# yu45020/Text_Segmentation_Image_Inpainting

Measured on NVIDIA H100. Metric: PartialConv UNet 512x512 images/sec (fwd+bwd), higher is better.
Workload: dtype bf16

## Files before the change

### text_segmentation_image_inpainting_b200/csrc/conv_tc.cu

```cuda
#include <cuda.h>
#include <stdlib.h>
#include <string.h>

#include <algorithm>

#include "pcb_common.cuh"
#include "pcb_ptx.cuh"

namespace {

constexpr int BLOCK_M = 128;
constexpr int BLOCK_K = 64;
constexpr int A_STAGE_BYTES = BLOCK_M * 128;
constexpr int NUM_PRODUCER_THREADS = 128;
constexpr int TC_MAX_PARTS = 2;
constexpr int MMA_WARPS = 8;
constexpr int MMA_THREADS = MMA_WARPS * 32;
constexpr int acc_pitch(int block_n) { return block_n + 4; }
constexpr int acc_stage_bytes(int block_n) { return BLOCK_M * acc_pitch(block_n) * 4; }

inline int rup(int v, int m) { return (v + m - 1) / m * m; }

struct TcPart {
    const bf16 *x;
    const uint64_t *tapmask;
    const uint8_t *mask;
    bf16 *dx;
    int c, c8, kext, koff, choff, cstride, xup, mup, dx_cstride;
};

struct TcParams {
    int n, h, w, cin, cout, kh, kw, stride, pad_h, pad_w, dil, ho, wo;
    int m_total;
    int nparts, no_guard, rowpack;
    int hg;
    int ring_a, ring_b;
    int ktap;
    int ncols;
    TcPart parts[TC_MAX_PARTS];
    const float *bias; const float *msum; bf16 *y; int y_cstride;
    const bf16 *dc; int dc_cstride, dc_c8, dc_kext;
    int *abort_flag;
    int l2pf;
    int box_w, box_h, box_n, stages, use_fix;
    int wk_base, wk_row, wk_col;
    int sub, py, px, fh, fw;
    int ksplit;
    float *partial;
    double *bn_sums;
    int bn_c;
    const float *ep_scale, *ep_shift;
    int ep_on, ep_act;
    float ep_slope;
};

constexpr int STAT_SLICE = 256;
constexpr int STAT_SMEM_BYTES = MMA_WARPS * STAT_SLICE * 4 + 16;
constexpr int EPI_WARPS = 4;
constexpr int EPI_STAT_SMEM_BYTES = EPI_WARPS * STAT_SLICE * 4;

__device__ __forceinline__ float warp_transpose_sum(float (&v)[32], int lane) {
#pragma unroll
    for (int off = 16, n = 32; off >= 1; off >>= 1, n >>= 1) {
        const bool upper = (lane & off) != 0;
#pragma unroll
        for (int i = 0; i < 16; ++i) {
            if (i < (n >> 1)) {
                const float send = upper ? v[i] : v[i + (n >> 1)];
                const float keep = upper ? v[i + (n >> 1)] : v[i];
                v[i] = keep + __shfl_xor_sync(0xffffffffu, send, off);
            }
        }
    }
    return v[0];
}

__device__ __forceinline__ uint32_t align1024(uint32_t a) { return (a + 1023u) & ~1023u; }

__device__ __forceinline__ void load_acc32(const float *src, uint32_t (&r)[32]) {
#pragma unroll
    for (int j = 0; j < 8; ++j) {
        const uint4 v = reinterpret_cast<const uint4 *>(src)[j];
        r[4 * j] = v.x; r[4 * j + 1] = v.y; r[4 * j + 2] = v.z; r[4 * j + 3] = v.w;
    }
}

struct EpiRow {
    long long mo;
    int m;
    bool rvalid, hole;
    float inv;
    float dscale[TC_MAX_PARTS];
};

template <int MODE>
__device__ __forceinline__ EpiRow tc_epi_row(const TcParams &P, int m) {
    EpiRow er;
    er.m = m;
    er.rvalid = m < P.m_total;
    er.inv = 0.f;
    er.hole = false;
    er.mo = m;
    int en = 0, eh = 0, ew = 0;
    if (MODE == 1 && er.rvalid) {
        en = m / (P.h * P.w); const int rem = m - en * P.h * P.w; eh = rem / P.w; ew = rem - eh * P.w;
        eh = eh * P.sub + P.py; ew = ew * P.sub + P.px;
        er.mo = (static_cast<long long>(en) * P.fh + eh) * P.fw + ew;
    }
    if (MODE == 0 && er.rvalid && P.sub != 1) {
        en = m / (P.ho * P.wo); const int rem = m - en * P.ho * P.wo; eh = rem / P.wo; ew = rem - eh * P.wo;
        er.mo = (static_cast<long long>(en) * P.fh + eh * P.sub + P.py) * P.fw + ew * P.sub + P.px;
    }
    if (MODE == 0 && er.rvalid) {
        const float s = P.msum ? P.msum[er.mo] : 1.f;
        er.hole = (s == 0.f) && !P.no_guard;
        er.inv = er.hole ? 0.f : 1.0f / s;
    }
#pragma unroll
    for (int p = 0; p < TC_MAX_PARTS; ++p) {
        er.dscale[p] = 1.f;
        if (MODE == 1 && p < P.nparts) {
            const TcPart &pt = P.parts[p];
            if (er.rvalid && pt.dx != nullptr && pt.mask != nullptr)
                er.dscale[p] = pt.mask[(static_cast<long long>(en) * (P.fh >> pt.mup) + (eh >> pt.mup)) * (P.fw >> pt.mup) + (ew >> pt.mup)] ? 1.f : 0.f;
        }
    }
    return er;
}

template <int BLOCK_N, int MODE>
__device__ __forceinline__ void tc_epilogue(const TcParams &P, const EpiRow &er, const float *acc_row, int lane, int n0, float *s_stat,
                                            int cb, int ce, int sq_off) {
                const int m = er.m;
                const bool rvalid = er.rvalid, hole = er.hole;
                const long long mo = er.mo;
                if (P.partial != nullptr) {
    #pragma unroll 1
                    for (int c0 = cb; c0 < ce; c0 += 32) {
                        uint32_t r[32];
                        load_acc32(acc_row + c0, r);
                        if (rvalid) {
                            float *dst = P.partial + static_cast<long long>(m) * P.ncols + n0 + c0;
    #pragma unroll
                            for (int j = 0; j < 32; ++j) atomicAdd(dst + j, __uint_as_float(r[j]));
                        }
                    }
                    return;
                }
    #pragma unroll 1
                for (int c0 = cb; c0 < ce; c0 += 32) {
                    uint32_t r[32];
                    load_acc32(acc_row + c0, r);
                    const int col = n0 + c0;
                    bf16 *orow = nullptr;
                    int nstore = 0;
                    float scale = er.inv;
                    if (MODE == 0) {
                        if (rvalid && col < P.y_cstride) { orow = P.y + mo * P.y_cstride + col; nstore = min(32, P.y_cstride - col); }
                    } else {
                        scale = 1.f;
#pragma unroll
                        for (int p = 0; p < TC_MAX_PARTS; ++p) {
                            if (p >= P.nparts) break;
                            const TcPart &pt = P.parts[p];
                            const int local = col - pt.koff;
                            if (local >= 0 && local < pt.kext && pt.dx != nullptr && local < pt.c8 && rvalid) {
                                orow = pt.dx + mo * pt.dx_cstride + local;
                                nstore = min(32, pt.c8 - local);
                                scale = er.dscale[p];
                            }
                        }
                    }
                    const bool stats = (MODE == 0) && (s_stat != nullptr);
                    if (__any_sync(0xffffffffu, nstore > 0) || stats) {
                        uint4 o[4];
                        __nv_bfloat162 *ob = reinterpret_cast<__nv_bfloat162 *>(o);
                        float bl = 0.f;
                        const bool has_bias = (MODE == 0) && (P.bias != nullptr);
                        if (has_bias && col + lane < P.cout) bl = P.bias[col + lane];
                        const bool edge = (MODE == 0) && (col + 32 > P.cout);
                        const bool ep = (MODE == 0) && (P.ep_on != 0);
                        float el = 1.f, eh = 0.f;
                        if (ep && P.ep_scale != nullptr && col + lane < P.cout) { el = P.ep_scale[col + lane]; eh = P.ep_shift[col + lane]; }
    #pragma unroll
                        for (int j = 0; j < 16; ++j) {
                            float a = __uint_as_float(r[2 * j]), b = __uint_as_float(r[2 * j + 1]);
                            if (MODE == 0) {
                                const float b0 = has_bias ? __shfl_sync(0xffffffffu, bl, 2 * j) : 0.f;
                                const float b1 = has_bias ? __shfl_sync(0xffffffffu, bl, 2 * j + 1) : 0.f;
                                a = hole ? 0.f : fmaf(a, scale, b0);
                                b = hole ? 0.f : fmaf(b, scale, b1);
                                if (ep) {
                                    a = apply_act(fmaf(a, __shfl_sync(0xffffffffu, el, 2 * j), __shfl_sync(0xffffffffu, eh, 2 * j)), P.ep_act, P.ep_slope);
                                    b = apply_act(fmaf(b, __shfl_sync(0xffffffffu, el, 2 * j + 1), __shfl_sync(0xffffffffu, eh, 2 * j + 1)), P.ep_act, P.ep_slope);
                                }
                                if (edge) {
                                    if (col + 2 * j >= P.cout) a = 0.f;
                                    if (col + 2 * j + 1 >= P.cout) b = 0.f;
                                }
                            } else {
                                a *= scale; b *= scale;
                            }
                            ob[j] = __floats2bfloat162_rn(a, b);
                        }
                        if (nstore > 0) {
                            uint4 *dst = reinterpret_cast<uint4 *>(orow);
    #pragma unroll
                            for (int j = 0; j < 4; ++j)
                                if (j * 8 < nstore) dst[j] = o[j];
                        }
                        if (stats) {
                            float v[32], q[32];
                            const float live = rvalid ? 1.f : 0.f;
    #pragma unroll
                            for (int j = 0; j < 16; ++j) {
                                const float2 f = __bfloat1622float2(ob[j]);
                                v[2 * j] = f.x * live; v[2 * j + 1] = f.y * live;
                                q[2 * j] = v[2 * j] * v[2 * j]; q[2 * j + 1] = v[2 * j + 1] * v[2 * j + 1];
                            }
                            const float cs = warp_transpose_sum(v, lane), cq = warp_transpose_sum(q, lane);
                            s_stat[c0 - cb + lane] += cs;
                            s_stat[sq_off + c0 - cb + lane] += cq;
                        }
                    }
                }
}

template <int BLOCK_N>
__device__ __forceinline__ void tc_stats_flush(const TcParams &P, float *s_stat, int lane, int n0, int cb, int ce, int sq_off) {
    __syncwarp();
    for (int c0 = cb; c0 < ce; c0 += 32) {
        const int co = n0 + c0 + lane;
        if (co < P.bn_c) {
            atomicAdd(P.bn_sums + co, static_cast<double>(s_stat[c0 - cb + lane]));
            atomicAdd(P.bn_sums + P.bn_c + co, static_cast<double>(s_stat[sq_off + c0 - cb + lane]));
        }
        s_stat[c0 - cb + lane] = 0.f; s_stat[sq_off + c0 - cb + lane] = 0.f;
    }
    __syncwarp();
}

template <int BLOCK_N>
struct EpiRole {
    static constexpr int HN = (BLOCK_N >= 64) ? BLOCK_N / 2 : BLOCK_N;
    int q, half, cb, ce;
    __device__ __forceinline__ explicit EpiRole(int e) {
        q = 2 * (e >> 2) + (e & 1);
        half = (e & 3) >> 1;
        cb = half * HN;
        ce = (cb + HN <= BLOCK_N) ? cb + HN : cb;
    }
    __device__ __forceinline__ int slice() const { return half * 4 + q; }
};

template <int BLOCK_N>
__device__ __forceinline__ void stage_acc(const float (&acc)[BLOCK_N / 2], float *stage, int e, int lane) {
    constexpr int PITCH = acc_pitch(BLOCK_N);
    const int r0 = 64 * (e >> 2) + 16 * (e & 3) + (lane >> 2), c0 = 2 * (lane & 3);
#pragma unroll
    for (int i = 0; i < BLOCK_N / 2; i += 2) {
        const int row = r0 + 8 * ((i >> 1) & 1), col = 8 * (i >> 2) + c0;
        *reinterpret_cast<float2 *>(stage + row * PITCH + col) = make_float2(acc[i], acc[i + 1]);
    }
}

template <int BLOCK_N, int MODE>
__device__ __forceinline__ void mma_epilogue(const TcParams &P, const float (&acc)[BLOCK_N / 2], float *stage, int e, int lane, int m0, int n0,
                                             float *s_stat) {
    constexpr int PITCH = acc_pitch(BLOCK_N);
    const int g = e >> 2;
    stage_acc<BLOCK_N>(acc, stage, e, lane);
    ptx::named_sync(1 + g, 128);
    const EpiRole<BLOCK_N> R(e);
    const EpiRow er = tc_epi_row<MODE>(P, m0 + R.q * 32 + lane);
    tc_epilogue<BLOCK_N, MODE>(P, er, stage + (R.q * 32 + lane) * PITCH, lane, n0, s_stat, R.cb, R.ce, 128);
    ptx::named_sync(1 + g, 128);
}

template <int BLOCK_N>
__device__ __forceinline__ void tc_stats_final(const TcParams &P, const float *stat_base, int w, int lane, int stat_n0) {
    for (int col = w * 32 + lane; col < BLOCK_N; col += EPI_WARPS * 32) {
        const int co = stat_n0 + col;
        if (co < P.bn_c) {
            float a = 0.f, q = 0.f;
#pragma unroll
            for (int w4 = 0; w4 < EPI_WARPS; ++w4) { a += stat_base[w4 * STAT_SLICE + col]; q += stat_base[w4 * STAT_SLICE + 128 + col]; }
            atomicAdd(P.bn_sums + co, static_cast<double>(a));
            atomicAdd(P.bn_sums + P.bn_c + co, static_cast<double>(q));
        }
    }
}

template <int R> __device__ __forceinline__ void zero_acc(float (&a)[R]) {
#pragma unroll
    for (int i = 0; i < R; ++i) a[i] = 0.f;
}

constexpr int HALO_MAX_HG = 12;
constexpr int PERSIST_THREADS = 4 * 32 + MMA_THREADS + 32;
constexpr int MAX_RING = 8;

template <int BLOCK_N, int MODE, bool HALO>
__global__ void __launch_bounds__(PERSIST_THREADS, 1)
pconv_tc_persistent_kernel(const __grid_constant__ TcParams P, const __grid_constant__ CUtensorMap tmap_w) {
    constexpr int B_STAGE_BYTES = BLOCK_N * 128;
    extern __shared__ uint8_t smem_raw[];
    const uint32_t smem_base = align1024(ptx::smem_u32(smem_raw));
    const int SA = P.ring_a, SB = P.ring_b;
    const int HG = P.hg;
    const uint32_t LBO = 16u * (16u * HG + 1u);
    const uint32_t A_STAGE = HALO ? ((8u * LBO + 127u) & ~127u) : static_cast<uint32_t>(A_STAGE_BYTES);
    const uint32_t sB = smem_base;
    const uint32_t sA = sB + SB * B_STAGE_BYTES;
    const uint32_t sBar = (sA + SA * A_STAGE + 15u) & ~15u;
    const uint32_t bar_full_a = sBar, bar_empty_a = sBar + 8 * MAX_RING;
    const uint32_t bar_full_b = sBar + 16 * MAX_RING, bar_empty_b = sBar + 24 * MAX_RING;
    const uint32_t s_stat_addr = sBar + 32 * MAX_RING;
    const uint32_t s_acc = (s_stat_addr + STAT_SMEM_BYTES + 15u) & ~15u;
    float *acc_stage = reinterpret_cast<float *>(smem_raw + (s_acc - ptx::smem_u32(smem_raw)));

    const int warp = threadIdx.x >> 5, lane = threadIdx.x & 31;
    const int taps = P.kh * P.kw;
    const int np = (MODE == 0) ? P.nparts : 1;
    const int n_tiles = P.ncols / BLOCK_N;
    const int num_tiles = ((P.m_total + BLOCK_M - 1) / BLOCK_M) * n_tiles;
    const int nB = HALO ? P.kw : 1;

    auto tile_active = [&](int n0) -> bool {
        if (MODE == 0) return true;
        for (int p = 0; p < P.nparts; ++p)
            if (P.parts[p].dx && n0 < P.parts[p].koff + P.parts[p].kext && n0 + BLOCK_N > P.parts[p].koff) return true;
        return false;
    };

    if (threadIdx.x == 0) {
        for (int s = 0; s < MAX_RING; ++s) {
            ptx::mbar_init(bar_full_a + 8 * s, NUM_PRODUCER_THREADS); ptx::mbar_init(bar_empty_a + 8 * s, 2);
            ptx::mbar_init(bar_full_b + 8 * s, 1); ptx::mbar_init(bar_empty_b + 8 * s, 2);
        }
        ptx::fence_mbar_init();
    }
    if (warp == 12 && lane == 0) ptx::prefetch_tmap(&tmap_w);
    __syncthreads();

    if (warp < 4) {
        const int t = threadIdx.x;
        const int chunk = t & 7, r0 = t >> 3;
        const int plane = (MODE == 0) ? P.ho * P.wo : P.h * P.w;
        const int pwid = (MODE == 0) ? P.wo : P.w;
        int it = 0;
        bool dead = false;
        constexpr int NW = HALO ? HALO_MAX_HG : 8;
        uint64_t wnext[TC_MAX_PARTS][NW];
        auto issue_mask_loads = [&](int tl) {
#pragma unroll
            for (int p = 0; p < TC_MAX_PARTS; ++p)
#pragma unroll
                for (int i = 0; i < NW; ++i) wnext[p][i] = 0ull;
            if (MODE != 0 || tl >= num_tiles) return;
            const int tm0 = (tl / n_tiles) * BLOCK_M;
#pragma unroll
            for (int i = 0; i < NW; ++i) {
                int idx;
                if (HALO) {
                    if (i >= HG) continue;
                    const int S = r0 + 16 * i;
                    const int g = S / HG, sl = S - g * HG;
                    const int tcs = sl > 7 ? (sl - 7 + P.dil - 1) / P.dil : 0;
                    idx = tm0 + g * 8 + (sl - tcs * P.dil);
                    if (tm0 + g * 8 >= P.m_total) continue;
                } else {
                    idx = tm0 + r0 + 16 * i;
                    if (idx >= P.m_total) continue;
                }
#pragma unroll
                for (int p = 0; p < TC_MAX_PARTS; ++p)
                    if (p < P.nparts) wnext[p][i] = __ldg(P.parts[p].tapmask + idx);
            }
        };
        issue_mask_loads(blockIdx.x);
        for (int tile = blockIdx.x; tile < num_tiles && !dead; tile += gridDim.x) {
            const int m0 = (tile / n_tiles) * BLOCK_M, n0 = (tile % n_tiles) * BLOCK_N;
            uint64_t wcur[TC_MAX_PARTS][NW];
#pragma unroll
            for (int p = 0; p < TC_MAX_PARTS; ++p)
#pragma unroll
                for (int i = 0; i < NW; ++i) wcur[p][i] = wnext[p][i];
            issue_mask_loads(tile + gridDim.x);
            if (!tile_active(n0)) continue;
            if (HALO) {
                int ph[HALO_MAX_HG];
                int cterm[TC_MAX_PARTS][HALO_MAX_HG];
                uint32_t vb[TC_MAX_PARTS][HALO_MAX_HG];
#pragma unroll
                for (int i = 0; i < HALO_MAX_HG; ++i) {
                    ph[i] = 0;
#pragma unroll
                    for (int p = 0; p < TC_MAX_PARTS; ++p) { vb[p][i] = 0; cterm[p][i] = 0; }
                    if (i >= HG) continue;
                    const int S = r0 + 16 * i;
                    const int g = S / HG, sl = S - g * HG;
                    const int m = m0 + g * 8;
                    const bool ok = m < P.m_total;
                    const int mm = ok ? m : 0;
                    const int nn = mm / plane, rem = mm - nn * plane;
                    const int hh = rem / pwid, ww = rem - hh * pwid;
                    if (MODE == 0) {
                        ph[i] = hh - P.pad_h;
                        const int col = ww - P.pad_w + sl;
                        const int tcs = sl > 7 ? (sl - 7 + P.dil - 1) / P.dil : 0;
#pragma unroll
                        for (int p = 0; p < TC_MAX_PARTS; ++p) {
                            if (p >= P.nparts || !ok) continue;
                            const TcPart &pt = P.parts[p];
                            const uint64_t word = wcur[p][i];
                            uint32_t bits = 0;
                            for (int tr = 0; tr < P.kh; ++tr) bits |= static_cast<uint32_t>((word >> (tr * P.kw + tcs)) & 1ull) << tr;
                            vb[p][i] = bits;
                            const int colc = min(max(col, 0), P.w - 1) >> pt.xup;
                            cterm[p][i] = (nn * (P.h >> pt.xup) * (P.w >> pt.xup) + colc) * pt.cstride + chunk * 8;
                        }
                    } else {
                        ph[i] = hh + P.pad_h;
                        const int col = ww + P.pad_w - (P.kw - 1) * P.dil + sl;
                        const bool cok = ok && col >= 0 && col < P.wo;
                        uint32_t bits = 0;
                        for (int tr = 0; tr < P.kh; ++tr) { const int hi = ph[i] - tr * P.dil; bits |= (cok && hi >= 0 && hi < P.ho ? 1u : 0u) << tr; }
                        vb[0][i] = bits;
                        cterm[0][i] = (nn * P.ho * P.wo + min(max(col, 0), P.wo - 1)) * P.dc_cstride + chunk * 8;
                    }
                }
                for (int tr = 0; tr < P.kh && !dead; ++tr) {
#pragma unroll
                    for (int p = 0; p < TC_MAX_PARTS; ++p) {
                        if (p >= np || dead) break;
                        const TcPart &pt = P.parts[p];
                        const bf16 *src = (MODE == 0) ? pt.x : P.dc;
                        const int xup = (MODE == 0) ? pt.xup : 0;
                        const int hmax = ((MODE == 0) ? (P.h >> xup) : P.ho) - 1;
// ... 75 lines not shown
                            const bool v = (chunk < P.kw) && ((tmv[0][i] >> (tr * P.kw + chunk)) & 1ull);
                            off[i] = v ? (ibase[0][i] - chunk * 8) + (ph[i] + tr * P.dil) * rowpitch + (pw[i] + chunk * P.dil) * cs : 0;
                            ok[i] = v;
                        }
                        if (!push(pt.x, off, ok)) dead = true;
                    }
                } else {
                    for (int tap = 0; tap < taps && !dead; ++tap) {
                        const int tr = tap / P.kw, tc = tap - tr * P.kw;
#pragma unroll
                        for (int p = 0; p < TC_MAX_PARTS; ++p) {
                            if (p >= np || dead) break;
                            const TcPart &pt = P.parts[p];
                            const bf16 *src = (MODE == 0) ? pt.x : P.dc;
                            const int cs = (MODE == 0) ? pt.cstride : P.dc_cstride;
                            const int xup = (MODE == 0) ? pt.xup : 0;
                            const int rowpitch = ((MODE == 0) ? (P.w >> xup) : P.wo) * cs;
                            int base[8];
                            bool rv[8];
#pragma unroll
                            for (int i = 0; i < 8; ++i) {
                                bool v;
                                int hi, wi;
                                if (MODE == 0) {
                                    v = (tmv[p][i] >> tap) & 1ull;
                                    hi = (ph[i] + tr * P.dil) >> xup; wi = (pw[i] + tc * P.dil) >> xup;
                                } else {
                                    const int th = ph[i] - tr * P.dil, tw = pw[i] - tc * P.dil;
                                    hi = th >> ls; wi = tw >> ls;
                                    v = prow[i] && th >= 0 && tw >= 0 && ((th | tw) & (P.stride - 1)) == 0 && hi < P.ho && wi < P.wo;
                                }
                                base[i] = v ? ibase[p][i] + hi * rowpitch + wi * cs : 0;
                                rv[i] = v;
                            }
                            const int nb = ((MODE == 0) ? pt.kext : P.dc_kext) / BLOCK_K;
                            const int c8 = (MODE == 0) ? pt.c8 : P.dc_c8;
                            for (int cb = 0; cb < nb; ++cb) {
                                const bool cv = cb * BLOCK_K + chunk * 8 < c8;
                                int off[8];
                                bool ok[8];
#pragma unroll
                                for (int i = 0; i < 8; ++i) { ok[i] = rv[i] && cv; off[i] = ok[i] ? base[i] + cb * BLOCK_K : 0; }
                                if (!push(src, off, ok)) { dead = true; break; }
                            }
                        }
                    }
                }
            }
        }
        ptx::cp_async_wait<0>();
    } else if (warp == 12) {
        if (lane == 0) {
            int itb = 0;
            bool dead = false;
            auto load = [&](int kidx, int n0) -> bool {
                const int s = itb % SB;
                if (!ptx::mbar_wait(bar_empty_b + 8 * s, ((itb / SB) & 1) ^ 1, P.abort_flag, 103)) return false;
                ptx::mbar_arrive_expect_tx(bar_full_b + 8 * s, B_STAGE_BYTES);
                ptx::tma_load_2d(sB + s * B_STAGE_BYTES, &tmap_w, kidx, n0, bar_full_b + 8 * s);
                ++itb;
                return true;
            };
            for (int tile = blockIdx.x; tile < num_tiles && !dead; tile += gridDim.x) {
                const int n0 = (tile % n_tiles) * BLOCK_N;
                if (!tile_active(n0)) continue;
                if (HALO) {
                    for (int tr = 0; tr < P.kh && !dead; ++tr)
                        for (int p = 0; p < np && !dead; ++p) {
                            const int nb = ((MODE == 0) ? P.parts[p].kext : P.dc_kext) / BLOCK_K;
                            for (int cb = 0; cb < nb && !dead; ++cb)
                                for (int tc = 0; tc < P.kw; ++tc) {
                                    const int tap = tr * P.kw + tc;
                                    const int kidx = (MODE == 0) ? tap * P.ktap + P.parts[p].koff + cb * BLOCK_K : tap * P.dc_kext + cb * BLOCK_K;
                                    if (!load(kidx, n0)) { dead = true; break; }
                                }
                        }
                } else {
                    const int num_kb = (MODE == 0) ? (P.rowpack ? P.kh : taps * (P.ktap / BLOCK_K)) : taps * (P.dc_kext / BLOCK_K);
                    for (int kb = 0; kb < num_kb; ++kb)
                        if (!load(kb * BLOCK_K, n0)) { dead = true; break; }
                }
            }
        }
    } else {
        const int e = warp - 4, g = e >> 2;
        const bool leader = (threadIdx.x & 127) == 0;
        int num_a = 0;
        if (HALO) {
            for (int p = 0; p < np; ++p) num_a += ((MODE == 0) ? P.parts[p].kext : P.dc_kext) / BLOCK_K;
            num_a *= P.kh;
        } else {
            num_a = (MODE == 0) ? (P.rowpack ? P.kh : taps * (P.ktap / BLOCK_K)) : taps * (P.dc_kext / BLOCK_K);
        }
        const uint32_t a_rows = HALO ? 8u * HG * 16u : 64u * 128u;
        float *s_stat = (MODE == 0 && P.bn_sums != nullptr && P.partial == nullptr)
                            ? reinterpret_cast<float *>(smem_raw + (s_stat_addr - ptx::smem_u32(smem_raw))) : nullptr;
        const EpiRole<BLOCK_N> R(e);
        float *my_stat = s_stat ? s_stat + R.slice() * STAT_SLICE : nullptr;
        int stat_n0 = -1;
        if (my_stat) {
            for (int i = lane; i < STAT_SLICE; i += 32) my_stat[i] = 0.f;
            __syncwarp();
        }
        int ita = 0, itb = 0;
        bool dead = false;
        for (int tile = blockIdx.x; tile < num_tiles && !dead; tile += gridDim.x) {
            const int m0 = (tile / n_tiles) * BLOCK_M, n0 = (tile % n_tiles) * BLOCK_N;
            if (!tile_active(n0)) continue;
            if (my_stat && n0 != stat_n0) {
                if (stat_n0 >= 0) tc_stats_flush<BLOCK_N>(P, my_stat, lane, stat_n0, R.cb, R.ce, 128);
                stat_n0 = n0;
            }
            float acc[BLOCK_N / 2];
            zero_acc(acc);
            for (int a = 0; a < num_a && !dead; ++a, ++ita) {
                const int sa = ita % SA;
                if (!__all_sync(0xffffffffu, ptx::mbar_wait(bar_full_a + 8 * sa, (ita / SA) & 1, P.abort_flag, 104))) { dead = true; break; }
                ptx::fence_proxy_async_smem();
                const int sb0 = itb % SB;
                for (int tc = 0; tc < nB; ++tc, ++itb) {
                    const int sb = itb % SB;
                    if (!__all_sync(0xffffffffu, ptx::mbar_wait(bar_full_b + 8 * sb, (itb / SB) & 1, P.abort_flag, 105))) { dead = true; break; }
                    const uint64_t db = ptx::make_smem_desc(sB + sb * B_STAGE_BYTES, 16, 1024);
                    ptx::wgmma_fence();
                    if (HALO) {
                        const int shift = ((MODE == 0) ? tc : (P.kw - 1 - tc)) * P.dil;
                        const uint32_t a0 = sA + sa * A_STAGE + g * a_rows + shift * 16;
#pragma unroll
                        for (int k = 0; k < BLOCK_K / 16; ++k)
                            ptx::wgmma_bf16<BLOCK_N, 0, 0>(acc, ptx::make_smem_desc_noswizzle(a0 + k * 2 * LBO, LBO, HG * 16), db + 2 * k);
                    } else {
                        const uint64_t da = ptx::make_smem_desc(sA + sa * A_STAGE + g * a_rows, 16, 1024);
#pragma unroll
                        for (int k = 0; k < BLOCK_K / 16; ++k)
                            ptx::wgmma_bf16<BLOCK_N, 0, 0>(acc, da + 2 * k, db + 2 * k);
                    }
                    ptx::wgmma_commit();
                }
                ptx::wgmma_wait<0>();
                ptx::wgmma_fence_regs(acc);
                if (leader) {
                    for (int tc = 0; tc < nB; ++tc) ptx::mbar_arrive(bar_empty_b + 8 * ((sb0 + tc) % SB));
                    ptx::mbar_arrive(bar_empty_a + 8 * sa);
                }
            }
            if (dead) { stat_n0 = -1; break; }
            mma_epilogue<BLOCK_N, MODE>(P, acc, acc_stage, e, lane, m0, n0, my_stat);
        }
        if (my_stat && stat_n0 >= 0) tc_stats_flush<BLOCK_N>(P, my_stat, lane, stat_n0, R.cb, R.ce, 128);
    }
}


constexpr int EPI_WARP0 = MMA_WARPS + 5;
constexpr int TMA_THREADS = (EPI_WARP0 + EPI_WARPS) * 32;

constexpr size_t TMA_BAR_BYTES = 24 * MAX_RING + 16;

template <int BLOCK_N, int MODE, typename TileFn>
__device__ __forceinline__ void tma_epilogue_warps(const TcParams &P, int tile0, int tstep, int num_tiles, TileFn tile_origin,
                                                   const float *acc_stage, uint32_t acc_full, uint32_t acc_empty, float *s_stat,
                                                   int &stat_n0, int w, int lane, int code) {
    constexpr int PITCH = acc_pitch(BLOCK_N);
    const float *acc_row = acc_stage + (w * 32 + lane) * PITCH;
    if (s_stat) {
        for (int i = lane; i < STAT_SLICE; i += 32) s_stat[i] = 0.f;
        __syncwarp();
    }
    uint32_t ph = 0;
    for (int tile = tile0; tile < num_tiles; tile += tstep) {
        int m0, n0;
        tile_origin(tile, m0, n0);
        if (n0 < 0) continue;
        if (s_stat && n0 != stat_n0) {
            if (stat_n0 >= 0) tc_stats_flush<BLOCK_N>(P, s_stat, lane, stat_n0, 0, BLOCK_N, 128);
            stat_n0 = n0;
        }
        const EpiRow er = tc_epi_row<MODE>(P, m0 + w * 32 + lane);
        if (!__all_sync(0xffffffffu, ptx::mbar_wait(acc_full, ph, P.abort_flag, code))) { stat_n0 = -1; return; }
        ph ^= 1;
        tc_epilogue<BLOCK_N, MODE>(P, er, acc_row, lane, n0, s_stat, 0, BLOCK_N, 128);
        __syncwarp();
        if (lane == 0) ptx::mbar_arrive(acc_empty);
    }
}

template <int BLOCK_N>
__device__ __forceinline__ bool tma_stage_tile(const TcParams &P, const float (&acc)[BLOCK_N / 2], float *acc_stage, uint32_t acc_full,
                                               uint32_t acc_empty, uint32_t &ph, int e, int lane, int code) {
    if (!__all_sync(0xffffffffu, ptx::mbar_wait(acc_empty, ph, P.abort_flag, code))) return false;
    ph ^= 1;
    stage_acc<BLOCK_N>(acc, acc_stage, e, lane);
    __syncwarp();
    if (lane == 0) ptx::mbar_arrive(acc_full);
    return true;
}

template <int BLOCK_N, int MODE, bool HALO>
__global__ void __launch_bounds__(TMA_THREADS, 1)
pconv_tc_tma_kernel(const __grid_constant__ TcParams P, const __grid_constant__ CUtensorMap tmap_w,
                    const __grid_constant__ CUtensorMap tmap_a0, const __grid_constant__ CUtensorMap tmap_a1) {
    constexpr uint32_t B_BYTES = BLOCK_N * 128;
    extern __shared__ uint8_t smem_raw[];
    const uint32_t smem_base = align1024(ptx::smem_u32(smem_raw));
    const int S = P.stages;
    const int nB = HALO ? P.kw : 1;
    const int hx = HALO ? (P.kw - 1) * P.dil : 0;
    const uint32_t A_BYTES = static_cast<uint32_t>(BLOCK_M + hx) * 128u;
    const uint32_t A_ROOM = (A_BYTES + 1023u) & ~1023u;
    const uint32_t STAGE = A_ROOM + nB * B_BYTES;
    const uint32_t STAGE_TX = A_BYTES + nB * B_BYTES;
    const uint32_t sBar = smem_base + S * STAGE;
    const uint32_t bar_full = sBar, bar_fixed = sBar + 8 * MAX_RING, bar_empty = sBar + 16 * MAX_RING;
    const uint32_t acc_full = sBar + 24 * MAX_RING, acc_empty = acc_full + 8;
    const uint32_t s_stat_addr = sBar + TMA_BAR_BYTES;
    const uint32_t s_acc = s_stat_addr + EPI_STAT_SMEM_BYTES;
    uint8_t *smem_gen = smem_raw + (smem_base - ptx::smem_u32(smem_raw));

    const int warp = __shfl_sync(0xffffffffu, threadIdx.x >> 5, 0), lane = threadIdx.x & 31;
    const int np = (MODE == 0) ? P.nparts : 1;
    const int n_tiles = P.ncols / BLOCK_N;
    const int KS = P.ksplit;
    const int m_tiles = (P.m_total + BLOCK_M - 1) / BLOCK_M;
    const int num_tiles = m_tiles * n_tiles * KS;
    const int tile0 = static_cast<int>(blockIdx.x), tstep = static_cast<int>(gridDim.x);
    auto m0_of = [&](int mt) -> int { return mt * BLOCK_M; };
    const bool fix = (MODE == 0) && P.use_fix;
    const int kwi = HALO ? 1 : P.kw;

    auto tile_active = [&](int n0) -> bool {
        if (MODE == 0) return true;
        for (int p = 0; p < P.nparts; ++p)
            if (P.parts[p].dx && n0 < P.parts[p].koff + P.parts[p].kext && n0 + BLOCK_N > P.parts[p].koff) return true;
        return false;
    };

    if (threadIdx.x == 0) {
        for (int s = 0; s < MAX_RING; ++s) {
            ptx::mbar_init(bar_full + 8 * s, 1); ptx::mbar_init(bar_fixed + 8 * s, 4); ptx::mbar_init(bar_empty + 8 * s, 2);
        }
        ptx::mbar_init(acc_full, MMA_WARPS); ptx::mbar_init(acc_empty, EPI_WARPS);
        ptx::fence_mbar_init();
    }
    if (warp == 8 && lane == 0) { ptx::prefetch_tmap(&tmap_w); ptx::prefetch_tmap(&tmap_a0); if (np > 1) ptx::prefetch_tmap(&tmap_a1); }
    __syncthreads();

    float *s_stat = nullptr;
    int stat_n0 = -1;
    float *acc_stage = reinterpret_cast<float *>(smem_gen + (s_acc - smem_base));
    if (warp >= EPI_WARP0) {
        const int w = warp - EPI_WARP0;
        s_stat = (MODE == 0 && P.bn_sums != nullptr && P.partial == nullptr)
                     ? reinterpret_cast<float *>(smem_gen + (s_stat_addr - smem_base)) + w * STAT_SLICE : nullptr;
        auto origin = [&](int tile, int &m0, int &n0) {
            const int mn = tile / KS;
            m0 = m0_of(mn / n_tiles); n0 = (mn % n_tiles) * BLOCK_N;
            if (!tile_active(n0)) n0 = -1;
        };
        tma_epilogue_warps<BLOCK_N, MODE>(P, tile0, tstep, num_tiles, origin, acc_stage, acc_full, acc_empty, s_stat, stat_n0, w, lane, 126);
    } else if (warp == 8) {
        int s = 0;
        uint32_t ph = 1;
        const int plane = (MODE == 0) ? P.ho * P.wo : P.h * P.w;
        const int pwid = (MODE == 0) ? P.wo : P.w;
        const int kext0 = (MODE == 0) ? P.parts[0].kext : P.dc_kext, kext1 = (MODE == 0 && np > 1) ? P.parts[1].kext : 0;
        const int dstep = (MODE == 0) ? P.dil : -P.dil;
        const int row_k = P.wk_row, col_k = P.wk_col;
        bool dead = false;
        for (int tile = tile0; tile < num_tiles && !dead; tile += tstep) {
            const int sp = tile % KS, mn = tile / KS;
            const int m0 = m0_of(mn / n_tiles), n0 = (mn % n_tiles) * BLOCK_N;
            if (!tile_active(n0)) continue;
            const int img = m0 / plane, rem = m0 - img * plane;
            const int oy = rem / pwid, ox = rem - oy * pwid;
            const int x_org = (MODE == 0) ? ox * P.stride - P.pad_w : (HALO ? ox + P.pad_w - hx : ox + P.pad_w);
            const int y_org = (MODE == 0) ? oy * P.stride - P.pad_h : oy + P.pad_h;
            int nx_org = 0, ny_org = 0, nimg = -1;
            if (P.l2pf && tile + tstep < num_tiles) {
                const int nmn = (tile + tstep) / KS;
                const int nm0 = m0_of(nmn / n_tiles);
                if (nm0 != m0) {
                    nimg = nm0 / plane;
                    const int nrem = nm0 - nimg * plane, noy = nrem / pwid, nox = nrem - noy * pwid;
                    nx_org = (MODE == 0) ? nox * P.stride - P.pad_w : (HALO ? nox + P.pad_w - hx : nox + P.pad_w);
                    ny_org = (MODE == 0) ? noy * P.stride - P.pad_h : noy + P.pad_h;
                }
            }
            int krow = P.wk_base;
            for (int tr = 0, y = y_org; tr < P.kh && !dead; ++tr, y += dstep, krow += row_k)
                for (int ti = 0, x = x_org, kidx = krow; ti < kwi && !dead; ++ti, x += dstep, kidx = krow + ti * col_k) {
#pragma unroll
                    for (int p = 0; p < TC_MAX_PARTS; ++p) {
                        const int kext = (p == 0) ? kext0 : kext1;
                        const CUtensorMap *ma = (p == 0) ? &tmap_a0 : &tmap_a1;
                        const int gb0 = (p == 0) ? 0 : kext0 / BLOCK_K;
                        for (int c0 = 0; c0 < kext; c0 += BLOCK_K, kidx += BLOCK_K) {
                            if (KS > 1 && (gb0 + c0 / BLOCK_K) % KS != sp) continue;
                            if (!__all_sync(0xffffffffu, ptx::mbar_wait(bar_empty + 8 * s, ph, P.abort_flag, 121))) { dead = true; break; }
                            if (ptx::elect_one()) {
                                const uint32_t full = bar_full + 8 * s, dst = smem_base + s * STAGE;
                                ptx::mbar_arrive_expect_tx(full, STAGE_TX);
                                ptx::tma_load_4d(dst, ma, c0, x, y, img, full);
                                uint32_t bdst = dst + A_ROOM;
                                for (int tc = 0, kb = kidx; tc < nB; ++tc, kb += col_k, bdst += B_BYTES)
                                    ptx::tma_load_2d(bdst, &tmap_w, kb, n0, full);
                                if (nimg >= 0) ptx::tma_prefetch_4d(ma, c0, nx_org + ti * dstep, ny_org + tr * dstep, nimg);
                            }
                            __syncwarp();
                            if (++s == S) { s = 0; ph ^= 1; }
                        }
                        if (dead) break;
                    }
                }
        }
    } else if (warp < MMA_WARPS) {
        const int e = warp, g = warp >> 2;
        const bool leader = (threadIdx.x & 127) == 0;
        const uint32_t ready = fix ? bar_fixed : bar_full;
        const uint64_t desc_a0 = ptx::make_smem_desc(smem_base + g * 64 * 128, 16, 1024);
        const uint64_t desc_b0 = ptx::make_smem_desc(smem_base + A_ROOM, 16, 1024);
        const uint32_t stage16 = STAGE >> 4;
        const int shift0 = (HALO && MODE == 1) ? hx * 8 : 0;
        const int dshift = HALO ? ((MODE == 1) ? -P.dil * 8 : P.dil * 8) : 0;
        const int rows_a = P.kh * kwi;
        int nb0, nb1 = 0, kl0, kl1 = 4;
        {
            const int kext = (MODE == 0) ? P.parts[0].kext : P.dc_kext, c8 = (MODE == 0) ? P.parts[0].c8 : P.dc_c8;
            nb0 = kext / BLOCK_K; kl0 = min(4, (c8 - (nb0 - 1) * BLOCK_K + 15) >> 4);
            if (MODE == 0 && np > 1) { nb1 = P.parts[1].kext / BLOCK_K; kl1 = min(4, (P.parts[1].c8 - (nb1 - 1) * BLOCK_K + 15) >> 4); }
        }
        int s = 0;
        uint32_t ph = 0, aph = 1;
        bool dead = false;
        for (int tile = tile0; tile < num_tiles && !dead; tile += tstep) {
            const int sp = tile % KS, mn = tile / KS;
            const int n0 = (mn % n_tiles) * BLOCK_N;
            if (!tile_active(n0)) continue;
            float acc[BLOCK_N / 2];
            zero_acc(acc);
            int held = -1;
            for (int r = 0; r < rows_a && !dead; ++r) {
#pragma unroll
                for (int p = 0; p < TC_MAX_PARTS; ++p) {
                    const int nbp = (p == 0) ? nb0 : nb1, klast = (p == 0) ? kl0 : kl1;
                    const int gb0 = (p == 0) ? 0 : nb0;
                    for (int cb = 0; cb < nbp; ++cb) {
                        if (KS > 1 && (gb0 + cb) % KS != sp) continue;
                        if (!__all_sync(0xffffffffu, ptx::mbar_wait(ready + 8 * s, ph, P.abort_flag, 124))) { dead = true; break; }
                        uint64_t da = desc_a0 + static_cast<uint64_t>(s * stage16 + shift0), db = desc_b0 + static_cast<uint64_t>(s * stage16);
                        const int ksteps = (cb + 1 < nbp) ? 4 : klast;
                        ptx::wgmma_fence();
                        for (int tc = 0; tc < nB; ++tc, da += dshift, db += B_BYTES >> 4) {
                            if (ksteps == 4) {
#pragma unroll
                                for (int k = 0; k < 4; ++k) ptx::wgmma_bf16<BLOCK_N, 0, 0>(acc, da + 2 * k, db + 2 * k);
                            } else {
                                for (int k = 0; k < ksteps; ++k) ptx::wgmma_bf16<BLOCK_N, 0, 0>(acc, da + 2 * k, db + 2 * k);
                            }
                        }
                        ptx::wgmma_commit();
                        ptx::wgmma_wait<1>();
                        if (held >= 0 && leader) ptx::mbar_arrive(bar_empty + 8 * held);
                        held = s;
                        if (++s == S) { s = 0; ph ^= 1; }
                    }
                    if (dead) break;
                }
            }
            ptx::wgmma_wait<0>();
            ptx::wgmma_fence_regs(acc);
            if (held >= 0 && leader) ptx::mbar_arrive(bar_empty + 8 * held);
            if (dead) break;
            if (!tma_stage_tile<BLOCK_N>(P, acc, acc_stage, acc_full, acc_empty, aph, e, lane, 125)) break;
        }
    } else if (warp > 8) {
        if (fix) {
            const int t = (warp - 9) * 32 + lane;
            int s = 0;
            uint32_t ph = 0;
            bool dead = false;
            if (!HALO) {
                uint64_t wnext[TC_MAX_PARTS];
                auto load_words = [&](int tl) {
#pragma unroll
                    for (int p = 0; p < TC_MAX_PARTS; ++p) {
                        wnext[p] = 0ull;
                        const int m = m0_of(tl / KS / n_tiles) + t;
                        if (fix && p < P.nparts && tl < num_tiles && m < P.m_total) wnext[p] = __ldg(P.parts[p].tapmask + m);
                    }
                };
                load_words(tile0);
                for (int tile = tile0; tile < num_tiles && !dead; tile += tstep) {
                    const int sp = tile % KS;
                    uint64_t wcur[TC_MAX_PARTS];
#pragma unroll
                    for (int p = 0; p < TC_MAX_PARTS; ++p) wcur[p] = wnext[p];
                    load_words(tile + tstep);
                    if (MODE == 1 && !tile_active(((tile / KS) % n_tiles) * BLOCK_N)) continue;
                    const int taps = P.kh * P.kw;
                    for (int tap = 0; tap < taps && !dead; ++tap) {
#pragma unroll
                        for (int p = 0; p < TC_MAX_PARTS; ++p) {
                            if (p >= np) break;
                            const bool hole = fix && ((wcur[p] >> tap) & 1ull) == 0ull;
                            const bool any_hole = __any_sync(0xffffffffu, hole);
                            const int nb = ((MODE == 0) ? P.parts[p].kext : P.dc_kext) / BLOCK_K;
                            const int gb0 = (p == 0) ? 0 : P.parts[0].kext / BLOCK_K;
                            for (int cb = 0; cb < nb; ++cb) {
                                if (KS > 1 && (gb0 + cb) % KS != sp) continue;
                                if (!ptx::mbar_wait(bar_full + 8 * s, ph, P.abort_flag, 122)) { dead = true; break; }
                                if (any_hole) {
                                    if (hole) {
                                        uint4 *r = reinterpret_cast<uint4 *>(smem_gen + s * STAGE + t * 128);
                                        const uint4 z = make_uint4(0u, 0u, 0u, 0u);
#pragma unroll
                                        for (int k = 0; k < 8; ++k) r[k] = z;
                                    }
                                    ptx::fence_proxy_async_smem();
                                }
                                __syncwarp();
                                if (lane == 0) ptx::mbar_arrive(bar_fixed + 8 * s);
                                if (++s == S) { s = 0; ph ^= 1; }
                            }
                            if (dead) break;
                        }
                    }
                }
            } else {
                const int plane = P.ho * P.wo;
                auto load_bits = [&](int tl, uint32_t &b0, uint32_t &b1) {
                    b0 = b1 = 0;
                    if (!fix || tl >= num_tiles) return;
                    const int m0 = m0_of(tl / KS / n_tiles);
                    const int img = m0 / plane, rem = m0 - img * plane;
                    const int oy = rem / P.wo, ox = rem - oy * P.wo;
#pragma unroll
                    for (int p = 0; p < TC_MAX_PARTS; ++p) {
                        if (p >= P.nparts || P.parts[p].mask == nullptr) continue;
                        const int mup = P.parts[p].mup;
                        const uint8_t *mk = P.parts[p].mask + static_cast<long long>(img) * (P.h >> mup) * (P.w >> mup);
                        for (int tr = 0; tr < P.kh; ++tr) {
                            const int y = oy - P.pad_h + tr * P.dil;
                            if (y < 0 || y >= P.h) continue;
                            const int x0 = ox - P.pad_w + t, x1 = x0 + 128;
                            if (x0 >= 0 && x0 < P.w && __ldg(mk + (y >> mup) * (P.w >> mup) + (x0 >> mup)) == 0) b0 |= 1u << (p * 8 + tr);
                            if (t < hx && x1 < P.w && __ldg(mk + (y >> mup) * (P.w >> mup) + (x1 >> mup)) == 0) b1 |= 1u << (p * 8 + tr);
                        }
                    }
                };
                uint32_t n0b, n1b;
                load_bits(tile0, n0b, n1b);
                for (int tile = tile0; tile < num_tiles && !dead; tile += tstep) {
                    const int sp = tile % KS;
                    const uint32_t c0b = n0b, c1b = n1b;
                    load_bits(tile + tstep, n0b, n1b);
                    if (MODE == 1 && !tile_active(((tile / KS) % n_tiles) * BLOCK_N)) continue;
                    for (int tr = 0; tr < P.kh && !dead; ++tr) {
#pragma unroll
                        for (int p = 0; p < TC_MAX_PARTS; ++p) {
                            if (p >= np) break;
                            const bool h0 = (c0b >> (p * 8 + tr)) & 1u, h1 = (c1b >> (p * 8 + tr)) & 1u;
                            const bool any_hole = __any_sync(0xffffffffu, h0 || h1);
                            const int nb = ((MODE == 0) ? P.parts[p].kext : P.dc_kext) / BLOCK_K;
                            const int gb0 = (p == 0) ? 0 : P.parts[0].kext / BLOCK_K;
                            for (int cb = 0; cb < nb; ++cb) {
                                if (KS > 1 && (gb0 + cb) % KS != sp) continue;
                                if (!ptx::mbar_wait(bar_full + 8 * s, ph, P.abort_flag, 122)) { dead = true; break; }
                                if (any_hole) {
                                    const uint4 z = make_uint4(0u, 0u, 0u, 0u);
                                    if (h0) {
                                        uint4 *r = reinterpret_cast<uint4 *>(smem_gen + s * STAGE + t * 128);
#pragma unroll
                                        for (int k = 0; k < 8; ++k) r[k] = z;
                                    }
                                    if (h1) {
                                        uint4 *r = reinterpret_cast<uint4 *>(smem_gen + s * STAGE + (t + 128) * 128);
#pragma unroll
                                        for (int k = 0; k < 8; ++k) r[k] = z;
                                    }
                                    ptx::fence_proxy_async_smem();
                                }
                                __syncwarp();
                                if (lane == 0) ptx::mbar_arrive(bar_fixed + 8 * s);
                                if (++s == S) { s = 0; ph ^= 1; }
                            }
                            if (dead) break;
                        }
                    }
                }
            }
        }
    }

    __syncthreads();
    if (s_stat != nullptr && stat_n0 >= 0) tc_stats_final<BLOCK_N>(P, s_stat - (warp - EPI_WARP0) * STAT_SLICE, warp - EPI_WARP0, lane, stat_n0);
}


constexpr int SP_MAX_ITEMS = 40;
struct SpItem { int part, dx, dy, wk, nb, wk_step, shift0, dshift; };
struct SpTable {
    int n_items;
    int step[TC_MAX_PARTS];
    int es[TC_MAX_PARTS];
    int ph[TC_MAX_PARTS], pw[TC_MAX_PARTS];
    int arows[TC_MAX_PARTS];
    int rows_max;
    SpItem it[SP_MAX_ITEMS];
};

template <int BLOCK_N, int MODE>
__global__ void __launch_bounds__(TMA_THREADS, 1)
pconv_tc_sp_kernel(const __grid_constant__ TcParams P, const __grid_constant__ SpTable TB, const __grid_constant__ CUtensorMap tmap_w,
                   const __grid_constant__ CUtensorMap tmap_a0, const __grid_constant__ CUtensorMap tmap_a1) {
    constexpr uint32_t B_BYTES = BLOCK_N * 128;
    extern __shared__ uint8_t smem_raw[];
    const uint32_t smem_base = align1024(ptx::smem_u32(smem_raw));
    const int S = P.stages;
    int nb_max = 1;
    for (int i = 0; i < TB.n_items; ++i) nb_max = max(nb_max, TB.it[i].nb);
    const uint32_t A_ROOM = (static_cast<uint32_t>(TB.rows_max) * 128u + 1023u) & ~1023u;
    const uint32_t STAGE = A_ROOM + nb_max * B_BYTES;
    const uint32_t sBar = smem_base + S * STAGE;
    const uint32_t bar_full = sBar, bar_fixed = sBar + 8 * MAX_RING, bar_empty = sBar + 16 * MAX_RING;
    const uint32_t acc_full = sBar + 24 * MAX_RING, acc_empty = acc_full + 8;
    const uint32_t s_stat_addr = sBar + TMA_BAR_BYTES;
    const uint32_t s_acc = s_stat_addr + EPI_STAT_SMEM_BYTES;
    uint8_t *smem_gen = smem_raw + (smem_base - ptx::smem_u32(smem_raw));

    const int warp = __shfl_sync(0xffffffffu, threadIdx.x >> 5, 0), lane = threadIdx.x & 31;
    const int n_tiles = P.ncols / BLOCK_N;
    const int m_tiles = (P.m_total + BLOCK_M - 1) / BLOCK_M;
    const int num_tiles = m_tiles * n_tiles;
    const int tile0 = static_cast<int>(blockIdx.x), tstep = static_cast<int>(gridDim.x);
    const bool fix = P.use_fix != 0;
    const int gw = (MODE == 0) ? P.wo : P.w, gh = (MODE == 0) ? P.ho : P.h;
    const int plane = gw * gh;
    int nbk[TC_MAX_PARTS], klast[TC_MAX_PARTS];
#pragma unroll
    for (int p = 0; p < TC_MAX_PARTS; ++p) {
        const int kext = (MODE == 0) ? P.parts[p].kext : P.dc_kext, c8 = (MODE == 0) ? P.parts[p].c8 : P.dc_c8;
        nbk[p] = (p < ((MODE == 0) ? P.nparts : 1)) ? kext / BLOCK_K : 0;
        klast[p] = nbk[p] ? min(4, (c8 - (nbk[p] - 1) * BLOCK_K + 15) >> 4) : 4;
    }

    if (threadIdx.x == 0) {
        for (int s = 0; s < MAX_RING; ++s) { ptx::mbar_init(bar_full + 8 * s, 1); ptx::mbar_init(bar_fixed + 8 * s, 4); ptx::mbar_init(bar_empty + 8 * s, 2); }
        ptx::mbar_init(acc_full, MMA_WARPS); ptx::mbar_init(acc_empty, EPI_WARPS);
        ptx::fence_mbar_init();
    }
    if (warp == 8 && lane == 0) { ptx::prefetch_tmap(&tmap_w); ptx::prefetch_tmap(&tmap_a0); ptx::prefetch_tmap(&tmap_a1); }
    __syncthreads();

    float *s_stat = nullptr;
    int stat_n0 = -1;
    float *acc_stage = reinterpret_cast<float *>(smem_gen + (s_acc - smem_base));
    if (warp >= EPI_WARP0) {
        const int w = warp - EPI_WARP0;
        s_stat = (MODE == 0 && P.bn_sums != nullptr) ? reinterpret_cast<float *>(smem_gen + (s_stat_addr - smem_base)) + w * STAT_SLICE : nullptr;
        auto origin = [&](int tile, int &m0, int &n0) { m0 = (tile / n_tiles) * BLOCK_M; n0 = (tile % n_tiles) * BLOCK_N; };
        tma_epilogue_warps<BLOCK_N, MODE>(P, tile0, tstep, num_tiles, origin, acc_stage, acc_full, acc_empty, s_stat, stat_n0, w, lane, 326);
    } else if (warp == 8) {
        int s = 0;
        uint32_t ph = 1;
        bool dead = false;
        for (int tile = tile0; tile < num_tiles && !dead; tile += tstep) {
            const int m0 = (tile / n_tiles) * BLOCK_M, n0 = (tile % n_tiles) * BLOCK_N;
            const int img = m0 / plane, rem = m0 - img * plane;
            const int oy = rem / gw, ox = rem - oy * gw;
            for (int i = 0; i < TB.n_items && !dead; ++i) {
                const SpItem it = TB.it[i];
                const CUtensorMap *ma = (it.part == 0) ? &tmap_a0 : &tmap_a1;
                const int x = ox * TB.step[it.part] + it.dx, y = oy * TB.step[it.part] + it.dy;
                const uint32_t a_bytes = static_cast<uint32_t>(TB.arows[it.part]) * 128u;
                for (int cb = 0; cb < nbk[it.part]; ++cb) {
                    if (!__all_sync(0xffffffffu, ptx::mbar_wait(bar_empty + 8 * s, ph, P.abort_flag, 321))) { dead = true; break; }
                    if (ptx::elect_one()) {
                        const uint32_t full = bar_full + 8 * s, dst = smem_base + s * STAGE;
                        ptx::mbar_arrive_expect_tx(full, a_bytes + it.nb * B_BYTES);
                        ptx::tma_load_4d(dst, ma, cb * BLOCK_K, x, y, img, full);
                        uint32_t bdst = dst + A_ROOM;
                        for (int tc = 0, kb = it.wk + cb * BLOCK_K; tc < it.nb; ++tc, kb += it.wk_step, bdst += B_BYTES)
                            ptx::tma_load_2d(bdst, &tmap_w, kb, n0, full);
                    }
                    __syncwarp();
                    if (++s == S) { s = 0; ph ^= 1; }
                }
            }
        }
    } else if (warp < MMA_WARPS) {
        const int e = warp, g = warp >> 2;
        const bool leader = (threadIdx.x & 127) == 0;
        const uint32_t ready = fix ? bar_fixed : bar_full;
        const uint64_t desc_a0 = ptx::make_smem_desc(smem_base + g * 64 * 128, 16, 1024);
        const uint64_t desc_b0 = ptx::make_smem_desc(smem_base + A_ROOM, 16, 1024);
        const uint32_t stage16 = STAGE >> 4;
        int s = 0;
        uint32_t ph = 0, aph = 1;
        bool dead = false;
        for (int tile = tile0; tile < num_tiles && !dead; tile += tstep) {
            float acc[BLOCK_N / 2];
            zero_acc(acc);
            int held = -1;
            for (int i = 0; i < TB.n_items && !dead; ++i) {
                const SpItem it = TB.it[i];
                for (int cb = 0; cb < nbk[it.part]; ++cb) {
                    if (!__all_sync(0xffffffffu, ptx::mbar_wait(ready + 8 * s, ph, P.abort_flag, 324))) { dead = true; break; }
                    uint64_t da = desc_a0 + static_cast<uint64_t>(s * stage16 + it.shift0), db = desc_b0 + static_cast<uint64_t>(s * stage16);
                    const int ksteps = (cb + 1 < nbk[it.part]) ? 4 : klast[it.part];
                    ptx::wgmma_fence();
                    for (int tc = 0; tc < it.nb; ++tc, da += it.dshift, db += B_BYTES >> 4)
                        for (int k = 0; k < ksteps; ++k) ptx::wgmma_bf16<BLOCK_N, 0, 0>(acc, da + 2 * k, db + 2 * k);
                    ptx::wgmma_commit();
                    ptx::wgmma_wait<1>();
                    if (held >= 0 && leader) ptx::mbar_arrive(bar_empty + 8 * held);
                    held = s;
                    if (++s == S) { s = 0; ph ^= 1; }
                }
            }
            ptx::wgmma_wait<0>();
            ptx::wgmma_fence_regs(acc);
            if (held >= 0 && leader) ptx::mbar_arrive(bar_empty + 8 * held);
            if (dead) break;
            if (!tma_stage_tile<BLOCK_N>(P, acc, acc_stage, acc_full, acc_empty, aph, e, lane, 325)) break;
        }
    } else if (warp > 8) {
        if (fix) {
            const int t = (warp - 9) * 32 + lane;
            int s = 0;
            uint32_t ph = 0;
            bool dead = false;
            auto load_bits = [&](int tl, uint64_t &b0, uint64_t &b1) {
                b0 = b1 = 0ull;
                if (tl >= num_tiles) return;
                const int m0 = (tl / n_tiles) * BLOCK_M;
                const int img = m0 / plane, rem = m0 - img * plane;
                const int oy = rem / gw, ox = rem - oy * gw;
                for (int i = 0; i < TB.n_items; ++i) {
                    const SpItem it = TB.it[i];
                    const uint8_t *mk = P.parts[it.part].mask;
                    if (mk == nullptr) continue;
                    const int pwid = TB.pw[it.part], phei = TB.ph[it.part], es = TB.es[it.part];
                    const int hrows = TB.arows[it.part] - BLOCK_M;
                    const int x0 = ox * TB.step[it.part] + it.dx, y0 = oy * TB.step[it.part] + it.dy;
                    int tx, ty, tn;
                    if (hrows > 0 || (P.box_h == 1 && P.box_n == 1)) { tx = t; ty = 0; tn = 0; }
                    else { tx = t % P.box_w; ty = (t / P.box_w) % P.box_h; tn = t / (P.box_w * P.box_h); }
                    const int X = x0 + tx * es, Y = y0 + ty * es, IM = img + tn;
                    if (X >= 0 && X < pwid && Y >= 0 && Y < phei && IM < P.n &&
                        __ldg(mk + (static_cast<long long>(IM) * phei + Y) * pwid + X) == 0) b0 |= 1ull << i;
                    if (t < hrows) {
                        const int X1 = x0 + (t + 128) * es;
                        if (X1 >= 0 && X1 < pwid && Y >= 0 && Y < phei && __ldg(mk + (static_cast<long long>(IM) * phei + Y) * pwid + X1) == 0) b1 |= 1ull << i;
                    }
                }
            };
            uint64_t n0b, n1b;
            load_bits(tile0, n0b, n1b);
            for (int tile = tile0; tile < num_tiles && !dead; tile += tstep) {
                const uint64_t c0b = n0b, c1b = n1b;
                load_bits(tile + tstep, n0b, n1b);
                for (int i = 0; i < TB.n_items && !dead; ++i) {
                    const bool h0 = (c0b >> i) & 1ull, h1 = (c1b >> i) & 1ull;
                    const bool any_hole = __any_sync(0xffffffffu, h0 || h1);
                    const int nb_i = nbk[TB.it[i].part];
                    for (int cb = 0; cb < nb_i; ++cb) {
                        if (!ptx::mbar_wait(bar_full + 8 * s, ph, P.abort_flag, 322)) { dead = true; break; }
                        if (any_hole) {
                            const uint4 z = make_uint4(0u, 0u, 0u, 0u);
                            if (h0) {
                                uint4 *r = reinterpret_cast<uint4 *>(smem_gen + s * STAGE + t * 128);
#pragma unroll
                                for (int k = 0; k < 8; ++k) r[k] = z;
                            }
                            if (h1) {
                                uint4 *r = reinterpret_cast<uint4 *>(smem_gen + s * STAGE + (t + 128) * 128);
#pragma unroll
                                for (int k = 0; k < 8; ++k) r[k] = z;
                            }
                            ptx::fence_proxy_async_smem();
                        }
                        __syncwarp();
                        if (lane == 0) ptx::mbar_arrive(bar_fixed + 8 * s);
                        if (++s == S) { s = 0; ph ^= 1; }
                    }
                }
            }
        }
    }

    __syncthreads();
    if (s_stat != nullptr && stat_n0 >= 0) tc_stats_final<BLOCK_N>(P, s_stat - (warp - EPI_WARP0) * STAT_SLICE, warp - EPI_WARP0, lane, stat_n0);
}

__global__ void upsample_part_kernel(const bf16 *__restrict__ src, int cstride, int c8, long long pixels_src, int hs, int ws, bf16 *__restrict__ dst) {
    const int chunks = c8 >> 3;
    const long long total = pixels_src * chunks;
    for (long long i = blockIdx.x * static_cast<long long>(blockDim.x) + threadIdx.x; i < total; i += static_cast<long long>(gridDim.x) * blockDim.x) {
        const int ch = static_cast<int>(i % chunks);
        const long long pix = i / chunks;
        const int x = static_cast<int>(pix % ws);
        const long long t = pix / ws;
        const int y = static_cast<int>(t % hs);
        const long long n = t / hs;
        const uint4 v = __ldg(reinterpret_cast<const uint4 *>(src + pix * cstride + ch * 8));
        bf16 *d = dst + ((n * (2 * hs) + 2 * y) * (2ll * ws) + 2 * x) * c8 + ch * 8;
        uint4 *d0 = reinterpret_cast<uint4 *>(d), *d1 = reinterpret_cast<uint4 *>(d + 2ll * ws * c8);
        d0[0] = v; *reinterpret_cast<uint4 *>(d + c8) = v;
        d1[0] = v; *reinterpret_cast<uint4 *>(d + 2ll * ws * c8 + c8) = v;
    }
}

struct WgParams {
    int n, h, w, cin, cout, kh, kw, stride, pad_h, pad_w, dil, ho, wo;
    int m_total;
    int nparts, rowpack;
    int ktap;
    int ntaps;
    TcPart parts[TC_MAX_PARTS];
    int tap_groups;
    int ci_tiles;
    int kb_per_split;
    float *dw;
    int *abort_flag;
    int box_w, box_h, box_n, stages, use_fix;
};

constexpr int WGRAD_THREADS = MMA_THREADS + 5 * 32;

template <int BLOCK_N, int T>
__device__ __forceinline__ void wgrad_store(const WgParams &P, const float (&acc)[T][BLOCK_N / 2], int ntap, int lane, int n0,
                                            int ncols, const int (&ci)[2], const int (&tap)[2][T]) {
    const int taps_full = P.kh * P.kw;
#pragma unroll
    for (int tl = 0; tl < T; ++tl) {
        if (tl >= ntap) break;
#pragma unroll
        for (int i = 0; i < BLOCK_N / 2; ++i) {
            if (2 * i >= ncols) break;
            const int h = (i >> 1) & 1;
            const int co = n0 + 8 * (i >> 2) + 2 * (lane & 3) + (i & 1);
            if (ci[h] >= 0 && co < P.cout)
                atomicAdd(P.dw + (static_cast<long long>(co) * taps_full + tap[h][tl]) * P.cin + ci[h], acc[tl][i]);
        }
    }
}

template <int BLOCK_N, int T, int STAGES>
__global__ void __launch_bounds__(WGRAD_THREADS, 1)
pconv_tc_wgrad_kernel(const __grid_constant__ WgParams P, const __grid_constant__ CUtensorMap tmap_dc) {
    constexpr int B_STAGE_BYTES = BLOCK_N * 128;
    constexpr int A_TAP_BYTES = 16384;
    constexpr int A_STAGE = T * A_TAP_BYTES;
    extern __shared__ uint8_t smem_raw[];
    const uint32_t smem_base = align1024(ptx::smem_u32(smem_raw));
    const uint32_t sA = smem_base;
    const uint32_t sB = sA + STAGES * A_STAGE;
    const uint32_t sBar = sB + STAGES * B_STAGE_BYTES;
    const uint32_t bar_full_a = sBar, bar_full_b = sBar + 8 * STAGES, bar_empty = sBar + 16 * STAGES;

    const int warp = threadIdx.x >> 5, lane = threadIdx.x & 31;
    int bx = blockIdx.x;
    const int ci_tile = bx % P.ci_tiles; bx /= P.ci_tiles;
    const int tap_group = bx % P.tap_groups;
    const int co_tile = bx / P.tap_groups;
    const int taps_full = P.kh * P.kw;
    const int tap0 = tap_group * T;
    const int ntap = min(T, P.ntaps - tap0);
    const int n0 = co_tile * BLOCK_N;
    const int total_kb = (P.m_total + 63) / 64;
    const int kb_begin = blockIdx.y * P.kb_per_split;
    const int kb_end = min(total_kb, kb_begin + P.kb_per_split);
    const int num_kb = max(0, kb_end - kb_begin);

    if (threadIdx.x == 0) {
        for (int s = 0; s < STAGES; ++s) {
            ptx::mbar_init(bar_full_a + 8 * s, NUM_PRODUCER_THREADS);
            ptx::mbar_init(bar_full_b + 8 * s, 1);
            ptx::mbar_init(bar_empty + 8 * s, 2);
        }
        ptx::fence_mbar_init();
    }
    if (warp == 12 && lane == 0) ptx::prefetch_tmap(&tmap_dc);
    __syncthreads();

    if (warp >= MMA_WARPS && warp < MMA_WARPS + 4) {
        const int t = threadIdx.x - MMA_THREADS;
        const int chunk = t & 7, r0 = t >> 3;
        const uint32_t sw = static_cast<uint32_t>((chunk ^ (r0 & 7)) << 4);
        int blk_part[2], blk_off[2];
        bool blk_cv[2];
#pragma unroll
        for (int hb = 0; hb < 2; ++hb) {
            const int kpos = ci_tile * 128 + hb * 64;
            blk_part[hb] = -1; blk_off[hb] = 0; blk_cv[hb] = false;
            if (P.rowpack) {
                if (kpos == 0) { blk_part[hb] = 0; blk_cv[hb] = chunk < P.kw; }
            } else {
                for (int p = 0; p < P.nparts; ++p)
                    if (kpos >= P.parts[p].koff && kpos < P.parts[p].koff + P.parts[p].kext) {
                        blk_part[hb] = p; blk_off[hb] = kpos - P.parts[p].koff;
                        blk_cv[hb] = blk_off[hb] + chunk * 8 < P.parts[p].c8;
                    }
            }
        }
        const int plane = P.ho * P.wo;
        bool dead = false;
        int dtr[T], dtc[T], tbit[T];
#pragma unroll
        for (int tl = 0; tl < T; ++tl) {
            const int tg = tap0 + tl;
            if (P.rowpack) { dtr[tl] = tg * P.dil; dtc[tl] = chunk * P.dil; tbit[tl] = tg * P.kw + chunk; }
            else { const int tr = tg / P.kw, tc = tg - tr * P.kw; dtr[tl] = tr * P.dil; dtc[tl] = tc * P.dil; tbit[tl] = tg; }
        }
        const bf16 *bsrc[2];
        int bcs[2], brow[2], bimg[2], bxup[2], boff[2];
#pragma unroll
        for (int hb = 0; hb < 2; ++hb) {
            const TcPart &pt = P.parts[blk_part[hb] >= 0 ? blk_part[hb] : 0];
            bsrc[hb] = pt.x; bcs[hb] = pt.cstride; bxup[hb] = pt.xup;
            brow[hb] = (P.w >> pt.xup) * pt.cstride;
            bimg[hb] = (P.h >> pt.xup) * brow[hb];
            boff[hb] = P.rowpack ? 0 : blk_off[hb] + chunk * 8;
        }
        const bool fastrow = P.wo >= 64;
        uint64_t tm_next[4][2];
        auto load_tm = [&](int kb, uint64_t (&dst)[4][2]) {
#pragma unroll
            for (int i = 0; i < 4; ++i) {
                const int m = kb * 64 + r0 + 16 * i;
#pragma unroll
                for (int hb = 0; hb < 2; ++hb)
                    dst[i][hb] = (m < P.m_total && blk_part[hb] >= 0 && blk_cv[hb]) ? __ldg(P.parts[blk_part[hb]].tapmask + m) : 0ull;
            }
        };
        if (num_kb > 0) load_tm(kb_begin, tm_next);
        for (int it = 0; it < num_kb && !dead; ++it) {
            const int kb = kb_begin + it;
            const int s = it % STAGES;
            const uint32_t parity = ((it / STAGES) & 1) ^ 1;
            uint64_t tm_cur[4][2];
#pragma unroll
            for (int i = 0; i < 4; ++i) { tm_cur[i][0] = tm_next[i][0]; tm_cur[i][1] = tm_next[i][1]; }
            if (it + 1 < num_kb) load_tm(kb + 1, tm_next);
            const int mf = kb * 64;
// ... 564 lines not shown
    P.pad_h = c->pad_h; P.pad_w = c->pad_w; P.dil = c->dil; P.ho = c->ho; P.wo = c->wo;
    P.nparts = c->nparts; P.no_guard = c->no_guard; P.rowpack = L.rowpack; P.ktap = L.ktap;
    P.sub = 1; P.py = 0; P.px = 0; P.fh = c->h; P.fw = c->w;
    P.l2pf = getenv("PCB_TMA_L2_PREFETCH") != nullptr;
}

int halo_hg(const pcb_conv *c, bool rowpack) {
    if (rowpack || c->stride != 1 || getenv("PCB_DISABLE_HALO")) return 0;
    const int hg = 8 + (c->kw - 1) * c->dil;
    if (c->kw < 2 || hg > HALO_MAX_HG || c->kh > 8) return 0;
    if (c->wo % 8 != 0 || c->w % 8 != 0 || c->wo != c->w) return 0;
    return hg;
}

constexpr size_t MAX_SMEM = 227 * 1024;
constexpr size_t RING_BUDGET = 208 * 1024;

template <int BLOCK_N, int MODE, bool HALO>
int launch_persistent(TcParams &P, const CUtensorMap &tm, cudaStream_t st) {
    const size_t a_stage = HALO ? ((8 * 16 * (16 * P.hg + 1) + 127) / 128 * 128) : A_STAGE_BYTES;
    const size_t b_stage = BLOCK_N * 128;
    const size_t budget = RING_BUDGET - acc_stage_bytes(BLOCK_N);
    P.ring_b = 6;
    P.ring_a = HALO ? 3 : 6;
    while (P.ring_a * a_stage + P.ring_b * b_stage > budget && P.ring_b > 3) --P.ring_b;
    while (P.ring_a * a_stage + P.ring_b * b_stage > budget && P.ring_a > 2) --P.ring_a;
    const size_t smem = 1024 + P.ring_a * a_stage + P.ring_b * b_stage + 32 * MAX_RING + 16 + STAT_SMEM_BYTES + acc_stage_bytes(BLOCK_N);
    PCB_CHECK(smem <= MAX_SMEM, "tensor-core conv: %zu bytes of shared memory do not fit", smem);
    auto kern = pconv_tc_persistent_kernel<BLOCK_N, MODE, HALO>;
    PCB_SMEM_OPT_IN(kern, MAX_SMEM);
    const int num_tiles = ((P.m_total + BLOCK_M - 1) / BLOCK_M) * (P.ncols / BLOCK_N);
    const int grid = std::min(num_tiles, pcb_num_sms());
    kern<<<grid, PERSIST_THREADS, smem, st>>>(P, tm);
    PCB_LAUNCH_CHECK();
    return 0;
}


float *splitk_scratch(size_t bytes) {
    static float *buf[PCB_MAX_DEVICES] = {};
    static size_t cap[PCB_MAX_DEVICES] = {};
    const int dev = pcb_cur_device();
    if (bytes > cap[dev]) {
        const size_t want = std::max<size_t>(bytes, 16u << 20);
        float *fresh = nullptr;
        if (cudaMalloc(&fresh, want) != cudaSuccess) { cudaGetLastError(); return nullptr; }
        buf[dev] = fresh; cap[dev] = want;
    }
    return buf[dev];
}

__global__ void splitk_finish_fwd_kernel(const float *__restrict__ part, int ncols, const float *__restrict__ msum, const float *__restrict__ bias, int cout,
                                         int no_guard, long long m_total, bf16 *__restrict__ y, int y_cstride) {
    const int cv = y_cstride >> 3;
    const long long total = m_total * cv;
    for (long long i = blockIdx.x * static_cast<long long>(blockDim.x) + threadIdx.x; i < total; i += static_cast<long long>(gridDim.x) * blockDim.x) {
        const long long m = i / cv;
        const int col = static_cast<int>(i - m * cv) * 8;
        const float s = msum ? msum[m] : 1.f;
        const bool hole = (s == 0.f) && !no_guard;
        const float inv = hole ? 0.f : 1.0f / s;
        uint4 o;
        __nv_bfloat162 *ob = reinterpret_cast<__nv_bfloat162 *>(&o);
#pragma unroll
        for (int j = 0; j < 4; ++j) {
            const int co = col + 2 * j;
            float a = (co < ncols) ? part[m * ncols + co] : 0.f, b = (co + 1 < ncols) ? part[m * ncols + co + 1] : 0.f;
            a = (hole || co >= cout) ? 0.f : a * inv + (bias ? bias[co] : 0.f);
            b = (hole || co + 1 >= cout) ? 0.f : b * inv + (bias ? bias[co + 1] : 0.f);
            ob[j] = __floats2bfloat162_rn(a, b);
        }
        *reinterpret_cast<uint4 *>(y + m * y_cstride + col) = o;
    }
}

__global__ void splitk_finish_dgrad_kernel(const float *__restrict__ part, const TcParams P) {
    const int cv = P.ncols >> 3;
    const long long total = static_cast<long long>(P.m_total) * cv;
    for (long long i = blockIdx.x * static_cast<long long>(blockDim.x) + threadIdx.x; i < total; i += static_cast<long long>(gridDim.x) * blockDim.x) {
        const int m = static_cast<int>(i / cv);
        const int col = static_cast<int>(i - static_cast<long long>(m) * cv) * 8;
        const int en = m / (P.h * P.w), rem = m - en * P.h * P.w;
        const int eh = (rem / P.w) * P.sub + P.py, ew = (rem % P.w) * P.sub + P.px;
        const long long mo = (static_cast<long long>(en) * P.fh + eh) * P.fw + ew;
        for (int p = 0; p < P.nparts; ++p) {
            const TcPart &pt = P.parts[p];
            const int local = col - pt.koff;
            if (local < 0 || local >= pt.c8 || pt.dx == nullptr) continue;
            float scale = 1.f;
            if (pt.mask != nullptr)
                scale = pt.mask[(static_cast<long long>(en) * (P.fh >> pt.mup) + (eh >> pt.mup)) * (P.fw >> pt.mup) + (ew >> pt.mup)] ? 1.f : 0.f;
            const float *src = part + static_cast<long long>(m) * P.ncols + col;
            uint4 o;
            __nv_bfloat162 *ob = reinterpret_cast<__nv_bfloat162 *>(&o);
#pragma unroll
            for (int j = 0; j < 4; ++j) ob[j] = __floats2bfloat162_rn(src[2 * j] * scale, src[2 * j + 1] * scale);
            *reinterpret_cast<uint4 *>(pt.dx + mo * pt.dx_cstride + local) = o;
        }
    }
}

int pick_ksplit(long long m_total, int ncols, int bn, int blocks_per_tap) {
    if (!getenv("PCB_SPLITK")) return 1;
    const long long tiles = ((m_total + BLOCK_M - 1) / BLOCK_M) * (ncols / bn);
    const int sms = pcb_num_sms();
    if (tiles * 2 > sms) return 1;
    int ks = static_cast<int>(std::min<long long>(16, sms / tiles));
    ks = std::min(ks, blocks_per_tap);
    return ks < 2 ? 1 : ks;
}

bool tile_box(int wt, int ht, int *bw, int *bh, int *bn) {
    if (wt < 4) return false;
    if (wt % 128 == 0) { *bw = 128; *bh = 1; *bn = 1; return true; }
    if (128 % wt) return false;
    const int rows = 128 / wt;
    *bw = wt;
    if (ht % rows == 0) { *bh = rows; *bn = 1; return true; }
    if (rows % ht) return false;
    *bh = ht; *bn = rows / ht;
    return true;
}

bool tma_fwd_ok(const pcb_conv *c) {
    if (getenv("PCB_DISABLE_TMA") || is_rowpack(c)) return false;
    int bw, bh, bn;
    if (!tile_box(c->wo, c->ho, &bw, &bh, &bn)) return false;
    if (c->stride > 2 || bw * c->stride > 256 || bh * c->stride > 256) return false;
    for (int p = 0; p < c->nparts; ++p)
        if (c->parts[p].x_up && ((c->h | c->w) & 1)) return false;
    return true;
}

bool tma_dgrad_ok(const pcb_conv *c) {
    if (getenv("PCB_DISABLE_TMA") || is_rowpack(c) || c->stride != 1) return false;
    int bw, bh, bn;
    return tile_box(c->w, c->h, &bw, &bh, &bn);
}

bool tma_dgrad_s2_ok(const pcb_conv *c) {
    if (getenv("PCB_DISABLE_TMA") || getenv("PCB_DISABLE_TMA_S2") || is_rowpack(c)) return false;
    if (c->stride != 2 || c->dil != 1 || c->kh < 2 || c->kw < 2 || ((c->h | c->w) & 1) || c->ho != c->h / 2 || c->wo != c->w / 2) return false;
    int bw, bh, bn;
    return tile_box(c->w / 2, c->h / 2, &bw, &bh, &bn);
}

size_t up_bytes(const pcb_conv *c, int p) {
    return (static_cast<size_t>(c->n) * c->h * c->w * rup(c->parts[p].c, 8) * 2 + 255) / 256 * 256;
}
size_t tapmask_bytes(const pcb_conv *c) {
    return (static_cast<size_t>(c->nparts) * c->n * c->ho * c->wo * sizeof(uint64_t) + 255) / 256 * 256;
}

template <int BLOCK_N, int MODE, bool HALO>
int launch_tma_n(TcParams &P, const CUtensorMap &tw, const CUtensorMap &ta0, const CUtensorMap &ta1, cudaStream_t st) {
    const int nb = HALO ? P.kw : 1;
    const size_t a_room = (static_cast<size_t>(BLOCK_M + (HALO ? (P.kw - 1) * P.dil : 0)) * 128 + 1023) / 1024 * 1024;
    const size_t stage = a_room + static_cast<size_t>(nb) * BLOCK_N * 128;
    P.stages = static_cast<int>(std::min<size_t>(MAX_RING, (RING_BUDGET - acc_stage_bytes(BLOCK_N)) / stage));
    PCB_CHECK(P.stages >= 2, "TMA-fed conv: stage of %zu bytes does not fit twice", stage);
    const size_t smem = 1024 + P.stages * stage + TMA_BAR_BYTES + EPI_STAT_SMEM_BYTES + acc_stage_bytes(BLOCK_N);
    auto kern = pconv_tc_tma_kernel<BLOCK_N, MODE, HALO>;
    PCB_SMEM_OPT_IN(kern, MAX_SMEM);
    if (P.ksplit < 1) P.ksplit = 1;
    const int m_tiles = (P.m_total + BLOCK_M - 1) / BLOCK_M;
    const int num_tiles = m_tiles * (P.ncols / BLOCK_N) * P.ksplit;
    const int grid = std::min(num_tiles, pcb_num_sms());
    kern<<<grid, TMA_THREADS, smem, st>>>(P, tw, ta0, ta1);
    PCB_LAUNCH_CHECK();
    return 0;
}

template <int MODE>
int launch_tma(TcParams &P, const CUtensorMap &tw, const CUtensorMap &ta0, const CUtensorMap &ta1, int bn, bool halo, cudaStream_t st) {
    if (halo) {
        if (bn == 128) return launch_tma_n<128, MODE, true>(P, tw, ta0, ta1, st);
        if (bn == 64) return launch_tma_n<64, MODE, true>(P, tw, ta0, ta1, st);
        return launch_tma_n<32, MODE, true>(P, tw, ta0, ta1, st);
    }
    if (bn == 128) return launch_tma_n<128, MODE, false>(P, tw, ta0, ta1, st);
    if (bn == 64) return launch_tma_n<64, MODE, false>(P, tw, ta0, ta1, st);
    return launch_tma_n<32, MODE, false>(P, tw, ta0, ta1, st);
}

bool halo_stages_fit(int kw, int dil, int block_n) {
    const size_t stage = (static_cast<size_t>(128 + (kw - 1) * dil) * 128 + 1023) / 1024 * 1024 + static_cast<size_t>(kw) * block_n * 128;
    return 3 * stage + acc_stage_bytes(block_n) <= RING_BUDGET;
}

bool tma_halo_ok(const pcb_conv *c, int bw, int bh, int bn, int block_n) {
    if (getenv("PCB_DISABLE_TMA_HALO")) return false;
    if (!(c->stride == 1 && bw == 128 && bh == 1 && bn == 1 && c->kw >= 2 && 128 + (c->kw - 1) * c->dil <= 256 && c->kh <= 8)) return false;
    return halo_stages_fit(c->kw, c->dil, block_n);
}

int pick_bn(int cols, long long m_total) {
    const long long m_tiles = (m_total + BLOCK_M - 1) / BLOCK_M;
    if (cols <= 32) return 32;
    int bn = (cols % 128 == 0) ? 128 : 64;
    if (!getenv("PCB_NO_NARROW_N"))
        while (bn > 32 && cols % (bn / 2) == 0 && m_tiles * (cols / bn) < pcb_num_sms() / 2) bn /= 2;
    return bn;
}

template <int MODE>
int launch_tc(TcParams &P, const CUtensorMap &tm, int bn, cudaStream_t st) {
    if (P.hg) return (bn == 128) ? launch_persistent<128, MODE, true>(P, tm, st) : launch_persistent<64, MODE, true>(P, tm, st);
    return (bn == 128) ? launch_persistent<128, MODE, false>(P, tm, st) : launch_persistent<64, MODE, false>(P, tm, st);
}

}

static bool smallco_ok(const pcb_conv *c);
namespace {

struct SpAxis { int e0[2], ne[2], tapbits[2][4]; bool ok; };

int floordiv2(int v) { return v >= 0 ? v / 2 : -((-v + 1) / 2); }

SpAxis sp_axis(int k, int d, int p) {
    SpAxis A;
    memset(&A, 0, sizeof(A));
    A.ok = k <= 4;
    for (int q = 0; q < 2 && A.ok; ++q) {
        A.e0[q] = floordiv2(q - p);
        const int last = floordiv2(q + (k - 1) * d - p);
        A.ne[q] = last - A.e0[q] + 1;
        if (A.ne[q] < 1 || A.ne[q] > 4) { A.ok = false; break; }
        for (int t = 0; t < k; ++t) A.tapbits[q][floordiv2(q + t * d - p) - A.e0[q]] |= 1 << t;
        for (int e = 0; e < A.ne[q]; ++e)
            if (!A.tapbits[q][e]) A.ok = false;
    }
    return A;
}

struct SpPlan {
    bool ok;
    bool fwd, dgrad;
    int pu, ps;
    SpAxis ay, ax;
    int net[4], eoff[4], net_total;
    int kext_u, kext_s, c8_u, c8_s;
    long long kc[4], clsoff[4], sp_fwd_elems, sp_dg_elems, kd_sp;
    int bw, bh, bn;
};

SpPlan sp_plan(const pcb_conv *c) {
    SpPlan S;
    memset(&S, 0, sizeof(S));
    S.pu = S.ps = -1;
    if (getenv("PCB_DISABLE_SUBPIXEL") || getenv("PCB_DISABLE_TMA") || !common_ok(c) || is_rowpack(c)) return S;
    if (c->stride != 1 || c->ho != c->h || c->wo != c->w || ((c->h | c->w) & 1) || c->nparts > 2) return S;
    for (int p = 0; p < c->nparts; ++p) {
        if (c->parts[p].x_up) { if (S.pu >= 0) return S; S.pu = p; }
        else { if (S.ps >= 0) return S; S.ps = p; }
    }
    if (S.pu < 0) return S;
    if (c->parts[S.pu].mask && c->parts[S.pu].mask_up != 1) return S;
    if (S.ps >= 0 && c->parts[S.ps].mask && c->parts[S.ps].mask_up != 0) return S;
    if (smallco_ok(c)) return S;
    S.ay = sp_axis(c->kh, c->dil, c->pad_h);
    S.ax = sp_axis(c->kw, c->dil, c->pad_w);
    if (!S.ay.ok || !S.ax.ok) return S;
    if (!tile_box(c->w / 2, c->h / 2, &S.bw, &S.bh, &S.bn)) return S;
    const Layout L = layout_of(c);
    S.kext_u = L.kext[S.pu]; S.c8_u = rup(c->parts[S.pu].c, 8);
    S.kext_s = S.ps >= 0 ? L.kext[S.ps] : 0; S.c8_s = S.ps >= 0 ? rup(c->parts[S.ps].c, 8) : 0;
    const int taps = c->kh * c->kw;
    long long off = 0;
    int eo = 0;
    for (int cls = 0; cls < 4; ++cls) {
        S.net[cls] = S.ay.ne[cls >> 1] * S.ax.ne[cls & 1];
        S.eoff[cls] = eo; eo += S.net[cls];
        S.kc[cls] = static_cast<long long>(S.net[cls]) * S.kext_u + static_cast<long long>(S.ps >= 0 ? taps : 0) * S.kext_s;
        S.clsoff[cls] = off; off += static_cast<long long>(L.rows_f) * S.kc[cls];
        if (S.net[cls] + (S.ps >= 0 ? taps : 0) > SP_MAX_ITEMS) return S;
    }
    S.net_total = eo;
    if (S.net_total > SP_MAX_ITEMS) return S;
    S.kd_sp = static_cast<long long>(S.net_total) * L.cout64;
    S.ok = true;
    const long long src_tiles = (static_cast<long long>(c->n) * (c->h / 2) * (c->w / 2) + BLOCK_M - 1) / BLOCK_M;
    S.dgrad = src_tiles >= pcb_num_sms() / 3 || getenv("PCB_SUBPIXEL_ALL") != nullptr;
    S.fwd = getenv("PCB_SUBPIXEL_FWD") != nullptr || getenv("PCB_SUBPIXEL_ALL") != nullptr;
    S.sp_fwd_elems = S.fwd ? off : 0;
    S.sp_dg_elems = S.dgrad ? static_cast<long long>(rup(S.kext_u, 128)) * S.kd_sp : 0;
    if (!S.fwd && !S.dgrad) S.ok = false;
    return S;
}

struct SpWParams {
    int cout, taps, cin, kw, cout64, rows_f;
    int choff_u, c_u, kext_u, choff_s, c_s, kext_s, has_skip;
    int net[4], eoff[4], nex[4], slot0[4];
    int ybits[2][4], xbits[2][4];
    long long kc[4], clsoff[4], kd_sp;
    int want_fwd, want_dg;
};

__global__ void sp_weight_prepare_kernel(const float *__restrict__ wm, const SpWParams W, bf16 *__restrict__ w_f, bf16 *__restrict__ w_d) {
    const int co = blockIdx.x;
    int slot = blockIdx.y, cls = 0;
    while (cls < 3 && slot >= W.slot0[cls + 1]) ++cls;
    slot -= W.slot0[cls];
    const float *wrow = wm + static_cast<long long>(co) * W.taps * W.cin;
    if (slot < W.net[cls]) {
        const int ey = slot / W.nex[cls], ex = slot - ey * W.nex[cls];
        const int yb = W.ybits[cls >> 1][ey], xb = W.xbits[cls & 1][ex];
        for (int ci = threadIdx.x; ci < W.c_u; ci += blockDim.x) {
            float v = 0.f;
            for (int tr = 0; tr < 4; ++tr)
                if ((yb >> tr) & 1)
                    for (int tc = 0; tc < 4; ++tc)
                        if ((xb >> tc) & 1) v += wrow[static_cast<long long>(tr * W.kw + tc) * W.cin + W.choff_u + ci];
            const bf16 b = __float2bfloat16_rn(v);
            if (W.want_fwd) w_f[W.clsoff[cls] + static_cast<long long>(co) * W.kc[cls] + static_cast<long long>(slot) * W.kext_u + ci] = b;
            if (W.want_dg) w_d[static_cast<long long>(ci) * W.kd_sp + static_cast<long long>(W.eoff[cls] + slot) * W.cout64 + co] = b;
        }
    } else if (W.has_skip && W.want_fwd) {
        const int tap = slot - W.net[cls];
        for (int ci = threadIdx.x; ci < W.c_s; ci += blockDim.x)
            w_f[W.clsoff[cls] + static_cast<long long>(co) * W.kc[cls] + static_cast<long long>(W.net[cls]) * W.kext_u + static_cast<long long>(tap) * W.kext_s + ci] =
                __float2bfloat16_rn(wrow[static_cast<long long>(tap) * W.cin + W.choff_s + ci]);
    }
}

__global__ void sp_weight_dg_kernel(const float *__restrict__ wm, const SpWParams W, bf16 *__restrict__ w_d) {
    const int ci = blockIdx.x;
    int slot = blockIdx.y, cls = 0;
    while (cls < 3 && slot >= W.eoff[cls + 1]) ++cls;
    slot -= W.eoff[cls];
    const int ey = slot / W.nex[cls], ex = slot - ey * W.nex[cls];
    const int yb = W.ybits[cls >> 1][ey], xb = W.xbits[cls & 1][ex];
    for (int co = threadIdx.x; co < W.cout; co += blockDim.x) {
        const float *wrow = wm + static_cast<long long>(co) * W.taps * W.cin + W.choff_u + ci;
        float v = 0.f;
        for (int tr = 0; tr < 4; ++tr)
            if ((yb >> tr) & 1)
                for (int tc = 0; tc < 4; ++tc)
                    if ((xb >> tc) & 1) v += wrow[static_cast<long long>(tr * W.kw + tc) * W.cin];
        w_d[static_cast<long long>(ci) * W.kd_sp + static_cast<long long>(W.eoff[cls] + slot) * W.cout64 + co] = __float2bfloat16_rn(v);
    }
}

int sp_weight_prepare(const pcb_conv *c, const SpPlan &S, const Layout &L, const float *w_master, bf16 *w_f, bf16 *w_d, cudaStream_t st) {
    SpWParams W;
    memset(&W, 0, sizeof(W));
    W.cout = c->cout; W.taps = c->kh * c->kw; W.cin = c->cin; W.kw = c->kw; W.cout64 = L.cout64; W.rows_f = L.rows_f;
    int off = 0;
    for (int p = 0; p < c->nparts; ++p) {
        if (p == S.pu) { W.choff_u = off; W.c_u = c->parts[p].c; }
        if (p == S.ps) { W.choff_s = off; W.c_s = c->parts[p].c; }
        off += c->parts[p].c;
    }
    W.kext_u = S.kext_u; W.kext_s = S.kext_s; W.has_skip = S.ps >= 0; W.kd_sp = S.kd_sp;
    W.want_fwd = S.fwd; W.want_dg = S.dgrad;
    int slot = 0;
    for (int cls = 0; cls < 4; ++cls) {
        W.net[cls] = S.net[cls]; W.eoff[cls] = S.eoff[cls]; W.nex[cls] = S.ax.ne[cls & 1]; W.slot0[cls] = slot;
        slot += S.net[cls] + (S.ps >= 0 ? W.taps : 0);
        W.kc[cls] = S.kc[cls]; W.clsoff[cls] = S.clsoff[cls];
    }
    for (int q = 0; q < 2; ++q)
        for (int e = 0; e < 4; ++e) { W.ybits[q][e] = S.ay.tapbits[q][e]; W.xbits[q][e] = S.ax.tapbits[q][e]; }
    if (S.fwd) {
        sp_weight_prepare_kernel<<<dim3(c->cout, slot), 128, 0, st>>>(w_master, W, w_f, w_d);
        PCB_LAUNCH_CHECK();
    } else if (S.dgrad) {
        sp_weight_dg_kernel<<<dim3(W.c_u, S.net_total), 128, 0, st>>>(w_master, W, w_d);
        PCB_LAUNCH_CHECK();
    }
    return 0;
}

int sp_bn(int cols, long long m_total) { return std::min(pick_bn(cols, m_total), 64); }

template <int BLOCK_N, int MODE>
int launch_sp_n(TcParams &P, const SpTable &TB, const CUtensorMap &tw, const CUtensorMap &ta0, const CUtensorMap &ta1, cudaStream_t st) {
    int nb_max = 1;
    for (int i = 0; i < TB.n_items; ++i) nb_max = std::max(nb_max, TB.it[i].nb);
    const size_t a_room = (static_cast<size_t>(TB.rows_max) * 128 + 1023) / 1024 * 1024;
    const size_t stage = a_room + static_cast<size_t>(nb_max) * BLOCK_N * 128;
    P.stages = static_cast<int>(std::min<size_t>(MAX_RING, (RING_BUDGET - acc_stage_bytes(BLOCK_N)) / stage));
    PCB_CHECK(P.stages >= 2, "sub-pixel conv: stage of %zu bytes does not fit twice", stage);
    const size_t smem = 1024 + P.stages * stage + TMA_BAR_BYTES + EPI_STAT_SMEM_BYTES + acc_stage_bytes(BLOCK_N);
    auto kern = pconv_tc_sp_kernel<BLOCK_N, MODE>;
    PCB_SMEM_OPT_IN(kern, MAX_SMEM);
    const int num_tiles = ((P.m_total + BLOCK_M - 1) / BLOCK_M) * (P.ncols / BLOCK_N);
    const int grid = std::min(num_tiles, pcb_num_sms());
    kern<<<grid, TMA_THREADS, smem, st>>>(P, TB, tw, ta0, ta1);
    PCB_LAUNCH_CHECK();
    return 0;
}

template <int MODE>
int launch_sp(TcParams &P, const SpTable &TB, const CUtensorMap &tw, const CUtensorMap &ta0, const CUtensorMap &ta1, int bn, cudaStream_t st) {
    if (bn == 64) return launch_sp_n<64, MODE>(P, TB, tw, ta0, ta1, st);
    return launch_sp_n<32, MODE>(P, TB, tw, ta0, ta1, st);
}

struct ClassStreams4 { cudaStream_t aux[3]; cudaEvent_t ev_fork, ev_join[3]; bool ready; };
int class_streams(ClassStreams4 **out) {
    static thread_local ClassStreams4 cs_all[PCB_MAX_DEVICES] = {};
    ClassStreams4 &CS = cs_all[pcb_cur_device()];
    if (!CS.ready) {
        for (int i = 0; i < 3; ++i) {
            PCB_CUDA(cudaStreamCreateWithFlags(&CS.aux[i], cudaStreamNonBlocking));
            PCB_CUDA(cudaEventCreateWithFlags(&CS.ev_join[i], cudaEventDisableTiming));
        }
        PCB_CUDA(cudaEventCreateWithFlags(&CS.ev_fork, cudaEventDisableTiming));
        CS.ready = true;
    }
    *out = &CS;
    return 0;
}

int sp_forward(const pcb_conv *c, const SpPlan &S, const Layout &L, const bf16 *w_sp, const float *bias, void *y, int y_cstride, const float *msum,
               double *bn_sums, const pcb_ep *ep, int *flag, cudaStream_t st) {
    const int hc = c->h / 2, wc = c->w / 2;
    const long long m_class = static_cast<long long>(c->n) * hc * wc;
    TcParams P;
    base_params(P, c, L);
    fill_parts(c, L, P.parts, nullptr, 0);
    P.ho = hc; P.wo = wc; P.m_total = static_cast<int>(m_class);
    P.sub = 2; P.fh = c->ho; P.fw = c->wo;
    P.bias = bias; P.msum = msum; P.y = static_cast<bf16 *>(y); P.y_cstride = y_cstride; P.abort_flag = flag;
    P.bn_sums = bn_sums; P.bn_c = c->cout;
    set_ep(P, ep);
    P.box_w = S.bw; P.box_h = S.bh; P.box_n = S.bn;
    const int cols = (c->cout <= 32) ? 32 : L.rows_f;
    const int bn = sp_bn(cols, m_class);
    P.ncols = cols;
    for (int p = 0; p < c->nparts; ++p)
        if (c->parts[p].mask) P.use_fix = 1;
    const bool row_tiles = S.bw == 128 && S.bh == 1 && S.bn == 1;
    const int taps = c->kh * c->kw;
    const long long class_tiles = ((m_class + BLOCK_M - 1) / BLOCK_M) * (cols / bn);
    const bool fork = class_tiles < pcb_num_sms() && !getenv("PCB_DISABLE_CLASS_STREAMS");
    ClassStreams4 *CS = nullptr;
    if (fork) {
        if (int rc = class_streams(&CS)) return rc;
        PCB_CUDA(cudaEventRecord(CS->ev_fork, st));
    }
    for (int cls = 0; cls < 4; ++cls) {
        const int py = cls >> 1, px = cls & 1;
        const int ney = S.ay.ne[py], nex = S.ax.ne[px], ey0 = S.ay.e0[py], ex0 = S.ax.e0[px];
        SpTable TB;
        memset(&TB, 0, sizeof(TB));
        const int pu = S.pu, ps = S.ps;
        TB.step[pu] = 1; TB.es[pu] = 1; TB.ph[pu] = hc; TB.pw[pu] = wc;
        const bool halo_u = row_tiles && nex > 1 && !getenv("PCB_DISABLE_TMA_HALO");
        TB.arows[pu] = BLOCK_M + (halo_u ? nex - 1 : 0);
        int ni = 0;
        for (int e = 0; e < ney; ++e) {
            if (halo_u) {
                SpItem &it = TB.it[ni++];
                it.part = pu; it.dx = ex0; it.dy = ey0 + e; it.nb = nex; it.wk = (e * nex) * S.kext_u; it.wk_step = S.kext_u; it.shift0 = 0; it.dshift = 8;
            } else {
                for (int f = 0; f < nex; ++f) {
                    SpItem &it = TB.it[ni++];
                    it.part = pu; it.dx = ex0 + f; it.dy = ey0 + e; it.nb = 1; it.wk = (e * nex + f) * S.kext_u; it.wk_step = 0; it.shift0 = 0; it.dshift = 0;
                }
            }
        }
        if (ps >= 0) {
            TB.step[ps] = 2; TB.es[ps] = 2; TB.ph[ps] = c->h; TB.pw[ps] = c->w;
            TB.arows[ps] = BLOCK_M;
            for (int tr = 0; tr < c->kh; ++tr)
                for (int tc = 0; tc < c->kw; ++tc) {
                    SpItem &it = TB.it[ni++];
                    it.part = ps; it.dx = px + tc * c->dil - c->pad_w; it.dy = py + tr * c->dil - c->pad_h; it.nb = 1;
                    it.wk = S.net[cls] * S.kext_u + (tr * c->kw + tc) * S.kext_s; it.wk_step = 0; it.shift0 = 0; it.dshift = 0;
                }
        }
        TB.n_items = ni;
        TB.rows_max = std::max(TB.arows[pu], ps >= 0 ? TB.arows[ps] : 0);
        PCB_CHECK(ni <= SP_MAX_ITEMS, "sub-pixel conv: too many items");
        CUtensorMap ta[TC_MAX_PARTS], tw;
        memset(ta, 0, sizeof(ta));
        if (int rc = make_tmap_nhwc(&ta[pu], c->parts[pu].x, S.c8_u, wc, hc, c->n, c->parts[pu].x_cstride, S.bw + (halo_u ? nex - 1 : 0), S.bh, S.bn, 1)) return rc;
        if (ps >= 0) {
            if (int rc = make_tmap_nhwc(&ta[ps], c->parts[ps].x, S.c8_s, c->w, c->h, c->n, c->parts[ps].x_cstride, S.bw, S.bh, S.bn, 2)) return rc;
        } else ta[1 - pu] = ta[pu];
        if (int rc = make_tmap_2d(&tw, w_sp + S.clsoff[cls], L.rows_f, S.kc[cls], S.kc[cls], bn)) return rc;
        TcParams Q = P;
        Q.py = py; Q.px = px;
        cudaStream_t cs = (fork && cls > 0) ? CS->aux[cls - 1] : st;
        if (fork && cls > 0) PCB_CUDA(cudaStreamWaitEvent(cs, CS->ev_fork, 0));
        if (int rc = launch_sp<0>(Q, TB, tw, ta[0], ta[1], bn, cs)) return rc;
        if (fork && cls > 0) {
            PCB_CUDA(cudaEventRecord(CS->ev_join[cls - 1], cs));
            PCB_CUDA(cudaStreamWaitEvent(st, CS->ev_join[cls - 1], 0));
        }
    }
    return 0;
}

int sp_dgrad_up(const pcb_conv *c, const SpPlan &S, const Layout &L, const void *dc, int dc_cstride, const bf16 *w_sp_dg, void *dx_u, int dx_cstride,
                int *flag, cudaStream_t st) {
    const int hs = c->h / 2, ws = c->w / 2;
    const long long m_src = static_cast<long long>(c->n) * hs * ws;
    TcParams P;
    base_params(P, c, L);
    P.h = hs; P.w = ws; P.m_total = static_cast<int>(m_src);
    P.sub = 1; P.py = 0; P.px = 0; P.fh = hs; P.fw = ws;
    P.nparts = 1;
    memset(P.parts, 0, sizeof(P.parts));
    TcPart &pt = P.parts[0];
    pt.c = c->parts[S.pu].c; pt.c8 = S.c8_u; pt.kext = S.kext_u; pt.koff = 0; pt.mask = c->parts[S.pu].mask; pt.mup = 0;
    pt.dx = static_cast<bf16 *>(dx_u); pt.dx_cstride = dx_cstride;
    PCB_CHECK(dx_cstride % 8 == 0 && dx_cstride >= S.c8_u && (reinterpret_cast<uintptr_t>(dx_u) & 15) == 0, "sub-pixel dgrad: dx must be 16-byte aligned with a channel stride that is a multiple of 8");
    P.dc = static_cast<const bf16 *>(dc); P.dc_cstride = dc_cstride; P.dc_c8 = rup(c->cout, 8); P.dc_kext = L.cout64;
    P.abort_flag = flag;
    P.ncols = S.kext_u;
    P.box_w = S.bw; P.box_h = S.bh; P.box_n = S.bn;
    const int bn = sp_bn(S.kext_u, m_src);
    SpTable TB;
    memset(&TB, 0, sizeof(TB));
    TB.step[0] = 2; TB.es[0] = 2; TB.ph[0] = c->ho; TB.pw[0] = c->wo; TB.arows[0] = BLOCK_M; TB.rows_max = BLOCK_M;
    int ni = 0;
    for (int cls = 0; cls < 4; ++cls) {
        const int py = cls >> 1, px = cls & 1;
        const int ney = S.ay.ne[py], nex = S.ax.ne[px];
        for (int e = 0; e < ney; ++e)
            for (int f = 0; f < nex; ++f) {
                SpItem &it = TB.it[ni++];
                it.part = 0; it.dx = px - 2 * (S.ax.e0[px] + f); it.dy = py - 2 * (S.ay.e0[py] + e); it.nb = 1;
                it.wk = (S.eoff[cls] + e * nex + f) * L.cout64; it.wk_step = 0; it.shift0 = 0; it.dshift = 0;
            }
    }
    TB.n_items = ni;
    CUtensorMap ta, tw;
    if (int rc = make_tmap_nhwc(&ta, dc, P.dc_c8, c->wo, c->ho, c->n, dc_cstride, S.bw, S.bh, S.bn, 2)) return rc;
    if (int rc = make_tmap_2d(&tw, w_sp_dg, rup(S.kext_u, 128), S.kd_sp, S.kd_sp, bn)) return rc;
    return launch_sp<1>(P, TB, tw, ta, ta, bn, st);
}

}

static bool smallco_ok(const pcb_conv *c) { return common_ok(c) && !is_rowpack(c) && pcb_smallco_eligible(c); }
static pcb_smallco_layout smallco_layout(const Layout &L) {
    pcb_smallco_layout S;
    S.ktap = L.ktap; S.koff[0] = L.koff[0]; S.koff[1] = L.koff[1]; S.cout64 = L.cout64; S.kf = L.kf; S.kd = L.kd;
    return S;
}

bool pcb_tc_eligible(const pcb_conv *c) { return common_ok(c) && !getenv("PCB_DISABLE_TC"); }

static bool tma_wgrad_ok(const pcb_conv *c);

static void k2r_bases(const Layout &L, size_t *fe, size_t *de) {
    *fe = (static_cast<size_t>(L.rows_f) * L.kf + 63) / 64 * 64;
    *de = (static_cast<size_t>(rup(L.ktap, 128)) * L.kd + 63) / 64 * 64;
}

static bool stem_ok(const pcb_conv *c) { return common_ok(c) && is_rowpack(c) && pcb_stem_ok(c); }
static size_t stem_base(const Layout &L) { return (static_cast<size_t>(L.rows_f) * L.kf + 63) / 64 * 64; }

size_t pcb_tc_workspace(const pcb_conv *c) {
    if (smallco_ok(c) && pcb_k2r_ok(c)) return pcb_k2r_workspace(c);
    if (stem_ok(c)) return std::max(pcb_stem_workspace(c), tapmask_bytes(c));
    size_t bytes = tapmask_bytes(c);
    if (tma_fwd_ok(c) || tma_wgrad_ok(c))
        for (int p = 0; p < c->nparts; ++p)
            if (c->parts[p].x_up) bytes += up_bytes(c, p);
    return bytes;
}

void pcb_tc_weight_layout(const pcb_conv *c, size_t *fwd_elems, size_t *dgrad_elems) {
    const Layout L = layout_of(c);
    *fwd_elems = static_cast<size_t>(L.rows_f) * L.kf;
    *dgrad_elems = L.rowpack ? 0 : static_cast<size_t>(rup(L.ktap, 128)) * L.kd;
    const SpPlan S = sp_plan(c);
    if (S.ok) { *fwd_elems += static_cast<size_t>(S.sp_fwd_elems); *dgrad_elems += static_cast<size_t>(S.sp_dg_elems); }
    if (smallco_ok(c) && pcb_k2r_ok(c)) {
        size_t fb, db, fx, dx;
        k2r_bases(L, &fb, &db);
        pcb_k2r_weight_layout(c, &fx, &dx);
        *fwd_elems = fb + fx; *dgrad_elems = db + dx;
    }
    if (stem_ok(c)) *fwd_elems = stem_base(L) + pcb_stem_weight_extra(c);
}

bool pcb_tc_subpixel(const pcb_conv *c) {
    if (smallco_ok(c)) return pcb_k2r_ok(c);
    const SpPlan S = sp_plan(c);
    return S.ok && S.dgrad;
}

int pcb_tc_weight_prepare(const pcb_conv *c, const float *w_master, void *w_fwd, void *w_dgrad, bool zero_padding, cudaStream_t st) {
    const Layout L = layout_of(c);
    size_t fe, de;
    pcb_tc_weight_layout(c, &fe, &de);
    if (zero_padding) {
        PCB_CUDA(cudaMemsetAsync(w_fwd, 0, fe * 2, st));
        if (w_dgrad && de) PCB_CUDA(cudaMemsetAsync(w_dgrad, 0, de * 2, st));
    }
    WPrepParams W;
    memset(&W, 0, sizeof(W));
    W.cout = c->cout; W.taps = c->kh * c->kw; W.cin = c->cin; W.kw = c->kw; W.rowpack = L.rowpack; W.nparts = c->nparts;
    W.ktap = L.ktap; W.cout64 = L.cout64; W.kf = L.kf; W.kd = L.kd;
    int off = 0;
    for (int p = 0; p < c->nparts; ++p) { W.choff[p] = off; W.c[p] = c->parts[p].c; W.koff[p] = L.koff[p]; off += c->parts[p].c; }
    if (!L.rowpack && W.taps <= 65535 && c->cout >= 32 && c->cin >= 32) {
        dim3 tg((c->cin + 31) / 32, (c->cout + 31) / 32, W.taps);
        tc_weight_prepare_tiled_kernel<<<tg, 256, 0, st>>>(w_master, W, static_cast<bf16 *>(w_fwd), (w_dgrad && de) ? static_cast<bf16 *>(w_dgrad) : nullptr);
        PCB_LAUNCH_CHECK();
        const SpPlan S = sp_plan(c);
        if (S.ok) {
            PCB_CHECK(w_dgrad != nullptr, "sub-pixel weights need the dgrad operand buffer");
            return sp_weight_prepare(c, S, L, w_master, static_cast<bf16 *>(w_fwd) + static_cast<size_t>(L.rows_f) * L.kf,
                                     static_cast<bf16 *>(w_dgrad) + static_cast<size_t>(rup(L.ktap, 128)) * L.kd, st);
        }
        return 0;
    }
    const long long total = static_cast<long long>(c->cout) * W.taps * c->cin;
    const int grid = static_cast<int>(std::min<long long>((total + 1023) / 1024, 8ll * pcb_num_sms()));
    tc_weight_prepare_kernel<<<grid < 1 ? 1 : grid, 256, 0, st>>>(w_master, W, static_cast<bf16 *>(w_fwd),
                                                                   (w_dgrad && de) ? static_cast<bf16 *>(w_dgrad) : nullptr);
    PCB_LAUNCH_CHECK();
    if (stem_ok(c)) return pcb_stem_weight_prepare(c, w_master, static_cast<bf16 *>(w_fwd) + stem_base(L), zero_padding, st);
    if (smallco_ok(c) && pcb_k2r_ok(c)) {
        PCB_CHECK(w_dgrad != nullptr, "kernel-to-row weights need the dgrad operand buffer");
        size_t fb, db;
        k2r_bases(L, &fb, &db);
        return pcb_k2r_weight_prepare(c, w_master, static_cast<bf16 *>(w_fwd) + fb, static_cast<bf16 *>(w_dgrad) + db, zero_padding, st);
    }
    const SpPlan S = sp_plan(c);
    if (S.ok) {
        PCB_CHECK(w_dgrad != nullptr, "sub-pixel weights need the dgrad operand buffer");
        return sp_weight_prepare(c, S, L, w_master, static_cast<bf16 *>(w_fwd) + static_cast<size_t>(L.rows_f) * L.kf,
                                 static_cast<bf16 *>(w_dgrad) + static_cast<size_t>(rup(L.ktap, 128)) * L.kd, st);
    }
    return 0;
}

int pcb_tc_forward_mask_pass(const pcb_conv *c, uint64_t *tapmask, cudaStream_t st) {
    const long long m_total = static_cast<long long>(c->n) * c->ho * c->wo;
    PCB_CHECK(m_total < (1ll << 31), "problem too large");
    const Layout L = layout_of(c);
    if (smallco_ok(c) || stem_ok(c)) return 0;
    { const SpPlan S = sp_plan(c); if (S.ok && S.fwd) return 0; }
    bool any_mask = false;
    for (int p = 0; p < c->nparts; ++p) any_mask = any_mask || (c->parts[p].mask != nullptr);
    if (tma_fwd_ok(c) && !any_mask) return 0;
    if (tma_fwd_ok(c)) {
        int bw, bh, bn;
        tile_box(c->wo, c->ho, &bw, &bh, &bn);
        if (tma_halo_ok(c, bw, bh, bn, pick_bn(c->cout <= 32 ? 32 : L.rows_f, m_total))) return 0;
    }
    return launch_tapmask(c, tapmask, st);
}

bool pcb_tc_fuses_bn_stats(const pcb_conv *c) {
    return pcb_tc_fuses_affine_act(c) && !getenv("PCB_DISABLE_FUSED_BN_STATS");
}

bool pcb_tc_fuses_affine_act(const pcb_conv *c) {
    return pcb_tc_eligible(c) && !smallco_ok(c) && !getenv("PCB_SPLITK");
}

int pcb_tc_forward_ws(const pcb_conv *c, const void *w_fwd, const float *bias, void *y, int y_cstride, const float *msum,
                      uint64_t *tapmask, bool mask_pass_done, double *bn_sums, const pcb_ep *ep, cudaStream_t st) {
    int *flag = abort_flag_ptr();
    PCB_CHECK(flag != nullptr, "cudaMalloc(abort flag) failed");
    const long long m_total = static_cast<long long>(c->n) * c->ho * c->wo;
    PCB_CHECK(m_total < (1ll << 31), "problem too large");
    PCB_CHECK(y_cstride % 8 == 0 && y_cstride >= c->cout, "tensor-core forward: y channel stride must be a multiple of 8 and >= cout");
    const Layout L = layout_of(c);
    if (!mask_pass_done)
        if (int rc = pcb_tc_forward_mask_pass(c, tapmask, st)) return rc;
    if (stem_ok(c)) {
        PCB_CHECK(bn_sums == nullptr || pcb_tc_fuses_bn_stats(c), "fused BatchNorm statistics requested from a kernel that does not produce them");
        PCB_CHECK(ep == nullptr || pcb_tc_fuses_affine_act(c), "fused BatchNorm + activation requested from a kernel that does not apply it");
        return pcb_stem_forward(c, static_cast<const bf16 *>(w_fwd) + stem_base(L), bias, y, y_cstride, msum, tapmask, bn_sums, ep, st);
    }
    if (smallco_ok(c)) {
        PCB_CHECK(ep == nullptr, "fused BatchNorm + activation requested from a small-Cout kernel that does not apply it");
        if (pcb_k2r_ok(c)) {
            size_t fb, db;
            k2r_bases(L, &fb, &db);
            return pcb_k2r_forward(c, smallco_layout(L), w_fwd, static_cast<const bf16 *>(w_fwd) + fb, bias, y, y_cstride, msum, tapmask, st);
        }
        return pcb_smallco_forward(c, smallco_layout(L), w_fwd, bias, y, y_cstride, msum, st);
    }
    {
        const SpPlan S = sp_plan(c);
        if (S.ok && S.fwd) {
            PCB_CHECK(bn_sums == nullptr || pcb_tc_fuses_bn_stats(c), "fused BatchNorm statistics requested from a kernel that does not produce them");
            return sp_forward(c, S, L, static_cast<const bf16 *>(w_fwd) + static_cast<size_t>(L.rows_f) * L.kf, bias, y, y_cstride, msum, bn_sums, ep, flag, st);
        }
    }
    TcParams P;
    base_params(P, c, L);
    P.m_total = static_cast<int>(m_total);
    fill_parts(c, L, P.parts, tapmask, m_total);
    P.bias = bias; P.msum = msum; P.y = static_cast<bf16 *>(y); P.y_cstride = y_cstride; P.abort_flag = flag;
    PCB_CHECK(bn_sums == nullptr || pcb_tc_fuses_bn_stats(c), "fused BatchNorm statistics requested from a kernel that does not produce them");
    P.bn_sums = bn_sums; P.bn_c = c->cout;
    PCB_CHECK(ep == nullptr || pcb_tc_fuses_affine_act(c), "fused BatchNorm + activation requested from a kernel that does not apply it");
    set_ep(P, ep);
    P.ncols = L.rows_f;
    CUtensorMap tm;
    if (tma_fwd_ok(c)) {
        tile_box(c->wo, c->ho, &P.box_w, &P.box_h, &P.box_n);
        const int bn = pick_bn(c->cout <= 32 ? 32 : L.rows_f, m_total);
        const bool halo = tma_halo_ok(c, P.box_w, P.box_h, P.box_n, bn);
        const int hx = halo ? (c->kw - 1) * c->dil : 0;
        CUtensorMap ta[TC_MAX_PARTS];
        memset(ta, 0, sizeof(ta));
        uint8_t *extra = reinterpret_cast<uint8_t *>(tapmask) + tapmask_bytes(c);
        for (int p = 0; p < c->nparts; ++p) {
            const pcb_part &pt = c->parts[p];
            const void *src = pt.x;
            long long cs = pt.x_cstride;
            const int c8 = rup(pt.c, 8);
            if (pt.x_up) {
                const long long pix = static_cast<long long>(c->n) * (c->h >> 1) * (c->w >> 1);
                const long long work = pix * (c8 >> 3);
                const int grid = static_cast<int>(std::min<long long>((work + 255) / 256, 16ll * pcb_num_sms()));
                upsample_part_kernel<<<grid, 256, 0, st>>>(static_cast<const bf16 *>(pt.x), pt.x_cstride, c8, pix, c->h >> 1, c->w >> 1, reinterpret_cast<bf16 *>(extra));
                PCB_LAUNCH_CHECK();
                src = extra; cs = c8;
                extra += up_bytes(c, p);
            }
            if (pt.mask) P.use_fix = 1;
            if (int rc = make_tmap_nhwc(&ta[p], src, c8, c->w, c->h, c->n, cs, P.box_w + hx, P.box_h, P.box_n, c->stride)) return rc;
        }
        if (c->nparts < 2) ta[1] = ta[0];
        P.ncols = (c->cout <= 32) ? 32 : L.rows_f;
        P.wk_base = 0; P.wk_col = L.ktap; P.wk_row = c->kw * L.ktap;
        if (int rc = make_tmap_2d(&tm, w_fwd, L.rows_f, L.kf, L.kf, bn)) return rc;
        P.ksplit = pick_ksplit(m_total, P.ncols, bn, L.ktap / BLOCK_K);
        if (P.ksplit > 1) {
            PCB_CHECK(!P.ep_on, "split-K forward: the finish kernel does not apply a fused BatchNorm + activation");
            const size_t bytes = static_cast<size_t>(m_total) * P.ncols * sizeof(float);
            P.partial = splitk_scratch(bytes);
            PCB_CHECK(P.partial != nullptr, "split-K scratch allocation failed");
            PCB_CUDA(cudaMemsetAsync(P.partial, 0, bytes, st));
            if (int rc = launch_tma<0>(P, tm, ta[0], ta[1], bn, halo, st)) return rc;
            const long long work = m_total * (y_cstride / 8);
            splitk_finish_fwd_kernel<<<static_cast<int>(std::min<long long>((work + 255) / 256, 8ll * pcb_num_sms())), 256, 0, st>>>(
                P.partial, P.ncols, msum, bias, c->cout, c->no_guard, m_total, static_cast<bf16 *>(y), y_cstride);
            PCB_LAUNCH_CHECK();
            return 0;
        }
        return launch_tma<0>(P, tm, ta[0], ta[1], bn, halo, st);
    }
    if (int rc = make_tmap_2d(&tm, w_fwd, L.rows_f, L.kf, L.kf, L.bn_f)) return rc;
    P.hg = halo_hg(c, L.rowpack);
    return launch_tc<0>(P, tm, L.bn_f, st);
}

bool pcb_tc_dgrad_supported(const pcb_conv *c) { return pcb_tc_eligible(c) && !is_rowpack(c); }

int pcb_tc_dgrad(const pcb_conv *c, const void *dc, int dc_cstride, const void *w_dgrad, void *const *dx, const int *dx_cstride,
                 cudaStream_t st) {
    int *flag = abort_flag_ptr();
    PCB_CHECK(flag != nullptr, "cudaMalloc(abort flag) failed");
    const long long m_total = static_cast<long long>(c->n) * c->h * c->w;
    PCB_CHECK(m_total < (1ll << 31), "problem too large");
    PCB_CHECK(dc_cstride % 8 == 0 && dc_cstride >= rup(c->cout, 8), "tensor-core dgrad: dc channel stride must be a multiple of 8");
    const Layout L = layout_of(c);
    if (smallco_ok(c)) {
        if (pcb_k2r_ok(c)) {
            size_t fb, db;
            k2r_bases(L, &fb, &db);
            return pcb_k2r_dgrad(c, smallco_layout(L), dc, dc_cstride, w_dgrad, static_cast<const bf16 *>(w_dgrad) + db, dx, dx_cstride, st);
        }
        return pcb_smallco_dgrad(c, smallco_layout(L), dc, dc_cstride, w_dgrad, dx, dx_cstride, st);
    }
    const SpPlan SPL = sp_plan(c);
    void *dx_local[TC_MAX_PARTS] = {nullptr, nullptr};
    for (int p = 0; p < c->nparts && p < TC_MAX_PARTS; ++p) dx_local[p] = dx[p];
    if (SPL.ok && SPL.dgrad) {
        if (dx[SPL.pu] != nullptr)
            if (int rc = sp_dgrad_up(c, SPL, L, dc, dc_cstride, static_cast<const bf16 *>(w_dgrad) + static_cast<size_t>(rup(L.ktap, 128)) * L.kd,
                                     dx[SPL.pu], dx_cstride[SPL.pu], flag, st)) return rc;
        dx_local[SPL.pu] = nullptr;
        if (SPL.ps < 0 || dx[SPL.ps] == nullptr) return 0;
    }
    dx = dx_local;
    TcParams P;
    base_params(P, c, L);
    P.m_total = static_cast<int>(m_total);
    fill_parts(c, L, P.parts, nullptr, 0);
    for (int p = 0; p < c->nparts; ++p) {
        P.parts[p].dx = static_cast<bf16 *>(dx[p]);
        P.parts[p].dx_cstride = dx_cstride[p];
        PCB_CHECK(!dx[p] || (dx_cstride[p] % 8 == 0 && dx_cstride[p] >= P.parts[p].c8 && (reinterpret_cast<uintptr_t>(dx[p]) & 15) == 0),
                  "tensor-core dgrad: dx[%d] must be 16-byte aligned with a channel stride that is a multiple of 8", p);
    }
    P.dc = static_cast<const bf16 *>(dc); P.dc_cstride = dc_cstride; P.dc_c8 = rup(c->cout, 8); P.dc_kext = L.cout64;
    P.abort_flag = flag;
    int bn = (L.ktap % 128 == 0) ? 128 : 64;
    P.ncols = L.ktap;
    CUtensorMap tm;
    if (tma_dgrad_ok(c)) {
        tile_box(c->w, c->h, &P.box_w, &P.box_h, &P.box_n);
        bn = pick_bn(L.ktap, m_total);
        const bool halo = tma_halo_ok(c, P.box_w, P.box_h, P.box_n, bn);
        P.wk_base = 0; P.wk_col = L.cout64; P.wk_row = c->kw * L.cout64;
        CUtensorMap ta;
        if (int rc = make_tmap_nhwc(&ta, dc, P.dc_c8, c->wo, c->ho, c->n, dc_cstride, P.box_w + (halo ? (c->kw - 1) * c->dil : 0), P.box_h, P.box_n, 1)) return rc;
        if (int rc = make_tmap_2d(&tm, w_dgrad, rup(L.ktap, 128), L.kd, L.kd, bn)) return rc;
        P.ksplit = pick_ksplit(m_total, P.ncols, bn, L.cout64 / BLOCK_K);
        if (P.ksplit > 1) {
            const size_t bytes = static_cast<size_t>(m_total) * P.ncols * sizeof(float);
            P.partial = splitk_scratch(bytes);
            PCB_CHECK(P.partial != nullptr, "split-K scratch allocation failed");
            PCB_CUDA(cudaMemsetAsync(P.partial, 0, bytes, st));
            if (int rc = launch_tma<1>(P, tm, ta, ta, bn, halo, st)) return rc;
            const long long work = m_total * (P.ncols / 8);
            splitk_finish_dgrad_kernel<<<static_cast<int>(std::min<long long>((work + 255) / 256, 8ll * pcb_num_sms())), 256, 0, st>>>(P.partial, P);
            PCB_LAUNCH_CHECK();
            return 0;
        }
        return launch_tma<1>(P, tm, ta, ta, bn, halo, st);
    }
    if (tma_dgrad_s2_ok(c)) {
        const int hh = c->h / 2, hw = c->w / 2;
        const long long m_class = static_cast<long long>(c->n) * hh * hw;
        tile_box(hw, hh, &P.box_w, &P.box_h, &P.box_n);
        bn = pick_bn(L.ktap, m_class);
        if (int rc = make_tmap_2d(&tm, w_dgrad, rup(L.ktap, 128), L.kd, L.kd, bn)) return rc;
        const long long class_tiles = ((m_class + BLOCK_M - 1) / BLOCK_M) * (L.ktap / bn);
        const bool fork = class_tiles < pcb_num_sms() && !getenv("PCB_DISABLE_CLASS_STREAMS");
        struct ClassStreams { cudaStream_t aux[3]; cudaEvent_t ev_fork, ev_join[3]; bool ready; };
        static thread_local ClassStreams cs_all[PCB_MAX_DEVICES] = {};
        ClassStreams &CS = cs_all[pcb_cur_device()];
        cudaStream_t *aux = CS.aux;
        cudaEvent_t *ev_join = CS.ev_join;
        if (fork && !CS.ready) {
            for (int i = 0; i < 3; ++i) {
                PCB_CUDA(cudaStreamCreateWithFlags(&aux[i], cudaStreamNonBlocking));
                PCB_CUDA(cudaEventCreateWithFlags(&ev_join[i], cudaEventDisableTiming));
            }
            PCB_CUDA(cudaEventCreateWithFlags(&CS.ev_fork, cudaEventDisableTiming));
            CS.ready = true;
        }
        cudaEvent_t ev_fork = CS.ev_fork;
        if (fork) PCB_CUDA(cudaEventRecord(ev_fork, st));
        for (int cls = 0; cls < 4; ++cls) {
            TcParams Q = P;
            const int py = cls >> 1, px = cls & 1;
            const int tr0 = (py + c->pad_h) & 1, tc0 = (px + c->pad_w) & 1;
            Q.kh = (c->kh - tr0 + 1) / 2; Q.kw = (c->kw - tc0 + 1) / 2;
            Q.pad_h = (py + c->pad_h - tr0) / 2; Q.pad_w = (px + c->pad_w - tc0) / 2;
            Q.h = hh; Q.w = hw; Q.stride = 1; Q.dil = 1;
            Q.m_total = static_cast<int>(m_class);
            Q.sub = 2; Q.py = py; Q.px = px; Q.fh = c->h; Q.fw = c->w;
            Q.wk_base = (tr0 * c->kw + tc0) * L.cout64; Q.wk_row = 2 * c->kw * L.cout64; Q.wk_col = 2 * L.cout64;
            const bool halo = !getenv("PCB_DISABLE_TMA_HALO") && Q.box_w == 128 && Q.box_h == 1 && Q.box_n == 1 && Q.kw >= 2 &&
                              halo_stages_fit(Q.kw, 1, bn);
            CUtensorMap ta;
            if (int rc = make_tmap_nhwc(&ta, dc, P.dc_c8, c->wo, c->ho, c->n, dc_cstride, Q.box_w + (halo ? Q.kw - 1 : 0), Q.box_h, Q.box_n, 1)) return rc;
            cudaStream_t cs = (fork && cls > 0) ? aux[cls - 1] : st;
            if (fork && cls > 0) PCB_CUDA(cudaStreamWaitEvent(cs, ev_fork, 0));
            if (int rc = launch_tma<1>(Q, tm, ta, ta, bn, halo, cs)) return rc;
            if (fork && cls > 0) {
                PCB_CUDA(cudaEventRecord(ev_join[cls - 1], cs));
                PCB_CUDA(cudaStreamWaitEvent(st, ev_join[cls - 1], 0));
            }
        }
        return 0;
    }
    if (int rc = make_tmap_2d(&tm, w_dgrad, rup(L.ktap, 128), L.kd, L.kd, bn)) return rc;
    P.hg = halo_hg(c, L.rowpack);
    return launch_tc<1>(P, tm, bn, st);
}


static bool kblock_box(int wt, int ht, int *bw, int *bh, int *bn) {
    if (wt < 4) return false;
    if (wt % 64 == 0) { *bw = 64; *bh = 1; *bn = 1; return true; }
    if (64 % wt) return false;
    const int rows = 64 / wt;
    *bw = wt;
    if (ht % rows == 0) { *bh = rows; *bn = 1; return true; }
    if (rows % ht) return false;
    *bh = ht; *bn = rows / ht;
    return true;
}

static bool tma_wgrad_ok(const pcb_conv *c) {
    if (getenv("PCB_DISABLE_TMA") || getenv("PCB_DISABLE_TMA_WGRAD") || is_rowpack(c) || c->stride > 2) return false;
    int bw, bh, bn;
    if (!kblock_box(c->wo, c->ho, &bw, &bh, &bn)) return false;
    for (int p = 0; p < c->nparts; ++p)
        if (c->parts[p].x_up && ((c->h | c->w) & 1)) return false;
    return true;
}

template <int BLOCK_N, int T, bool HALO>
int launch_wgrad_tma(WgParams &P, const CUtensorMap &tdc, const CUtensorMap &ta0, const CUtensorMap &ta1, cudaStream_t st) {
    const int rows_a = 64 + (HALO ? (P.kw - 1) * P.dil : 0);
    PCB_CHECK(rows_a <= (HALO ? 3 : 1) * WGRAD_FIX_THREADS, "TMA-fed wgrad: %d-row A blocks exceed the fixer warps", rows_a);
    const size_t a_blk = (static_cast<size_t>(rows_a) * 128 + 1023) / 1024 * 1024;
    const size_t stage = (HALO ? 1 : T) * 2 * a_blk + static_cast<size_t>(BLOCK_N) * 128;
    P.stages = static_cast<int>(std::min<size_t>(MAX_RING, RING_BUDGET / stage));
    PCB_CHECK(P.stages >= 2, "TMA-fed wgrad: stage of %zu bytes does not fit twice", stage);
    const size_t smem = 1024 + P.stages * stage + 24 * MAX_RING;
    auto kern = pconv_tc_wgrad_tma_kernel<BLOCK_N, T, HALO>;
    PCB_SMEM_OPT_IN(kern, MAX_SMEM);
    P.tap_groups = HALO ? P.kh : (P.kh * P.kw + T - 1) / T;
    P.ci_tiles = (P.ktap + 127) / 128;
    const int co_tiles = (P.cout + BLOCK_N - 1) / BLOCK_N;
    const int base_ctas = co_tiles * P.tap_groups * P.ci_tiles;
    const int total_kb = (P.m_total + 63) / 64;
    int splits = (2 * pcb_num_sms() + base_ctas - 1) / base_ctas;
    splits = std::max(1, std::min(splits, total_kb));
    splits = std::min(splits, 65535);
    P.kb_per_split = (total_kb + splits - 1) / splits;
    splits = (total_kb + P.kb_per_split - 1) / P.kb_per_split;
    dim3 grid(base_ctas, splits);
    kern<<<grid, WGRAD_TMA_THREADS, smem, st>>>(P, tdc, ta0, ta1);
    PCB_LAUNCH_CHECK();
    return 0;
}

template <int BLOCK_N, int T, int STAGES>
static int launch_wgrad(WgParams &P, const CUtensorMap &tm, int cout, cudaStream_t st) {
    constexpr size_t smem = 1024 + STAGES * (T * 16384 + BLOCK_N * 128) + 24 * STAGES;
    auto kern = pconv_tc_wgrad_kernel<BLOCK_N, T, STAGES>;
    PCB_SMEM_OPT_IN(kern, (int)smem);
    P.tap_groups = (P.ntaps + T - 1) / T;
    P.ci_tiles = (P.ktap + 127) / 128;
    const int co_tiles = (cout + BLOCK_N - 1) / BLOCK_N;
    const int base_ctas = co_tiles * P.tap_groups * P.ci_tiles;
    const int total_kb = (P.m_total + 63) / 64;
    int splits = (4 * pcb_num_sms() + base_ctas - 1) / base_ctas;
    splits = std::max(1, std::min(splits, total_kb));
    splits = std::min(splits, 65535);
    P.kb_per_split = (total_kb + splits - 1) / splits;
    splits = (total_kb + P.kb_per_split - 1) / P.kb_per_split;
    dim3 grid(base_ctas, splits);
    kern<<<grid, WGRAD_THREADS, smem, st>>>(P, tm);
    PCB_LAUNCH_CHECK();
    return 0;
}

int pcb_tc_wgrad(const pcb_conv *c, const void *dc, int dc_cstride, float *dw, void *workspace, bool zero_dw, cudaStream_t st) {
    int *flag = abort_flag_ptr();
    PCB_CHECK(flag != nullptr, "cudaMalloc(abort flag) failed");
    PCB_CHECK(workspace != nullptr, "pcb_tc_wgrad: workspace required");
    const long long m_total = static_cast<long long>(c->n) * c->ho * c->wo;
    PCB_CHECK(m_total < (1ll << 31), "problem too large");
    PCB_CHECK(dc_cstride % 8 == 0 && dc_cstride >= c->cout, "tensor-core wgrad: dc channel stride must be a multiple of 8");
    if (stem_ok(c)) return pcb_stem_wgrad(c, dc, dc_cstride, dw, workspace, zero_dw, st);
    if (smallco_ok(c)) {
        if (pcb_k2r_ok(c)) return pcb_k2r_wgrad(c, dc, dc_cstride, dw, workspace, zero_dw, st);
        return pcb_smallco_wgrad(c, smallco_layout(layout_of(c)), dc, dc_cstride, dw, zero_dw, st);
    }
    uint64_t *tapmask = static_cast<uint64_t *>(workspace);
    bool any_mask = false;
    for (int p = 0; p < c->nparts; ++p) any_mask = any_mask || (c->parts[p].mask != nullptr);
    if (any_mask || !tma_wgrad_ok(c))
        if (int rc = launch_tapmask(c, tapmask, st)) return rc;
    const size_t dw_bytes = sizeof(float) * c->cout * c->kh * c->kw * c->cin;
    if (zero_dw) PCB_CUDA(cudaMemsetAsync(dw, 0, dw_bytes, st));
    const Layout L = layout_of(c);
    WgParams P;
    memset(&P, 0, sizeof(P));
    P.n = c->n; P.h = c->h; P.w = c->w; P.cin = c->cin; P.cout = c->cout; P.kh = c->kh; P.kw = c->kw; P.stride = c->stride;
    P.pad_h = c->pad_h; P.pad_w = c->pad_w; P.dil = c->dil; P.ho = c->ho; P.wo = c->wo; P.m_total = static_cast<int>(m_total);
    P.nparts = c->nparts; P.rowpack = L.rowpack; P.ktap = L.ktap; P.ntaps = L.rowpack ? c->kh : c->kh * c->kw;
    fill_parts(c, L, P.parts, tapmask, m_total);
    P.dw = dw; P.abort_flag = flag;
    CUtensorMap tm;
    if (int rc = make_tmap_2d(&tm, dc, m_total, c->cout, dc_cstride, 64)) return rc;
    if (tma_wgrad_ok(c)) {
        kblock_box(c->wo, c->ho, &P.box_w, &P.box_h, &P.box_n);
        const bool halo = !getenv("PCB_DISABLE_TMA_HALO") && c->stride == 1 && c->kw == 3 && P.box_w == 64 &&
                          P.box_h == 1 && P.box_n == 1 && 64 + (c->kw - 1) * c->dil <= 256;
        const int hx = halo ? (c->kw - 1) * c->dil : 0;
        CUtensorMap ta[TC_MAX_PARTS];
        memset(ta, 0, sizeof(ta));
// ... 37 lines not shown
```

### text_segmentation_image_inpainting_b200/csrc/pcb_ptx.cuh

```cuda
#pragma once
#include <cuda.h>
#include <cuda_runtime.h>
#include <stdint.h>

namespace ptx {

__device__ __forceinline__ uint32_t smem_u32(const void *p) { return static_cast<uint32_t>(__cvta_generic_to_shared(p)); }

__device__ __forceinline__ bool elect_one() {
    uint32_t pred = 0;
    asm volatile(
        "{\n\t.reg .pred P;\n\telect.sync _|P, 0xffffffff;\n\tselp.b32 %0, 1, 0, P;\n\t}" : "=r"(pred));
    return pred != 0;
}

__device__ __forceinline__ void mbar_init(uint32_t bar, uint32_t count) {
    asm volatile("mbarrier.init.shared::cta.b64 [%0], %1;" ::"r"(bar), "r"(count) : "memory");
}
__device__ __forceinline__ void fence_mbar_init() { asm volatile("fence.mbarrier_init.release.cluster;" ::: "memory"); }
__device__ __forceinline__ void mbar_arrive(uint32_t bar) {
    asm volatile("mbarrier.arrive.shared::cta.b64 _, [%0];" ::"r"(bar) : "memory");
}
__device__ __forceinline__ void mbar_arrive_expect_tx(uint32_t bar, uint32_t bytes) {
    asm volatile("mbarrier.arrive.expect_tx.shared::cta.b64 _, [%0], %1;" ::"r"(bar), "r"(bytes) : "memory");
}
__device__ __forceinline__ bool mbar_try_wait(uint32_t bar, uint32_t parity) {
    uint32_t ok;
    asm volatile(
        "{\n\t.reg .pred P;\n\t"
        "mbarrier.try_wait.parity.shared::cta.b64 P, [%1], %2;\n\t"
        "selp.b32 %0, 1, 0, P;\n\t}"
        : "=r"(ok)
        : "r"(bar), "r"(parity)
        : "memory");
    return ok != 0;
}
__device__ __forceinline__ bool mbar_wait(uint32_t bar, uint32_t parity, int *abort_flag, int code) {
    if (mbar_try_wait(bar, parity)) return true;
    const long long t0 = clock64();
    for (uint32_t it = 1;; ++it) {
        if (mbar_try_wait(bar, parity)) return true;
        if ((it & 63) == 0) {
            if (*reinterpret_cast<volatile int *>(abort_flag) != 0) return false;
            if (clock64() - t0 > 4000000000ll) break;
        }
    }
    atomicCAS(abort_flag, 0, code);
    return false;
}
__device__ __forceinline__ void cp_async_mbar_arrive(uint32_t bar) {
    asm volatile("cp.async.mbarrier.arrive.shared::cta.b64 [%0];" ::"r"(bar) : "memory");
}

__device__ __forceinline__ void cp_async_16(uint32_t dst, const void *src, bool valid) {
    const uint32_t sz = valid ? 16u : 0u;
    asm volatile("cp.async.cg.shared.global [%0], [%1], 16, %2;" ::"r"(dst), "l"(src), "r"(sz) : "memory");
}
__device__ __forceinline__ void cp_async_commit() { asm volatile("cp.async.commit_group;" ::: "memory"); }
template <int N> __device__ __forceinline__ void cp_async_wait() { asm volatile("cp.async.wait_group %0;" ::"n"(N) : "memory"); }

__device__ __forceinline__ void fence_proxy_async_smem() { asm volatile("fence.proxy.async.shared::cta;" ::: "memory"); }

__device__ __forceinline__ void prefetch_tmap(const CUtensorMap *m) {
    asm volatile("prefetch.tensormap [%0];" ::"l"(reinterpret_cast<uint64_t>(m)) : "memory");
}
__device__ __forceinline__ void tma_load_2d(uint32_t dst, const CUtensorMap *m, int c0, int c1, uint32_t bar) {
    asm volatile(
        "cp.async.bulk.tensor.2d.shared::cluster.global.mbarrier::complete_tx::bytes [%0], [%1, {%3, %4}], [%2];"
        ::"r"(dst), "l"(reinterpret_cast<uint64_t>(m)), "r"(bar), "r"(c0), "r"(c1)
        : "memory");
}
__device__ __forceinline__ void tma_prefetch_4d(const CUtensorMap *m, int c0, int c1, int c2, int c3) {
    asm volatile("cp.async.bulk.prefetch.tensor.4d.L2.global.tile [%0, {%1, %2, %3, %4}];"
                 ::"l"(reinterpret_cast<uint64_t>(m)), "r"(c0), "r"(c1), "r"(c2), "r"(c3)
                 : "memory");
}
__device__ __forceinline__ void tma_load_4d(uint32_t dst, const CUtensorMap *m, int c0, int c1, int c2, int c3, uint32_t bar) {
    asm volatile(
        "cp.async.bulk.tensor.4d.shared::cluster.global.mbarrier::complete_tx::bytes [%0], [%1, {%3, %4, %5, %6}], [%2];"
        ::"r"(dst), "l"(reinterpret_cast<uint64_t>(m)), "r"(bar), "r"(c0), "r"(c1), "r"(c2), "r"(c3)
        : "memory");
}

__device__ __forceinline__ void wgmma_fence() { asm volatile("wgmma.fence.sync.aligned;" ::: "memory"); }
__device__ __forceinline__ void wgmma_commit() { asm volatile("wgmma.commit_group.sync.aligned;" ::: "memory"); }
template <int N> __device__ __forceinline__ void wgmma_wait() { asm volatile("wgmma.wait_group.sync.aligned %0;" ::"n"(N) : "memory"); }
template <int R> __device__ __forceinline__ void wgmma_fence_regs(float (&d)[R]) {
#pragma unroll
    for (int i = 0; i < R; ++i) asm volatile("" : "+f"(d[i])::"memory");
}
template <int TA, int TB> __device__ __forceinline__ void wgmma_m64n32(float (&d)[16], uint64_t a_desc, uint64_t b_desc) {
    asm volatile(
        "{\n\t"
        "wgmma.mma_async.sync.aligned.m64n32k16.f32.bf16.bf16 "
        "{%0, %1, %2, %3, %4, %5, %6, %7, %8, %9, %10, %11, %12, %13, %14, %15}, %16, %17, 1, 1, 1, %18, %19;\n\t"
        "}"
        : "+f"(d[0]), "+f"(d[1]), "+f"(d[2]), "+f"(d[3]), "+f"(d[4]), "+f"(d[5]), "+f"(d[6]), "+f"(d[7]), "+f"(d[8]), "+f"(d[9]), "+f"(d[10]), "+f"(d[11]), "+f"(d[12]), "+f"(d[13]), "+f"(d[14]), "+f"(d[15])
        : "l"(a_desc), "l"(b_desc), "n"(TA), "n"(TB));
}
template <int TA, int TB, int R> __device__ __forceinline__ void wgmma_m64n64(float (&d)[R], uint64_t a_desc, uint64_t b_desc) {
    static_assert(R >= 32, "m64n64 accumulator");
    asm volatile(
        "{\n\t"
        "wgmma.mma_async.sync.aligned.m64n64k16.f32.bf16.bf16 "
        "{%0, %1, %2, %3, %4, %5, %6, %7, %8, %9, %10, %11, %12, %13, %14, %15, %16, %17, %18, %19, %20, %21, %22, %23, %24, %25, %26, %27, %28, %29, %30, %31}, %32, %33, 1, 1, 1, %34, %35;\n\t"
        "}"
        : "+f"(d[0]), "+f"(d[1]), "+f"(d[2]), "+f"(d[3]), "+f"(d[4]), "+f"(d[5]), "+f"(d[6]), "+f"(d[7]), "+f"(d[8]), "+f"(d[9]), "+f"(d[10]), "+f"(d[11]), "+f"(d[12]), "+f"(d[13]), "+f"(d[14]), "+f"(d[15]), "+f"(d[16]), "+f"(d[17]), "+f"(d[18]), "+f"(d[19]), "+f"(d[20]), "+f"(d[21]), "+f"(d[22]), "+f"(d[23]), "+f"(d[24]), "+f"(d[25]), "+f"(d[26]), "+f"(d[27]), "+f"(d[28]), "+f"(d[29]), "+f"(d[30]), "+f"(d[31])
        : "l"(a_desc), "l"(b_desc), "n"(TA), "n"(TB));
}
template <int TA, int TB> __device__ __forceinline__ void wgmma_m64n128(float (&d)[64], uint64_t a_desc, uint64_t b_desc) {
    asm volatile(
        "{\n\t"
        "wgmma.mma_async.sync.aligned.m64n128k16.f32.bf16.bf16 "
        "{%0, %1, %2, %3, %4, %5, %6, %7, %8, %9, %10, %11, %12, %13, %14, %15, %16, %17, %18, %19, %20, %21, %22, %23, %24, %25, %26, %27, %28, %29, %30, %31, %32, %33, %34, %35, %36, %37, %38, %39, %40, %41, %42, %43, %44, %45, %46, %47, %48, %49, %50, %51, %52, %53, %54, %55, %56, %57, %58, %59, %60, %61, %62, %63}, %64, %65, 1, 1, 1, %66, %67;\n\t"
        "}"
        : "+f"(d[0]), "+f"(d[1]), "+f"(d[2]), "+f"(d[3]), "+f"(d[4]), "+f"(d[5]), "+f"(d[6]), "+f"(d[7]), "+f"(d[8]), "+f"(d[9]), "+f"(d[10]), "+f"(d[11]), "+f"(d[12]), "+f"(d[13]), "+f"(d[14]), "+f"(d[15]), "+f"(d[16]), "+f"(d[17]), "+f"(d[18]), "+f"(d[19]), "+f"(d[20]), "+f"(d[21]), "+f"(d[22]), "+f"(d[23]), "+f"(d[24]), "+f"(d[25]), "+f"(d[26]), "+f"(d[27]), "+f"(d[28]), "+f"(d[29]), "+f"(d[30]), "+f"(d[31]), "+f"(d[32]), "+f"(d[33]), "+f"(d[34]), "+f"(d[35]), "+f"(d[36]), "+f"(d[37]), "+f"(d[38]), "+f"(d[39]), "+f"(d[40]), "+f"(d[41]), "+f"(d[42]), "+f"(d[43]), "+f"(d[44]), "+f"(d[45]), "+f"(d[46]), "+f"(d[47]), "+f"(d[48]), "+f"(d[49]), "+f"(d[50]), "+f"(d[51]), "+f"(d[52]), "+f"(d[53]), "+f"(d[54]), "+f"(d[55]), "+f"(d[56]), "+f"(d[57]), "+f"(d[58]), "+f"(d[59]), "+f"(d[60]), "+f"(d[61]), "+f"(d[62]), "+f"(d[63])
        : "l"(a_desc), "l"(b_desc), "n"(TA), "n"(TB));
}
template <int N, int TA, int TB> __device__ __forceinline__ void wgmma_bf16(float (&d)[N / 2], uint64_t a_desc, uint64_t b_desc) {
    if constexpr (N == 32) wgmma_m64n32<TA, TB>(d, a_desc, b_desc);
    else if constexpr (N == 64) wgmma_m64n64<TA, TB>(d, a_desc, b_desc);
    else { static_assert(N == 128, "wgmma tile width"); wgmma_m64n128<TA, TB>(d, a_desc, b_desc); }
}
template <int N> __device__ __forceinline__ void setmaxnreg_inc() { asm volatile("setmaxnreg.inc.sync.aligned.u32 %0;" ::"n"(N)); }
template <int N> __device__ __forceinline__ void setmaxnreg_dec() { asm volatile("setmaxnreg.dec.sync.aligned.u32 %0;" ::"n"(N)); }
__device__ __forceinline__ void named_sync(int id, int threads) { asm volatile("bar.sync %0, %1;" ::"r"(id), "r"(threads) : "memory"); }

__host__ __device__ __forceinline__ uint64_t make_smem_desc(uint32_t smem_addr, uint32_t lbo_bytes, uint32_t sbo_bytes) {
    uint64_t d = 0;
    d |= static_cast<uint64_t>((smem_addr >> 4) & 0x3FFFu);
    d |= static_cast<uint64_t>((lbo_bytes >> 4) & 0x3FFFu) << 16;
    d |= static_cast<uint64_t>((sbo_bytes >> 4) & 0x3FFFu) << 32;
    d |= 1ull << 62;
    return d;
}
__host__ __device__ __forceinline__ uint64_t make_smem_desc_noswizzle(uint32_t smem_addr, uint32_t lbo_bytes, uint32_t sbo_bytes) {
    uint64_t d = 0;
    d |= static_cast<uint64_t>((smem_addr >> 4) & 0x3FFFu);
    d |= static_cast<uint64_t>((lbo_bytes >> 4) & 0x3FFFu) << 16;
    d |= static_cast<uint64_t>((sbo_bytes >> 4) & 0x3FFFu) << 32;
    return d;
}

}
```

Baseline: 919.1.

## Add 256-wide TMA conv tiles with bf16 staging and register rebalancing

```diff
diff --git a/text_segmentation_image_inpainting_b200/csrc/conv_tc.cu b/text_segmentation_image_inpainting_b200/csrc/conv_tc.cu
--- a/text_segmentation_image_inpainting_b200/csrc/conv_tc.cu
+++ b/text_segmentation_image_inpainting_b200/csrc/conv_tc.cu
@@ -57,7 +57,29 @@
 constexpr int STAT_SLICE = 256;
 constexpr int STAT_SMEM_BYTES = MMA_WARPS * STAT_SLICE * 4 + 16;
 constexpr int EPI_WARPS = 4;
-constexpr int EPI_STAT_SMEM_BYTES = EPI_WARPS * STAT_SLICE * 4;
+constexpr int EPI_STAT_SLICE = 512;
+constexpr int EPI_STAT_SQ = EPI_STAT_SLICE / 2;
+constexpr int EPI_STAT_SMEM_BYTES = EPI_WARPS * EPI_STAT_SLICE * 4;
+constexpr int bf16_pitch(int block_n) { return block_n + 8; }
+constexpr int bf16_stage_bytes(int block_n) { return BLOCK_M * bf16_pitch(block_n) * 2; }
+
+__device__ __forceinline__ float warp_transpose_sum16(float (&v)[16], int lane) {
+#pragma unroll
+    for (int i = 0; i < 16; ++i) v[i] += __shfl_xor_sync(0xffffffffu, v[i], 16);
+#pragma unroll
+    for (int off = 8, n = 16; off >= 1; off >>= 1, n >>= 1) {
+        const bool upper = (lane & off) != 0;
+#pragma unroll
+        for (int i = 0; i < 8; ++i) {
+            if (i < (n >> 1)) {
+                const float send = upper ? v[i] : v[i + (n >> 1)];
+                const float keep = upper ? v[i + (n >> 1)] : v[i];
+                v[i] = keep + __shfl_xor_sync(0xffffffffu, send, off);
+            }
+        }
+    }
+    return v[0];
+}
 
 __device__ __forceinline__ float warp_transpose_sum(float (&v)[32], int lane) {
 #pragma unroll
@@ -94,7 +116,7 @@
 };
 
 template <int MODE>
-__device__ __forceinline__ EpiRow tc_epi_row(const TcParams &P, int m) {
+__device__ __forceinline__ EpiRow tc_epi_row(const TcParams &P, int m, bool renorm = true) {
     EpiRow er;
     er.m = m;
     er.rvalid = m < P.m_total;
@@ -111,7 +133,7 @@
         en = m / (P.ho * P.wo); const int rem = m - en * P.ho * P.wo; eh = rem / P.wo; ew = rem - eh * P.wo;
         er.mo = (static_cast<long long>(en) * P.fh + eh * P.sub + P.py) * P.fw + ew * P.sub + P.px;
     }
-    if (MODE == 0 && er.rvalid) {
+    if (MODE == 0 && er.rvalid && renorm) {
         const float s = P.msum ? P.msum[er.mo] : 1.f;
         er.hole = (s == 0.f) && !P.no_guard;
         er.inv = er.hole ? 0.f : 1.0f / s;
@@ -284,7 +306,7 @@
         if (co < P.bn_c) {
             float a = 0.f, q = 0.f;
 #pragma unroll
-            for (int w4 = 0; w4 < EPI_WARPS; ++w4) { a += stat_base[w4 * STAT_SLICE + col]; q += stat_base[w4 * STAT_SLICE + 128 + col]; }
+            for (int w4 = 0; w4 < EPI_WARPS; ++w4) { a += stat_base[w4 * EPI_STAT_SLICE + col]; q += stat_base[w4 * EPI_STAT_SLICE + EPI_STAT_SQ + col]; }
             atomicAdd(P.bn_sums + co, static_cast<double>(a));
             atomicAdd(P.bn_sums + P.bn_c + co, static_cast<double>(q));
         }
@@ -666,19 +688,94 @@
 }
 
 
-constexpr int EPI_WARP0 = MMA_WARPS + 5;
+constexpr int EPI_WARP0 = MMA_WARPS + 4;
 constexpr int TMA_THREADS = (EPI_WARP0 + EPI_WARPS) * 32;
+constexpr int TMA_FIX_THREADS = 96;
+constexpr int TMA_REGS = 128;
+constexpr int TMA_CONSUMER_REGS = 192, TMA_SUPPORT_REGS = 64;
+static_assert(TMA_THREADS == 512 && 2 * 128 * TMA_CONSUMER_REGS + 2 * 128 * TMA_SUPPORT_REGS == TMA_THREADS * TMA_REGS &&
+              TMA_THREADS * TMA_REGS <= 65536, "TMA-fed fwd / dgrad register budget");
 
 constexpr size_t TMA_BAR_BYTES = 24 * MAX_RING + 16;
+
+template <int BLOCK_N, int MODE>
+__device__ __forceinline__ void tc_epilogue_bf16(const TcParams &P, const EpiRow &er, const bf16 *srow, int lane, int n0, float *s_stat) {
+    const bool stats = (MODE == 0) && (s_stat != nullptr);
+#pragma unroll 1
+    for (int c0 = 0; c0 < BLOCK_N; c0 += 32) {
+        const int col = n0 + c0;
+        bf16 *orow = nullptr;
+        int nstore = 0;
+        float scale = 1.f;
+        if (MODE == 0) {
+            if (er.rvalid && col < P.y_cstride) { orow = P.y + er.mo * P.y_cstride + col; nstore = min(32, P.y_cstride - col); }
+        } else {
+#pragma unroll
+            for (int p = 0; p < TC_MAX_PARTS; ++p) {
+                if (p >= P.nparts) break;
+                const TcPart &pt = P.parts[p];
+                const int local = col - pt.koff;
+                if (local >= 0 && local < pt.kext && pt.dx != nullptr && local < pt.c8 && er.rvalid) {
+                    orow = pt.dx + er.mo * pt.dx_cstride + local;
+                    nstore = min(32, pt.c8 - local);
+                    scale = er.dscale[p];
+                }
+            }
+        }
+        if (nstore == 0 && !stats) continue;
+        uint4 o[4];
+#pragma unroll
+        for (int j = 0; j < 4; ++j) o[j] = reinterpret_cast<const uint4 *>(srow + c0)[j];
+        if (MODE == 1 && scale != 1.f) {
+            __nv_bfloat162 *ob = reinterpret_cast<__nv_bfloat162 *>(o);
+#pragma unroll
+            for (int j = 0; j < 16; ++j) {
+                const float2 f = __bfloat1622float2(ob[j]);
+                ob[j] = __floats2bfloat162_rn(f.x * scale, f.y * scale);
+            }
+        }
+        if (nstore > 0) {
+            uint4 *dst = reinterpret_cast<uint4 *>(orow);
+#pragma unroll
+            for (int j = 0; j < 4; ++j)
+                if (j * 8 < nstore) dst[j] = o[j];
+        }
+        if (stats) {
+            const float live = er.rvalid ? 1.f : 0.f;
+            const __nv_bfloat162 *ob = reinterpret_cast<const __nv_bfloat162 *>(o);
+            float cs = 0.f, cq = 0.f;
+#pragma unroll
+            for (int h = 0; h < 2; ++h) {
+                float v[16];
+#pragma unroll
+                for (int j = 0; j < 8; ++j) {
+                    const float2 f = __bfloat1622float2(ob[8 * h + j]);
+                    v[2 * j] = f.x * live; v[2 * j + 1] = f.y * live;
+                }
+                const float s = warp_transpose_sum16(v, lane);
+#pragma unroll
+                for (int j = 0; j < 8; ++j) {
+                    const float2 f = __bfloat1622float2(ob[8 * h + j]);
+                    const float a = f.x * live, b = f.y * live;
+                    v[2 * j] = a * a; v[2 * j + 1] = b * b;
+                }
+                const float q = warp_transpose_sum16(v, lane);
+                if ((lane >> 4) == h) { cs = s; cq = q; }
+            }
+            s_stat[c0 + lane] += cs;
+            s_stat[EPI_STAT_SQ + c0 + lane] += cq;
+        }
+    }
+}
 
 template <int BLOCK_N, int MODE, typename TileFn>
 __device__ __forceinline__ void tma_epilogue_warps(const TcParams &P, int tile0, int tstep, int num_tiles, TileFn tile_origin,
-                                                   const float *acc_stage, uint32_t acc_full, uint32_t acc_empty, float *s_stat,
+                                                   const uint8_t *stage, uint32_t acc_full, uint32_t acc_empty, float *s_stat,
                                                    int &stat_n0, int w, int lane, int code) {
-    constexpr int PITCH = acc_pitch(BLOCK_N);
-    const float *acc_row = acc_stage + (w * 32 + lane) * PITCH;
+    const int row = w * 32 + lane;
+    const bool f32 = P.partial != nullptr;
     if (s_stat) {
-        for (int i = lane; i < STAT_SLICE; i += 32) s_stat[i] = 0.f;
+        for (int i = lane; i < EPI_STAT_SLICE; i += 32) s_stat[i] = 0.f;
         __syncwarp();
     }
     uint32_t ph = 0;
@@ -687,31 +784,93 @@
         tile_origin(tile, m0, n0);
         if (n0 < 0) continue;
         if (s_stat && n0 != stat_n0) {
-            if (stat_n0 >= 0) tc_stats_flush<BLOCK_N>(P, s_stat, lane, stat_n0, 0, BLOCK_N, 128);
+            if (stat_n0 >= 0) tc_stats_flush<BLOCK_N>(P, s_stat, lane, stat_n0, 0, BLOCK_N, EPI_STAT_SQ);
             stat_n0 = n0;
         }
-        const EpiRow er = tc_epi_row<MODE>(P, m0 + w * 32 + lane);
+        const EpiRow er = tc_epi_row<MODE>(P, m0 + row, false);
         if (!__all_sync(0xffffffffu, ptx::mbar_wait(acc_full, ph, P.abort_flag, code))) { stat_n0 = -1; return; }
         ph ^= 1;
-        tc_epilogue<BLOCK_N, MODE>(P, er, acc_row, lane, n0, s_stat, 0, BLOCK_N, 128);
+        if constexpr (BLOCK_N <= 128) {
+            if (f32) tc_epilogue<BLOCK_N, MODE>(P, er, reinterpret_cast<const float *>(stage) + row * acc_pitch(BLOCK_N), lane, n0, s_stat, 0, BLOCK_N, EPI_STAT_SQ);
+        }
+        if (!f32) tc_epilogue_bf16<BLOCK_N, MODE>(P, er, reinterpret_cast<const bf16 *>(stage) + row * bf16_pitch(BLOCK_N), lane, n0, s_stat);
         __syncwarp();
         if (lane == 0) ptx::mbar_arrive(acc_empty);
     }
 }
 
-template <int BLOCK_N>
-__device__ __forceinline__ bool tma_stage_tile(const TcParams &P, const float (&acc)[BLOCK_N / 2], float *acc_stage, uint32_t acc_full,
-                                               uint32_t acc_empty, uint32_t &ph, int e, int lane, int code) {
+struct ConsRows {
+    float inv[2];
+    bool hole[2];
+};
+template <int MODE>
+__device__ __forceinline__ ConsRows cons_rows(const TcParams &P, int m0, int e, int lane) {
+    ConsRows cr;
+#pragma unroll
+    for (int h = 0; h < 2; ++h) {
+        cr.inv[h] = 0.f; cr.hole[h] = false;
+        if (MODE == 0 && P.partial == nullptr) {
+            const EpiRow er = tc_epi_row<0>(P, m0 + 64 * (e >> 2) + 16 * (e & 3) + (lane >> 2) + 8 * h);
+            cr.inv[h] = er.inv; cr.hole[h] = er.hole;
+        }
+    }
+    return cr;
+}
+
+template <int BLOCK_N, int MODE>
+__device__ __forceinline__ void stage_acc_bf16(const TcParams &P, const float (&acc)[BLOCK_N / 2], bf16 *stage, int e, int lane, int n0,
+                                               const ConsRows &cr) {
+    constexpr int PITCH = bf16_pitch(BLOCK_N);
+    const int r0 = 64 * (e >> 2) + 16 * (e & 3) + (lane >> 2), c0 = 2 * (lane & 3);
+    const bool has_bias = (MODE == 0) && (P.bias != nullptr);
+    const bool ep = (MODE == 0) && (P.ep_on != 0);
+    const bool ep_aff = ep && (P.ep_scale != nullptr);
+#pragma unroll
+    for (int j = 0; j < BLOCK_N / 8; ++j) {
+        const int col = n0 + 8 * j + c0;
+        float b0 = 0.f, b1 = 0.f, s0 = 1.f, s1 = 1.f, t0 = 0.f, t1 = 0.f;
+        if (MODE == 0) {
+            const bool in0 = col < P.cout, in1 = col + 1 < P.cout;
+            if (has_bias) { if (in0) b0 = __ldg(P.bias + col); if (in1) b1 = __ldg(P.bias + col + 1); }
+            if (ep_aff) {
+                if (in0) { s0 = __ldg(P.ep_scale + col); t0 = __ldg(P.ep_shift + col); }
+                if (in1) { s1 = __ldg(P.ep_scale + col + 1); t1 = __ldg(P.ep_shift + col + 1); }
+            }
+        }
+#pragma unroll
+        for (int h = 0; h < 2; ++h) {
+            float a = acc[4 * j + 2 * h], b = acc[4 * j + 2 * h + 1];
+            if (MODE == 0) {
+                a = cr.hole[h] ? 0.f : fmaf(a, cr.inv[h], b0);
+                b = cr.hole[h] ? 0.f : fmaf(b, cr.inv[h], b1);
+                if (ep) {
+                    a = apply_act(fmaf(a, s0, t0), P.ep_act, P.ep_slope);
+                    b = apply_act(fmaf(b, s1, t1), P.ep_act, P.ep_slope);
+                }
+                if (col >= P.cout) a = 0.f;
+                if (col + 1 >= P.cout) b = 0.f;
+            }
+            *reinterpret_cast<__nv_bfloat162 *>(stage + (r0 + 8 * h) * PITCH + 8 * j + c0) = __floats2bfloat162_rn(a, b);
+        }
+    }
+}
+
+template <int BLOCK_N, int MODE>
+__device__ __forceinline__ bool tma_stage_tile(const TcParams &P, const float (&acc)[BLOCK_N / 2], uint8_t *stage, uint32_t acc_full,
+                                               uint32_t acc_empty, uint32_t &ph, int e, int lane, int n0, const ConsRows &cr, int code) {
     if (!__all_sync(0xffffffffu, ptx::mbar_wait(acc_empty, ph, P.abort_flag, code))) return false;
     ph ^= 1;
-    stage_acc<BLOCK_N>(acc, acc_stage, e, lane);
+    if constexpr (BLOCK_N <= 128) {
+        if (P.partial != nullptr) stage_acc<BLOCK_N>(acc, reinterpret_cast<float *>(stage), e, lane);
+    }
+    if (P.partial == nullptr) stage_acc_bf16<BLOCK_N, MODE>(P, acc, reinterpret_cast<bf16 *>(stage), e, lane, n0, cr);
     __syncwarp();
     if (lane == 0) ptx::mbar_arrive(acc_full);
     return true;
 }
 
 template <int BLOCK_N, int MODE, bool HALO>
-__global__ void __launch_bounds__(TMA_THREADS, 1)
+__global__ void __maxnreg__(TMA_REGS)
 pconv_tc_tma_kernel(const __grid_constant__ TcParams P, const __grid_constant__ CUtensorMap tmap_w,
                     const __grid_constant__ CUtensorMap tmap_a0, const __grid_constant__ CUtensorMap tmap_a1) {
     constexpr uint32_t B_BYTES = BLOCK_N * 128;
@@ -751,7 +910,7 @@
 
     if (threadIdx.x == 0) {
         for (int s = 0; s < MAX_RING; ++s) {
-            ptx::mbar_init(bar_full + 8 * s, 1); ptx::mbar_init(bar_fixed + 8 * s, 4); ptx::mbar_init(bar_empty + 8 * s, 2);
+            ptx::mbar_init(bar_full + 8 * s, 1); ptx::mbar_init(bar_fixed + 8 * s, TMA_FIX_THREADS / 32); ptx::mbar_init(bar_empty + 8 * s, 2);
         }
         ptx::mbar_init(acc_full, MMA_WARPS); ptx::mbar_init(acc_empty, EPI_WARPS);
         ptx::fence_mbar_init();
@@ -761,73 +920,9 @@
 
     float *s_stat = nullptr;
     int stat_n0 = -1;
-    float *acc_stage = reinterpret_cast<float *>(smem_gen + (s_acc - smem_base));
-    if (warp >= EPI_WARP0) {
-        const int w = warp - EPI_WARP0;
-        s_stat = (MODE == 0 && P.bn_sums != nullptr && P.partial == nullptr)
-                     ? reinterpret_cast<float *>(smem_gen + (s_stat_addr - smem_base)) + w * STAT_SLICE : nullptr;
-        auto origin = [&](int tile, int &m0, int &n0) {
-            const int mn = tile / KS;
-            m0 = m0_of(mn / n_tiles); n0 = (mn % n_tiles) * BLOCK_N;
-            if (!tile_active(n0)) n0 = -1;
-        };
-        tma_epilogue_warps<BLOCK_N, MODE>(P, tile0, tstep, num_tiles, origin, acc_stage, acc_full, acc_empty, s_stat, stat_n0, w, lane, 126);
-    } else if (warp == 8) {
-        int s = 0;
-        uint32_t ph = 1;
-        const int plane = (MODE == 0) ? P.ho * P.wo : P.h * P.w;
-        const int pwid = (MODE == 0) ? P.wo : P.w;
-        const int kext0 = (MODE == 0) ? P.parts[0].kext : P.dc_kext, kext1 = (MODE == 0 && np > 1) ? P.parts[1].kext : 0;
-        const int dstep = (MODE == 0) ? P.dil : -P.dil;
-        const int row_k = P.wk_row, col_k = P.wk_col;
-        bool dead = false;
-        for (int tile = tile0; tile < num_tiles && !dead; tile += tstep) {
-            const int sp = tile % KS, mn = tile / KS;
-            const int m0 = m0_of(mn / n_tiles), n0 = (mn % n_tiles) * BLOCK_N;
-            if (!tile_active(n0)) continue;
-            const int img = m0 / plane, rem = m0 - img * plane;
-            const int oy = rem / pwid, ox = rem - oy * pwid;
-            const int x_org = (MODE == 0) ? ox * P.stride - P.pad_w : (HALO ? ox + P.pad_w - hx : ox + P.pad_w);
-            const int y_org = (MODE == 0) ? oy * P.stride - P.pad_h : oy + P.pad_h;
-            int nx_org = 0, ny_org = 0, nimg = -1;
-            if (P.l2pf && tile + tstep < num_tiles) {
-                const int nmn = (tile + tstep) / KS;
-                const int nm0 = m0_of(nmn / n_tiles);
-                if (nm0 != m0) {
-                    nimg = nm0 / plane;
-                    const int nrem = nm0 - nimg * plane, noy = nrem / pwid, nox = nrem - noy * pwid;
-                    nx_org = (MODE == 0) ? nox * P.stride - P.pad_w : (HALO ? nox + P.pad_w - hx : nox + P.pad_w);
-                    ny_org = (MODE == 0) ? noy * P.stride - P.pad_h : noy + P.pad_h;
-                }
-            }
-            int krow = P.wk_base;
-            for (int tr = 0, y = y_org; tr < P.kh && !dead; ++tr, y += dstep, krow += row_k)
-                for (int ti = 0, x = x_org, kidx = krow; ti < kwi && !dead; ++ti, x += dstep, kidx = krow + ti * col_k) {
-#pragma unroll
-                    for (int p = 0; p < TC_MAX_PARTS; ++p) {
-                        const int kext = (p == 0) ? kext0 : kext1;
-                        const CUtensorMap *ma = (p == 0) ? &tmap_a0 : &tmap_a1;
-                        const int gb0 = (p == 0) ? 0 : kext0 / BLOCK_K;
-                        for (int c0 = 0; c0 < kext; c0 += BLOCK_K, kidx += BLOCK_K) {
-                            if (KS > 1 && (gb0 + c0 / BLOCK_K) % KS != sp) continue;
-                            if (!__all_sync(0xffffffffu, ptx::mbar_wait(bar_empty + 8 * s, ph, P.abort_flag, 121))) { dead = true; break; }
-                            if (ptx::elect_one()) {
-                                const uint32_t full = bar_full + 8 * s, dst = smem_base + s * STAGE;
-                                ptx::mbar_arrive_expect_tx(full, STAGE_TX);
-                                ptx::tma_load_4d(dst, ma, c0, x, y, img, full);
-                                uint32_t bdst = dst + A_ROOM;
-                                for (int tc = 0, kb = kidx; tc < nB; ++tc, kb += col_k, bdst += B_BYTES)
-                                    ptx::tma_load_2d(bdst, &tmap_w, kb, n0, full);
-                                if (nimg >= 0) ptx::tma_prefetch_4d(ma, c0, nx_org + ti * dstep, ny_org + tr * dstep, nimg);
-                            }
-                            __syncwarp();
-                            if (++s == S) { s = 0; ph ^= 1; }
-                        }
-                        if (dead) break;
-                    }
-                }
-        }
-    } else if (warp < MMA_WARPS) {
+    uint8_t *acc_stage = smem_gen + (s_acc - smem_base);
+    if (warp < MMA_WARPS) {
+        ptx::setmaxnreg_inc<TMA_CONSUMER_REGS>();
         const int e = warp, g = warp >> 2;
         const bool leader = (threadIdx.x & 127) == 0;
         const uint32_t ready = fix ? bar_fixed : bar_full;
@@ -850,6 +945,7 @@
             const int sp = tile % KS, mn = tile / KS;
             const int n0 = (mn % n_tiles) * BLOCK_N;
             if (!tile_active(n0)) continue;
+            const ConsRows cr = cons_rows<MODE>(P, m0_of(mn / n_tiles), e, lane);
             float acc[BLOCK_N / 2];
             zero_acc(acc);
             int held = -1;
@@ -885,120 +981,204 @@
             ptx::wgmma_fence_regs(acc);
             if (held >= 0 && leader) ptx::mbar_arrive(bar_empty + 8 * held);
             if (dead) break;
-            if (!tma_stage_tile<BLOCK_N>(P, acc, acc_stage, acc_full, acc_empty, aph, e, lane, 125)) break;
-        }
-    } else if (warp > 8) {
-        if (fix) {
-            const int t = (warp - 9) * 32 + lane;
+            if (!tma_stage_tile<BLOCK_N, MODE>(P, acc, acc_stage, acc_full, acc_empty, aph, e, lane, n0, cr, 125)) break;
+        }
+    } else {
+        ptx::setmaxnreg_dec<TMA_SUPPORT_REGS>();
+        if (warp >= EPI_WARP0) {
+            const int w = warp - EPI_WARP0;
+            s_stat = (MODE == 0 && P.bn_sums != nullptr && P.partial == nullptr)
+                         ? reinterpret_cast<float *>(smem_gen + (s_stat_addr - smem_base)) + w * EPI_STAT_SLICE : nullptr;
+            auto origin = [&](int tile, int &m0, int &n0) {
+                const int mn = tile / KS;
+                m0 = m0_of(mn / n_tiles); n0 = (mn % n_tiles) * BLOCK_N;
+                if (!tile_active(n0)) n0 = -1;
+            };
+            tma_epilogue_warps<BLOCK_N, MODE>(P, tile0, tstep, num_tiles, origin, acc_stage, acc_full, acc_empty, s_stat, stat_n0, w, lane, 126);
+            ptx::named_sync(1, EPI_WARPS * 32);
+            if (s_stat != nullptr && stat_n0 >= 0) tc_stats_final<BLOCK_N>(P, s_stat - w * EPI_STAT_SLICE, w, lane, stat_n0);
+        } else if (warp == 8) {
             int s = 0;
-            uint32_t ph = 0;
+            uint32_t ph = 1;
+            const int plane = (MODE == 0) ? P.ho * P.wo : P.h * P.w;
+            const int pwid = (MODE == 0) ? P.wo : P.w;
+            const int kext0 = (MODE == 0) ? P.parts[0].kext : P.dc_kext, kext1 = (MODE == 0 && np > 1) ? P.parts[1].kext : 0;
+            const int dstep = (MODE == 0) ? P.dil : -P.dil;
+            const int row_k = P.wk_row, col_k = P.wk_col;
             bool dead = false;
-            if (!HALO) {
-                uint64_t wnext[TC_MAX_PARTS];
-                auto load_words = [&](int tl) {
-#pragma unroll
-                    for (int p = 0; p < TC_MAX_PARTS; ++p) {
-                        wnext[p] = 0ull;
-                        const int m = m0_of(tl / KS / n_tiles) + t;
-                        if (fix && p < P.nparts && tl < num_tiles && m < P.m_total) wnext[p] = __ldg(P.parts[p].tapmask + m);
+            for (int tile = tile0; tile < num_tiles && !dead; tile += tstep) {
+                const int sp = tile % KS, mn = tile / KS;
+                const int m0 = m0_of(mn / n_tiles), n0 = (mn % n_tiles) * BLOCK_N;
+                if (!tile_active(n0)) continue;
+                const int img = m0 / plane, rem = m0 - img * plane;
+                const int oy = rem / pwid, ox = rem - oy * pwid;
+                const int x_org = (MODE == 0) ? ox * P.stride - P.pad_w : (HALO ? ox + P.pad_w - hx : ox + P.pad_w);
+                const int y_org = (MODE == 0) ? oy * P.stride - P.pad_h : oy + P.pad_h;
+                int nx_org = 0, ny_org = 0, nimg = -1;
+                if (P.l2pf && tile + tstep < num_tiles) {
+                    const int nmn = (tile + tstep) / KS;
+                    const int nm0 = m0_of(nmn / n_tiles);
+                    if (nm0 != m0) {
+                        nimg = nm0 / plane;
+                        const int nrem = nm0 - nimg * plane, noy = nrem / pwid, nox = nrem - noy * pwid;
+                        nx_org = (MODE == 0) ? nox * P.stride - P.pad_w : (HALO ? nox + P.pad_w - hx : nox + P.pad_w);
+                        ny_org = (MODE == 0) ? noy * P.stride - P.pad_h : noy + P.pad_h;
                     }
-                };
-                load_words(tile0);
-                for (int tile = tile0; tile < num_tiles && !dead; tile += tstep) {
-                    const int sp = tile % KS;
-                    uint64_t wcur[TC_MAX_PARTS];
-#pragma unroll
-                    for (int p = 0; p < TC_MAX_PARTS; ++p) wcur[p] = wnext[p];
-                    load_words(tile + tstep);
-                    if (MODE == 1 && !tile_active(((tile / KS) % n_tiles) * BLOCK_N)) continue;
-                    const int taps = P.kh * P.kw;
-                    for (int tap = 0; tap < taps && !dead; ++tap) {
+                }
+                int krow = P.wk_base;
+                for (int tr = 0, y = y_org; tr < P.kh && !dead; ++tr, y += dstep, krow += row_k)
+                    for (int ti = 0, x = x_org, kidx = krow; ti < kwi && !dead; ++ti, x += dstep, kidx = krow + ti * col_k) {
 #pragma unroll
                         for (int p = 0; p < TC_MAX_PARTS; ++p) {
-                            if (p >= np) break;
-                            const bool hole = fix && ((wcur[p] >> tap) & 1ull) == 0ull;
-                            const bool any_hole = __any_sync(0xffffffffu, hole);
-                            const int nb = ((MODE == 0) ? P.parts[p].kext : P.dc_kext) / BLOCK_K;
-                            const int gb0 = (p == 0) ? 0 : P.parts[0].kext / BLOCK_K;
-                            for (int cb = 0; cb < nb; ++cb) {
-                                if (KS > 1 && (gb0 + cb) % KS != sp) continue;
-                                if (!ptx::mbar_wait(bar_full + 8 * s, ph, P.abort_flag, 122)) { dead = true; break; }
-                                if (any_hole) {
-                                    if (hole) {
-                                        uint4 *r = reinterpret_cast<uint4 *>(smem_gen + s * STAGE + t * 128);
-                                        const uint4 z = make_uint4(0u, 0u, 0u, 0u);
-#pragma unroll
-                                        for (int k = 0; k < 8; ++k) r[k] = z;
-                                    }
-                                    ptx::fence_proxy_async_smem();
+                            const int kext = (p == 0) ? kext0 : kext1;
+                            const CUtensorMap *ma = (p == 0) ? &tmap_a0 : &tmap_a1;
+                            const int gb0 = (p == 0) ? 0 : kext0 / BLOCK_K;
+                            for (int c0 = 0; c0 < kext; c0 += BLOCK_K, kidx += BLOCK_K) {
+                                if (KS > 1 && (gb0 + c0 / BLOCK_K) % KS != sp) continue;
+                                if (!__all_sync(0xffffffffu, ptx::mbar_wait(bar_empty + 8 * s, ph, P.abort_flag, 121))) { dead = true; break; }
+                                if (ptx::elect_one()) {
+                                    const uint32_t full = bar_full + 8 * s, dst = smem_base + s * STAGE;
+                                    ptx::mbar_arrive_expect_tx(full, STAGE_TX);
+                                    ptx::tma_load_4d(dst, ma, c0, x, y, img, full);
+                                    uint32_t bdst = dst + A_ROOM;
+                                    for (int tc = 0, kb = kidx; tc < nB; ++tc, kb += col_k, bdst += B_BYTES)
+                                        ptx::tma_load_2d(bdst, &tmap_w, kb, n0, full);
+                                    if (nimg >= 0) ptx::tma_prefetch_4d(ma, c0, nx_org + ti * dstep, ny_org + tr * dstep, nimg);
                                 }
                                 __syncwarp();
-                                if (lane == 0) ptx::mbar_arrive(bar_fixed + 8 * s);
                                 if (++s == S) { s = 0; ph ^= 1; }
                             }
                             if (dead) break;
                         }
                     }
-                }
-            } else {
-                const int plane = P.ho * P.wo;
-                auto load_bits = [&](int tl, uint32_t &b0, uint32_t &b1) {
-                    b0 = b1 = 0;
-                    if (!fix || tl >= num_tiles) return;
-                    const int m0 = m0_of(tl / KS / n_tiles);
-                    const int img = m0 / plane, rem = m0 - img * plane;
-                    const int oy = rem / P.wo, ox = rem - oy * P.wo;
-#pragma unroll
-                    for (int p = 0; p < TC_MAX_PARTS; ++p) {
-                        if (p >= P.nparts || P.parts[p].mask == nullptr) continue;
-                        const int mup = P.parts[p].mup;
-                        const uint8_t *mk = P.parts[p].mask + static_cast<long long>(img) * (P.h >> mup) * (P.w >> mup);
-                        for (int tr = 0; tr < P.kh; ++tr) {
-                            const int y = oy - P.pad_h + tr * P.dil;
-                            if (y < 0 || y >= P.h) continue;
-                            const int x0 = ox - P.pad_w + t, x1 = x0 + 128;
-                            if (x0 >= 0 && x0 < P.w && __ldg(mk + (y >> mup) * (P.w >> mup) + (x0 >> mup)) == 0) b0 |= 1u << (p * 8 + tr);
-                            if (t < hx && x1 < P.w && __ldg(mk + (y >> mup) * (P.w >> mup) + (x1 >> mup)) == 0) b1 |= 1u << (p * 8 + tr);
+            }
+        } else {
+            if (fix) {
+                constexpr int FR = HALO ? 3 : 2;
+                const int t = (warp - 9) * 32 + lane;
+                int s = 0;
+                uint32_t ph = 0;
+                bool dead = false;
+                auto zero_row = [&](int row) {
+                    uint4 *r = reinterpret_cast<uint4 *>(smem_gen + s * STAGE + row * 128);
+                    const uint4 z = make_uint4(0u, 0u, 0u, 0u);
+#pragma unroll
+                    for (int k = 0; k < 8; ++k) r[k] = z;
+                };
+                if (!HALO) {
+                    uint64_t wnext[FR][TC_MAX_PARTS];
+                    auto load_words = [&](int tl) {
+#pragma unroll
+                        for (int r = 0; r < FR; ++r)
+#pragma unroll
+                            for (int p = 0; p < TC_MAX_PARTS; ++p) {
+                                wnext[r][p] = 0ull;
+                                const int m = m0_of(tl / KS / n_tiles) + t + TMA_FIX_THREADS * r;
+                                if (p < P.nparts && tl < num_tiles && t + TMA_FIX_THREADS * r < BLOCK_M && m < P.m_total)
+                                    wnext[r][p] = __ldg(P.parts[p].tapmask + m);
+                            }
+                    };
+                    load_words(tile0);
+                    for (int tile = tile0; tile < num_tiles && !dead; tile += tstep) {
+                        const int sp = tile % KS;
+                        uint64_t wcur[FR][TC_MAX_PARTS];
+#pragma unroll
+                        for (int r = 0; r < FR; ++r)
+#pragma unroll
+                            for (int p = 0; p < TC_MAX_PARTS; ++p) wcur[r][p] = wnext[r][p];
+                        load_words(tile + tstep);
+                        if (MODE == 1 && !tile_active(((tile / KS) % n_tiles) * BLOCK_N)) continue;
+                        const int taps = P.kh * P.kw;
+                        for (int tap = 0; tap < taps && !dead; ++tap) {
+#pragma unroll
+                            for (int p = 0; p < TC_MAX_PARTS; ++p) {
+                                if (p >= np) break;
+                                bool hole[FR], mine = false;
+#pragma unroll
+                                for (int r = 0; r < FR; ++r) {
+                                    hole[r] = t + TMA_FIX_THREADS * r < BLOCK_M && ((wcur[r][p] >> tap) & 1ull) == 0ull;
+                                    mine = mine || hole[r];
+                                }
+                                const bool any_hole = __any_sync(0xffffffffu, mine);
+                                const int nb = ((MODE == 0) ? P.parts[p].kext : P.dc_kext) / BLOCK_K;
+                                const int gb0 = (p == 0) ? 0 : P.parts[0].kext / BLOCK_K;
+                                for (int cb = 0; cb < nb; ++cb) {
+                                    if (KS > 1 && (gb0 + cb) % KS != sp) continue;
+                                    if (!ptx::mbar_wait(bar_full + 8 * s, ph, P.abort_flag, 122)) { dead = true; break; }
+                                    if (any_hole) {
+#pragma unroll
+                                        for (int r = 0; r < FR; ++r)
+                                            if (hole[r]) zero_row(t + TMA_FIX_THREADS * r);
+                                        ptx::fence_proxy_async_smem();
+                                    }
+                                    __syncwarp();
+                                    if (lane == 0) ptx::mbar_arrive(bar_fixed + 8 * s);
+                                    if (++s == S) { s = 0; ph ^= 1; }
+                                }
+                                if (dead) break;
+                            }
                         }
                     }
-                };
-                uint32_t n0b, n1b;
-                load_bits(tile0, n0b, n1b);
-                for (int tile = tile0; tile < num_tiles && !dead; tile += tstep) {
-                    const int sp = tile % KS;
-                    const uint32_t c0b = n0b, c1b = n1b;
-                    load_bits(tile + tstep, n0b, n1b);
-                    if (MODE == 1 && !tile_active(((tile / KS) % n_tiles) * BLOCK_N)) continue;
-                    for (int tr = 0; tr < P.kh && !dead; ++tr) {
+                } else {
+                    const int plane = P.ho * P.wo;
+                    auto load_bits = [&](int tl, uint32_t (&b)[FR]) {
+#pragma unroll
+                        for (int r = 0; r < FR; ++r) b[r] = 0;
+                        if (tl >= num_tiles) return;
+                        const int m0 = m0_of(tl / KS / n_tiles);
+                        const int img = m0 / plane, rem = m0 - img * plane;
+                        const int oy = rem / P.wo, ox = rem - oy * P.wo;
 #pragma unroll
                         for (int p = 0; p < TC_MAX_PARTS; ++p) {
-                            if (p >= np) break;
-                            const bool h0 = (c0b >> (p * 8 + tr)) & 1u, h1 = (c1b >> (p * 8 + tr)) & 1u;
-                            const bool any_hole = __any_sync(0xffffffffu, h0 || h1);
-                            const int nb = ((MODE == 0) ? P.parts[p].kext : P.dc_kext) / BLOCK_K;
-                            const int gb0 = (p == 0) ? 0 : P.parts[0].kext / BLOCK_K;
-                            for (int cb = 0; cb < nb; ++cb) {
-                                if (KS > 1 && (gb0 + cb) % KS != sp) continue;
-                                if (!ptx::mbar_wait(bar_full + 8 * s, ph, P.abort_flag, 122)) { dead = true; break; }
-                                if (any_hole) {
-                                    const uint4 z = make_uint4(0u, 0u, 0u, 0u);
-                                    if (h0) {
-                                        uint4 *r = reinterpret_cast<uint4 *>(smem_gen + s * STAGE + t * 128);
-#pragma unroll
-                                        for (int k = 0; k < 8; ++k) r[k] = z;
+                            if (p >= P.nparts || P.parts[p].mask == nullptr) continue;
+                            const int mup = P.parts[p].mup;
+                            const uint8_t *mk = P.parts[p].mask + static_cast<long long>(img) * (P.h >> mup) * (P.w >> mup);
+                            for (int tr = 0; tr < P.kh; ++tr) {
+                                const int y = oy - P.pad_h + tr * P.dil;
+                                if (y < 0 || y >= P.h) continue;
+#pragma unroll
+                                for (int r = 0; r < FR; ++r) {
+                                    const int row = t + TMA_FIX_THREADS * r, x = ox - P.pad_w + row;
+                                    if (row < BLOCK_M + hx && x >= 0 && x < P.w && __ldg(mk + (y >> mup) * (P.w >> mup) + (x >> mup)) == 0)
+                                        b[r] |= 1u << (p * 8 + tr);
+                                }
+                            }
+                        }
+                    };
+                    uint32_t nb_bits[FR];
+                    load_bits(tile0, nb_bits);
+                    for (int tile = tile0; tile < num_tiles && !dead; tile += tstep) {
+                        const int sp = tile % KS;
+                        uint32_t cb_bits[FR];
+#pragma unroll
+                        for (int r = 0; r < FR; ++r) cb_bits[r] = nb_bits[r];
+                        load_bits(tile + tstep, nb_bits);
+                        if (MODE == 1 && !tile_active(((tile / KS) % n_tiles) * BLOCK_N)) continue;
+                        for (int tr = 0; tr < P.kh && !dead; ++tr) {
+#pragma unroll
+                            for (int p = 0; p < TC_MAX_PARTS; ++p) {
+                                if (p >= np) break;
+                                bool hole[FR], mine = false;
+#pragma unroll
+                                for (int r = 0; r < FR; ++r) { hole[r] = (cb_bits[r] >> (p * 8 + tr)) & 1u; mine = mine || hole[r]; }
+                                const bool any_hole = __any_sync(0xffffffffu, mine);
+                                const int nb = ((MODE == 0) ? P.parts[p].kext : P.dc_kext) / BLOCK_K;
+                                const int gb0 = (p == 0) ? 0 : P.parts[0].kext / BLOCK_K;
+                                for (int cb = 0; cb < nb; ++cb) {
+                                    if (KS > 1 && (gb0 + cb) % KS != sp) continue;
+                                    if (!ptx::mbar_wait(bar_full + 8 * s, ph, P.abort_flag, 122)) { dead = true; break; }
+                                    if (any_hole) {
+#pragma unroll
+                                        for (int r = 0; r < FR; ++r)
+                                            if (hole[r]) zero_row(t + TMA_FIX_THREADS * r);
+                                        ptx::fence_proxy_async_smem();
                                     }
-                                    if (h1) {
-                                        uint4 *r = reinterpret_cast<uint4 *>(smem_gen + s * STAGE + (t + 128) * 128);
-#pragma unroll
-                                        for (int k = 0; k < 8; ++k) r[k] = z;
-                                    }
-                                    ptx::fence_proxy_async_smem();
+                                    __syncwarp();
+                                    if (lane == 0) ptx::mbar_arrive(bar_fixed + 8 * s);
+                                    if (++s == S) { s = 0; ph ^= 1; }
                                 }
-                                __syncwarp();
-                                if (lane == 0) ptx::mbar_arrive(bar_fixed + 8 * s);
-                                if (++s == S) { s = 0; ph ^= 1; }
+                                if (dead) break;
                             }
-                            if (dead) break;
                         }
                     }
                 }
@@ -1006,8 +1186,6 @@
         }
     }
 
-    __syncthreads();
-    if (s_stat != nullptr && stat_n0 >= 0) tc_stats_final<BLOCK_N>(P, s_stat - (warp - EPI_WARP0) * STAT_SLICE, warp - EPI_WARP0, lane, stat_n0);
 }
 
 
@@ -1024,7 +1202,7 @@
 };
 
 template <int BLOCK_N, int MODE>
-__global__ void __launch_bounds__(TMA_THREADS, 1)
+__global__ void __maxnreg__(TMA_REGS)
 pconv_tc_sp_kernel(const __grid_constant__ TcParams P, const __grid_constant__ SpTable TB, const __grid_constant__ CUtensorMap tmap_w,
                    const __grid_constant__ CUtensorMap tmap_a0, const __grid_constant__ CUtensorMap tmap_a1) {
     constexpr uint32_t B_BYTES = BLOCK_N * 128;
@@ -1059,7 +1237,7 @@
     }
 
     if (threadIdx.x == 0) {
-        for (int s = 0; s < MAX_RING; ++s) { ptx::mbar_init(bar_full + 8 * s, 1); ptx::mbar_init(bar_fixed + 8 * s, 4); ptx::mbar_init(bar_empty + 8 * s, 2); }
+        for (int s = 0; s < MAX_RING; ++s) { ptx::mbar_init(bar_full + 8 * s, 1); ptx::mbar_init(bar_fixed + 8 * s, TMA_FIX_THREADS / 32); ptx::mbar_init(bar_empty + 8 * s, 2); }
         ptx::mbar_init(acc_full, MMA_WARPS); ptx::mbar_init(acc_empty, EPI_WARPS);
         ptx::fence_mbar_init();
     }
@@ -1068,41 +1246,9 @@
 
     float *s_stat = nullptr;
     int stat_n0 = -1;
-    float *acc_stage = reinterpret_cast<float *>(smem_gen + (s_acc - smem_base));
-    if (warp >= EPI_WARP0) {
-        const int w = warp - EPI_WARP0;
-        s_stat = (MODE == 0 && P.bn_sums != nullptr) ? reinterpret_cast<float *>(smem_gen + (s_stat_addr - smem_base)) + w * STAT_SLICE : nullptr;
-        auto origin = [&](int tile, int &m0, int &n0) { m0 = (tile / n_tiles) * BLOCK_M; n0 = (tile % n_tiles) * BLOCK_N; };
-        tma_epilogue_warps<BLOCK_N, MODE>(P, tile0, tstep, num_tiles, origin, acc_stage, acc_full, acc_empty, s_stat, stat_n0, w, lane, 326);
-    } else if (warp == 8) {
-        int s = 0;
-        uint32_t ph = 1;
-        bool dead = false;
-        for (int tile = tile0; tile < num_tiles && !dead; tile += tstep) {
-            const int m0 = (tile / n_tiles) * BLOCK_M, n0 = (tile % n_tiles) * BLOCK_N;
-            const int img = m0 / plane, rem = m0 - img * plane;
-            const int oy = rem / gw, ox = rem - oy * gw;
-            for (int i = 0; i < TB.n_items && !dead; ++i) {
-                const SpItem it = TB.it[i];
-                const CUtensorMap *ma = (it.part == 0) ? &tmap_a0 : &tmap_a1;
-                const int x = ox * TB.step[it.part] + it.dx, y = oy * TB.step[it.part] + it.dy;
-                const uint32_t a_bytes = static_cast<uint32_t>(TB.arows[it.part]) * 128u;
-                for (int cb = 0; cb < nbk[it.part]; ++cb) {
-                    if (!__all_sync(0xffffffffu, ptx::mbar_wait(bar_empty + 8 * s, ph, P.abort_flag, 321))) { dead = true; break; }
-                    if (ptx::elect_one()) {
-                        const uint32_t full = bar_full + 8 * s, dst = smem_base + s * STAGE;
-                        ptx::mbar_arrive_expect_tx(full, a_bytes + it.nb * B_BYTES);
-                        ptx::tma_load_4d(dst, ma, cb * BLOCK_K, x, y, img, full);
-                        uint32_t bdst = dst + A_ROOM;
-                        for (int tc = 0, kb = it.wk + cb * BLOCK_K; tc < it.nb; ++tc, kb += it.wk_step, bdst += B_BYTES)
-                            ptx::tma_load_2d(bdst, &tmap_w, kb, n0, full);
-                    }
-                    __syncwarp();
-                    if (++s == S) { s = 0; ph ^= 1; }
-                }
-            }
-        }
-    } else if (warp < MMA_WARPS) {
+    uint8_t *acc_stage = smem_gen + (s_acc - smem_base);
+    if (warp < MMA_WARPS) {
+        ptx::setmaxnreg_inc<TMA_CONSUMER_REGS>();
         const int e = warp, g = warp >> 2;
         const bool leader = (threadIdx.x & 127) == 0;
         const uint32_t ready = fix ? bar_fixed : bar_full;
@@ -1113,6 +1259,7 @@
         uint32_t ph = 0, aph = 1;
         bool dead = false;
         for (int tile = tile0; tile < num_tiles && !dead; tile += tstep) {
+            const ConsRows cr = cons_rows<MODE>(P, (tile / n_tiles) * BLOCK_M, e, lane);
             float acc[BLOCK_N / 2];
             zero_acc(acc);
             int held = -1;
@@ -1136,75 +1283,115 @@
             ptx::wgmma_fence_regs(acc);
             if (held >= 0 && leader) ptx::mbar_arrive(bar_empty + 8 * held);
             if (dead) break;
-            if (!tma_stage_tile<BLOCK_N>(P, acc, acc_stage, acc_full, acc_empty, aph, e, lane, 325)) break;
-        }
-    } else if (warp > 8) {
-        if (fix) {
-            const int t = (warp - 9) * 32 + lane;
+            if (!tma_stage_tile<BLOCK_N, MODE>(P, acc, acc_stage, acc_full, acc_empty, aph, e, lane, (tile % n_tiles) * BLOCK_N, cr, 325)) break;
+        }
+    } else {
+        ptx::setmaxnreg_dec<TMA_SUPPORT_REGS>();
+        if (warp >= EPI_WARP0) {
+            const int w = warp - EPI_WARP0;
+            s_stat = (MODE == 0 && P.bn_sums != nullptr) ? reinterpret_cast<float *>(smem_gen + (s_stat_addr - smem_base)) + w * EPI_STAT_SLICE : nullptr;
+            auto origin = [&](int tile, int &m0, int &n0) { m0 = (tile / n_tiles) * BLOCK_M; n0 = (tile % n_tiles) * BLOCK_N; };
+            tma_epilogue_warps<BLOCK_N, MODE>(P, tile0, tstep, num_tiles, origin, acc_stage, acc_full, acc_empty, s_stat, stat_n0, w, lane, 326);
+            ptx::named_sync(1, EPI_WARPS * 32);
+            if (s_stat != nullptr && stat_n0 >= 0) tc_stats_final<BLOCK_N>(P, s_stat - w * EPI_STAT_SLICE, w, lane, stat_n0);
+        } else if (warp == 8) {
             int s = 0;
-            uint32_t ph = 0;
+            uint32_t ph = 1;
             bool dead = false;
-            auto load_bits = [&](int tl, uint64_t &b0, uint64_t &b1) {
-                b0 = b1 = 0ull;
-                if (tl >= num_tiles) return;
-                const int m0 = (tl / n_tiles) * BLOCK_M;
+            for (int tile = tile0; tile < num_tiles && !dead; tile += tstep) {
+                const int m0 = (tile / n_tiles) * BLOCK_M, n0 = (tile % n_tiles) * BLOCK_N;
                 const int img = m0 / plane, rem = m0 - img * plane;
                 const int oy = rem / gw, ox = rem - oy * gw;
-                for (int i = 0; i < TB.n_items; ++i) {
+                for (int i = 0; i < TB.n_items && !dead; ++i) {
                     const SpItem it = TB.it[i];
-                    const uint8_t *mk = P.parts[it.part].mask;
-                    if (mk == nullptr) continue;
-                    const int pwid = TB.pw[it.part], phei = TB.ph[it.part], es = TB.es[it.part];
-                    const int hrows = TB.arows[it.part] - BLOCK_M;
-                    const int x0 = ox * TB.step[it.part] + it.dx, y0 = oy * TB.step[it.part] + it.dy;
-                    int tx, ty, tn;
-                    if (hrows > 0 || (P.box_h == 1 && P.box_n == 1)) { tx = t; ty = 0; tn = 0; }
-                    else { tx = t % P.box_w; ty = (t / P.box_w) % P.box_h; tn = t / (P.box_w * P.box_h); }
-                    const int X = x0 + tx * es, Y = y0 + ty * es, IM = img + tn;
-                    if (X >= 0 && X < pwid && Y >= 0 && Y < phei && IM < P.n &&
-                        __ldg(mk + (static_cast<long long>(IM) * phei + Y) * pwid + X) == 0) b0 |= 1ull << i;
-                    if (t < hrows) {
-                        const int X1 = x0 + (t + 128) * es;
-                        if (X1 >= 0 && X1 < pwid && Y >= 0 && Y < phei && __ldg(mk + (static_cast<long long>(IM) * phei + Y) * pwid + X1) == 0) b1 |= 1ull << i;
-                    }
-                }
-            };
-            uint64_t n0b, n1b;
-            load_bits(tile0, n0b, n1b);
-            for (int tile = tile0; tile < num_tiles && !dead; tile += tstep) {
-                const uint64_t c0b = n0b, c1b = n1b;
-                load_bits(tile + tstep, n0b, n1b);
-                for (int i = 0; i < TB.n_items && !dead; ++i) {
-                    const bool h0 = (c0b >> i) & 1ull, h1 = (c1b >> i) & 1ull;
-                    const bool any_hole = __any_sync(0xffffffffu, h0 || h1);
-                    const int nb_i = nbk[TB.it[i].part];
-                    for (int cb = 0; cb < nb_i; ++cb) {
-                        if (!ptx::mbar_wait(bar_full + 8 * s, ph, P.abort_flag, 322)) { dead = true; break; }
-                        if (any_hole) {
-                            const uint4 z = make_uint4(0u, 0u, 0u, 0u);
-                            if (h0) {
-                                uint4 *r = reinterpret_cast<uint4 *>(smem_gen + s * STAGE + t * 128);
-#pragma unroll
-                                for (int k = 0; k < 8; ++k) r[k] = z;
-                            }
-                            if (h1) {
-                                uint4 *r = reinterpret_cast<uint4 *>(smem_gen + s * STAGE + (t + 128) * 128);
-#pragma unroll
-                                for (int k = 0; k < 8; ++k) r[k] = z;
-                            }
-                            ptx::fence_proxy_async_smem();
+                    const CUtensorMap *ma = (it.part == 0) ? &tmap_a0 : &tmap_a1;
+                    const int x = ox * TB.step[it.part] + it.dx, y = oy * TB.step[it.part] + it.dy;
+                    const uint32_t a_bytes = static_cast<uint32_t>(TB.arows[it.part]) * 128u;
+                    for (int cb = 0; cb < nbk[it.part]; ++cb) {
+                        if (!__all_sync(0xffffffffu, ptx::mbar_wait(bar_empty + 8 * s, ph, P.abort_flag, 321))) { dead = true; break; }
+                        if (ptx::elect_one()) {
+                            const uint32_t full = bar_full + 8 * s, dst = smem_base + s * STAGE;
+                            ptx::mbar_arrive_expect_tx(full, a_bytes + it.nb * B_BYTES);
+                            ptx::tma_load_4d(dst, ma, cb * BLOCK_K, x, y, img, full);
+                            uint32_t bdst = dst + A_ROOM;
+                            for (int tc = 0, kb = it.wk + cb * BLOCK_K; tc < it.nb; ++tc, kb += it.wk_step, bdst += B_BYTES)
+                                ptx::tma_load_2d(bdst, &tmap_w, kb, n0, full);
                         }
                         __syncwarp();
-                        if (lane == 0) ptx::mbar_arrive(bar_fixed + 8 * s);
                         if (++s == S) { s = 0; ph ^= 1; }
                     }
                 }
             }
-        }
-    }
-
-    __syncthreads();
-    if (s_stat != nullptr && stat_n0 >= 0) tc_stats_final<BLOCK_N>(P, s_stat - (warp - EPI_WARP0) * STAT_SLICE, warp - EPI_WARP0, lane, stat_n0);
+        } else {
+            if (fix) {
+                constexpr int FR = 3;
+                const int t = (warp - 9) * 32 + lane;
+                int s = 0;
+                uint32_t ph = 0;
+                bool dead = false;
+                auto load_bits = [&](int tl, uint64_t (&b)[FR]) {
+#pragma unroll
+                    for (int r = 0; r < FR; ++r) b[r] = 0ull;
+                    if (tl >= num_tiles) return;
+                    const int m0 = (tl / n_tiles) * BLOCK_M;
+                    const int img = m0 / plane, rem = m0 - img * plane;
+                    const int oy = rem / gw, ox = rem - oy * gw;
+                    for (int i = 0; i < TB.n_items; ++i) {
+                        const SpItem it = TB.it[i];
+                        const uint8_t *mk = P.parts[it.part].mask;
+                        if (mk == nullptr) continue;
+                        const int pwid = TB.pw[it.part], phei = TB.ph[it.part], es = TB.es[it.part];
+                        const int hrows = TB.arows[it.part] - BLOCK_M;
+                        const int x0 = ox * TB.step[it.part] + it.dx, y0 = oy * TB.step[it.part] + it.dy;
+#pragma unroll
+                        for (int r = 0; r < FR; ++r) {
+                            const int row = t + TMA_FIX_THREADS * r;
+                            if (row >= BLOCK_M + hrows) continue;
+                            int tx, ty, tn;
+                            if (hrows > 0 || (P.box_h == 1 && P.box_n == 1)) { tx = row; ty = 0; tn = 0; }
+                            else { tx = row % P.box_w; ty = (row / P.box_w) % P.box_h; tn = row / (P.box_w * P.box_h); }
+                            const int X = x0 + tx * es, Y = y0 + ty * es, IM = img + tn;
+                            if (X >= 0 && X < pwid && Y >= 0 && Y < phei && IM < P.n &&
+                                __ldg(mk + (static_cast<long long>(IM) * phei + Y) * pwid + X) == 0) b[r] |= 1ull << i;
+                        }
+                    }
+                };
+                uint64_t nb_bits[FR];
+                load_bits(tile0, nb_bits);
+                for (int tile = tile0; tile < num_tiles && !dead; tile += tstep) {
+                    uint64_t cb_bits[FR];
+#pragma unroll
+                    for (int r = 0; r < FR; ++r) cb_bits[r] = nb_bits[r];
+                    load_bits(tile + tstep, nb_bits);
+                    for (int i = 0; i < TB.n_items && !dead; ++i) {
+                        bool hole[FR], mine = false;
+#pragma unroll
+                        for (int r = 0; r < FR; ++r) { hole[r] = (cb_bits[r] >> i) & 1ull; mine = mine || hole[r]; }
+                        const bool any_hole = __any_sync(0xffffffffu, mine);
+                        const int nb_i = nbk[TB.it[i].part];
+                        for (int cb = 0; cb < nb_i; ++cb) {
+                            if (!ptx::mbar_wait(bar_full + 8 * s, ph, P.abort_flag, 322)) { dead = true; break; }
+                            if (any_hole) {
+                                const uint4 z = make_uint4(0u, 0u, 0u, 0u);
+#pragma unroll
+                                for (int r = 0; r < FR; ++r)
+                                    if (hole[r]) {
+                                        uint4 *rw = reinterpret_cast<uint4 *>(smem_gen + s * STAGE + (t + TMA_FIX_THREADS * r) * 128);
+#pragma unroll
+                                        for (int k = 0; k < 8; ++k) rw[k] = z;
+                                    }
+                                ptx::fence_proxy_async_smem();
+                            }
+                            __syncwarp();
+                            if (lane == 0) ptx::mbar_arrive(bar_fixed + 8 * s);
+                            if (++s == S) { s = 0; ph ^= 1; }
+                        }
+                    }
+                }
+            }
+        }
+    }
+
 }
 
 __global__ void upsample_part_kernel(const bf16 *__restrict__ src, int cstride, int c8, long long pixels_src, int hs, int ws, bf16 *__restrict__ dst) {
@@ -2075,14 +2262,20 @@
     return (static_cast<size_t>(c->nparts) * c->n * c->ho * c->wo * sizeof(uint64_t) + 255) / 256 * 256;
 }
 
+size_t tma_fixed_smem(int block_n, bool splitk) {
+    return 1024 + TMA_BAR_BYTES + EPI_STAT_SMEM_BYTES + (splitk ? acc_stage_bytes(block_n) : bf16_stage_bytes(block_n));
+}
+
 template <int BLOCK_N, int MODE, bool HALO>
 int launch_tma_n(TcParams &P, const CUtensorMap &tw, const CUtensorMap &ta0, const CUtensorMap &ta1, cudaStream_t st) {
     const int nb = HALO ? P.kw : 1;
     const size_t a_room = (static_cast<size_t>(BLOCK_M + (HALO ? (P.kw - 1) * P.dil : 0)) * 128 + 1023) / 1024 * 1024;
     const size_t stage = a_room + static_cast<size_t>(nb) * BLOCK_N * 128;
-    P.stages = static_cast<int>(std::min<size_t>(MAX_RING, (RING_BUDGET - acc_stage_bytes(BLOCK_N)) / stage));
+    PCB_CHECK(BLOCK_N <= 128 || P.partial == nullptr, "TMA-fed conv: split-K stages fp32 partials, at most 128 columns wide");
+    const size_t fixed = tma_fixed_smem(BLOCK_N, P.partial != nullptr);
+    P.stages = static_cast<int>(std::min<size_t>(MAX_RING, (MAX_SMEM - fixed) / stage));
     PCB_CHECK(P.stages >= 2, "TMA-fed conv: stage of %zu bytes does not fit twice", stage);
-    const size_t smem = 1024 + P.stages * stage + TMA_BAR_BYTES + EPI_STAT_SMEM_BYTES + acc_stage_bytes(BLOCK_N);
+    const size_t smem = fixed + P.stages * stage;
     auto kern = pconv_tc_tma_kernel<BLOCK_N, MODE, HALO>;
     PCB_SMEM_OPT_IN(kern, MAX_SMEM);
     if (P.ksplit < 1) P.ksplit = 1;
@@ -2096,11 +2289,13 @@
 
 template <int MODE>
 int launch_tma(TcParams &P, const CUtensorMap &tw, const CUtensorMap &ta0, const CUtensorMap &ta1, int bn, bool halo, cudaStream_t st) {
+    PCB_CHECK(!(halo && bn == 256), "TMA-fed conv: no 256-wide row-halo tiles");
     if (halo) {
         if (bn == 128) return launch_tma_n<128, MODE, true>(P, tw, ta0, ta1, st);
         if (bn == 64) return launch_tma_n<64, MODE, true>(P, tw, ta0, ta1, st);
         return launch_tma_n<32, MODE, true>(P, tw, ta0, ta1, st);
     }
+    if (bn == 256) return launch_tma_n<256, MODE, false>(P, tw, ta0, ta1, st);
     if (bn == 128) return launch_tma_n<128, MODE, false>(P, tw, ta0, ta1, st);
     if (bn == 64) return launch_tma_n<64, MODE, false>(P, tw, ta0, ta1, st);
     return launch_tma_n<32, MODE, false>(P, tw, ta0, ta1, st);
@@ -2117,9 +2312,12 @@
     return halo_stages_fit(c->kw, c->dil, block_n);
 }
 
-int pick_bn(int cols, long long m_total) {
+int pick_bn(int cols, long long m_total, bool fwd) {
     const long long m_tiles = (m_total + BLOCK_M - 1) / BLOCK_M;
     if (cols <= 32) return 32;
+    const long long sms = pcb_num_sms();
+    auto waves = [&](int b) { return (m_tiles * (cols / b) + sms - 1) / sms; };
+    if (cols % 256 == 0 && 2 * waves(256) <= waves(128) && (!fwd || waves(256) == 1)) return 256;
     int bn = (cols % 128 == 0) ? 128 : 64;
     if (!getenv("PCB_NO_NARROW_N"))
         while (bn > 32 && cols % (bn / 2) == 0 && m_tiles * (cols / bn) < pcb_num_sms() / 2) bn /= 2;
@@ -2296,7 +2494,7 @@
     return 0;
 }
 
-int sp_bn(int cols, long long m_total) { return std::min(pick_bn(cols, m_total), 64); }
+int sp_bn(int cols, long long m_total) { return std::min(pick_bn(cols, m_total, true), 64); }
 
 template <int BLOCK_N, int MODE>
 int launch_sp_n(TcParams &P, const SpTable &TB, const CUtensorMap &tw, const CUtensorMap &ta0, const CUtensorMap &ta1, cudaStream_t st) {
@@ -2304,9 +2502,10 @@
     for (int i = 0; i < TB.n_items; ++i) nb_max = std::max(nb_max, TB.it[i].nb);
     const size_t a_room = (static_cast<size_t>(TB.rows_max) * 128 + 1023) / 1024 * 1024;
     const size_t stage = a_room + static_cast<size_t>(nb_max) * BLOCK_N * 128;
-    P.stages = static_cast<int>(std::min<size_t>(MAX_RING, (RING_BUDGET - acc_stage_bytes(BLOCK_N)) / stage));
+    const size_t fixed = tma_fixed_smem(BLOCK_N, false);
+    P.stages = static_cast<int>(std::min<size_t>(MAX_RING, (MAX_SMEM - fixed) / stage));
     PCB_CHECK(P.stages >= 2, "sub-pixel conv: stage of %zu bytes does not fit twice", stage);
-    const size_t smem = 1024 + P.stages * stage + TMA_BAR_BYTES + EPI_STAT_SMEM_BYTES + acc_stage_bytes(BLOCK_N);
+    const size_t smem = fixed + P.stages * stage;
     auto kern = pconv_tc_sp_kernel<BLOCK_N, MODE>;
     PCB_SMEM_OPT_IN(kern, MAX_SMEM);
     const int num_tiles = ((P.m_total + BLOCK_M - 1) / BLOCK_M) * (P.ncols / BLOCK_N);
@@ -2570,7 +2769,7 @@
     if (tma_fwd_ok(c)) {
         int bw, bh, bn;
         tile_box(c->wo, c->ho, &bw, &bh, &bn);
-        if (tma_halo_ok(c, bw, bh, bn, pick_bn(c->cout <= 32 ? 32 : L.rows_f, m_total))) return 0;
+        if (tma_halo_ok(c, bw, bh, bn, pick_bn(c->cout <= 32 ? 32 : L.rows_f, m_total, true))) return 0;
     }
     return launch_tapmask(c, tapmask, st);
 }
@@ -2627,7 +2826,7 @@
     CUtensorMap tm;
     if (tma_fwd_ok(c)) {
         tile_box(c->wo, c->ho, &P.box_w, &P.box_h, &P.box_n);
-        const int bn = pick_bn(c->cout <= 32 ? 32 : L.rows_f, m_total);
+        const int bn = pick_bn(c->cout <= 32 ? 32 : L.rows_f, m_total, true);
         const bool halo = tma_halo_ok(c, P.box_w, P.box_h, P.box_n, bn);
         const int hx = halo ? (c->kw - 1) * c->dil : 0;
         CUtensorMap ta[TC_MAX_PARTS];
@@ -2721,7 +2920,7 @@
     CUtensorMap tm;
     if (tma_dgrad_ok(c)) {
         tile_box(c->w, c->h, &P.box_w, &P.box_h, &P.box_n);
-        bn = pick_bn(L.ktap, m_total);
+        bn = pick_bn(L.ktap, m_total, false);
         const bool halo = tma_halo_ok(c, P.box_w, P.box_h, P.box_n, bn);
         P.wk_base = 0; P.wk_col = L.cout64; P.wk_row = c->kw * L.cout64;
         CUtensorMap ta;
@@ -2745,7 +2944,7 @@
         const int hh = c->h / 2, hw = c->w / 2;
         const long long m_class = static_cast<long long>(c->n) * hh * hw;
         tile_box(hw, hh, &P.box_w, &P.box_h, &P.box_n);
-        bn = pick_bn(L.ktap, m_class);
+        bn = pick_bn(L.ktap, m_class, false);
         if (int rc = make_tmap_2d(&tm, w_dgrad, rup(L.ktap, 128), L.kd, L.kd, bn)) return rc;
         const long long class_tiles = ((m_class + BLOCK_M - 1) / BLOCK_M) * (L.ktap / bn);
         const bool fork = class_tiles < pcb_num_sms() && !getenv("PCB_DISABLE_CLASS_STREAMS");
diff --git a/text_segmentation_image_inpainting_b200/csrc/pcb_ptx.cuh b/text_segmentation_image_inpainting_b200/csrc/pcb_ptx.cuh
--- a/text_segmentation_image_inpainting_b200/csrc/pcb_ptx.cuh
+++ b/text_segmentation_image_inpainting_b200/csrc/pcb_ptx.cuh
@@ -120,7 +120,12 @@
 template <int N, int TA, int TB> __device__ __forceinline__ void wgmma_bf16(float (&d)[N / 2], uint64_t a_desc, uint64_t b_desc) {
     if constexpr (N == 32) wgmma_m64n32<TA, TB>(d, a_desc, b_desc);
     else if constexpr (N == 64) wgmma_m64n64<TA, TB>(d, a_desc, b_desc);
-    else { static_assert(N == 128, "wgmma tile width"); wgmma_m64n128<TA, TB>(d, a_desc, b_desc); }
+    else if constexpr (N == 128) wgmma_m64n128<TA, TB>(d, a_desc, b_desc);
+    else {
+        static_assert(N == 256 && TB == 0, "wgmma tile width");
+        wgmma_m64n128<TA, TB>(*reinterpret_cast<float (*)[64]>(&d[0]), a_desc, b_desc);
+        wgmma_m64n128<TA, TB>(*reinterpret_cast<float (*)[64]>(&d[64]), a_desc, b_desc + (16384 >> 4));
+    }
 }
 template <int N> __device__ __forceinline__ void setmaxnreg_inc() { asm volatile("setmaxnreg.inc.sync.aligned.u32 %0;" ::"n"(N)); }
 template <int N> __device__ __forceinline__ void setmaxnreg_dec() { asm volatile("setmaxnreg.dec.sync.aligned.u32 %0;" ::"n"(N)); }
```

Result: faster. 950.0 (median of 6 runs) (+3.4%).
